# Excalibur1224/Cuda-v-MPI

Hardware: AMD Instinct MI355X
Metric: Riemann subintervals/sec at N=1e9 fp64; |error| vs analytic π (higher is better)
Workload: dtype fp64

## Files before the change

### csrc/cli/miint.cpp

```cpp
#include <algorithm>
#include <cmath>
#include <cstdio>
#include <string>
#include <vector>

#include "cli_common.hpp"
#include "miint/integrator.hpp"
#include "miint/oracle.hpp"
#include "miint/table2d.hpp"
#include "miint/trainscan.hpp"

using namespace miint;

namespace {

struct BenchRow {
  std::string integrand, dtype, rule;
  double n = 0, result = 0, exact = 0, ms = 0;
  int gpus = 1;
  int block = 0, grid = 0;
  bool multistep = false, close_in_launch = false, allreduce_to_host = false;
  BatchDiag diag;
  std::string timeline_file;
  cli::RankFacts facts;
  cli::Topology topo;
};

Integrand integrand_of(const std::string& s) { return cli::parse_integrand(s); }

RiemannConfig make_cfg(const std::string& integ, double n, const std::string& dtype,
                       const std::string& rule, const std::string& div) {
  RiemannConfig c;
  c.integrand = integrand_of(integ);
  c.a = 0.0;
  c.b = c.integrand == Integrand::kPi4 || c.integrand == Integrand::kPoly ? 1.0
      : c.integrand == Integrand::kSin ? 3.14159265358979323846 : 1800.0;
  c.n = static_cast<uint64_t>(n);
  c.dtype = cli::parse_dtype(dtype);
  c.rule = cli::parse_rule(rule);
  c.div = cli::parse_div(div);
  if (c.integrand == Integrand::kTrainVel) { c.p0 = oracle::kTrainTs; c.p1 = oracle::kTrainVs; }
  if (c.integrand == Integrand::kTable) c.table = oracle::profile_table();
  if (c.integrand == Integrand::kPoly) c.coef = {0.3, -1.2, 0.7, 0.05, -0.4, 0.9, 0.1};
  return c;
}

template <class T>
void write_rows(std::FILE* f, const std::vector<T>& v, size_t cols) {
  std::fputc('[', f);
  for (size_t i = 0; i < v.size(); ++i) {
    if (i % cols == 0) std::fputs(i ? ",[" : "[", f);
    else std::fputc(',', f);
    std::fprintf(f, "%llu", static_cast<unsigned long long>(v[i]));
    if (i % cols == cols - 1) std::fputc(']', f);
  }
  std::fputc(']', f);
}

void write_timeline(const std::string& path, const BatchTimeline& t, const RiemannConfig& cfg,
                    const std::string& integrand, const std::string& dtype,
                    const std::string& div, double plain_device_us) {
  std::FILE* f = std::fopen(path.c_str(), "w");
  if (!f) fail("--timeline: cannot open " + path + " for writing", __FILE__, __LINE__);
  std::fprintf(f, "{\"integrand\":\"%s\",\"n\":%llu,", cli::json_escape(integrand).c_str(),
               static_cast<unsigned long long>(cfg.n));
  if (cfg.slice_world > 0)
    std::fprintf(f, "\"slice_of\":[%d,%d],", cfg.slice_rank, cfg.slice_world);
  else
    std::fputs("\"slice_of\":null,", f);
  std::fprintf(f, "\"dtype\":\"%s\",\"div\":\"%s\",", cli::json_escape(dtype).c_str(),
               cli::json_escape(div).c_str());
  std::fprintf(f, "\"steps\":%d,\"grid\":%d,\"block\":%d,\"clock_khz\":%d,\"device_us\":%.17g,",
               t.steps, t.grid, t.block, t.clock_khz, t.device_us);
  if (plain_device_us > 0) std::fprintf(f, "\"plain_device_us\":%.17g,", plain_device_us);
  else std::fputs("\"plain_device_us\":null,", f);
  std::fputs("\"values\":[", f);
  for (size_t i = 0; i < t.values.size(); ++i)
    std::fprintf(f, i ? ",%.17g" : "%.17g", t.values[i]);
  std::fputs("],\n\"stamps\":", f);
  write_rows(f, t.stamps, static_cast<size_t>(t.steps) + 2);
  std::fputs(",\n\"shader_clock\":", f);
  write_rows(f, t.shader_clock, 2);
  std::fputs(",\n\"hw\":", f);
  write_rows(f, t.hw, 2);
  std::fputs("}\n", f);
  if (std::fclose(f) != 0) fail("--timeline: writing " + path + " failed", __FILE__, __LINE__);
}

struct TimelineRequest {
  std::string file, integrand, dtype, div;
};

BenchRow bench_one(const cli::Topology& topo, RiemannConfig cfg, int iters, bool graphs,
                   int settle_steps = -1, bool diagnose = false,
                   const TimelineRequest& timeline = {}) {
  BenchRow row;
  row.n = static_cast<double>(cfg.n);
  row.gpus = topo.world;
  row.exact = oracle::analytic(cfg.integrand, cfg.a, cfg.b, cfg.coef, cfg.p0, cfg.p1);
  row.topo = topo;
  std::mutex mu;
  cli::run_ranks(topo, [&](int rank, int dev, const Comm* comm) {
    RiemannPlan plan(cfg, dev, comm);
    RankAgree agree(comm);
    plan.run_steps(3, comm != nullptr, graphs);
    const double est_s = static_cast<double>(plan.count()) / 1.3e13;
    const int settle = settle_steps >= 0 ? settle_steps
                       : static_cast<int>(std::min(20000.0, std::max(3.0, 0.06 / est_s)));
    plan.run_steps(settle, comm != nullptr, graphs);
    StepTiming t = plan.run_steps(iters, comm != nullptr, graphs);
    const double ms = agree.max(t.wall_s * 1e3 / iters);
    BatchDiag d;
    if (diagnose) d = plan.diagnose_batch(std::min(iters, plan.config().slots));
    if (!timeline.file.empty()) {
      const BatchTimeline tl = plan.timeline_batch(std::min(iters, plan.config().slots));
      if (rank == 0)
        write_timeline(timeline.file, tl, cfg, timeline.integrand, timeline.dtype, timeline.div,
                       d.steps == tl.steps ? d.device_us : 0.0);
    }
    std::lock_guard<std::mutex> g(mu);
    if (ms > row.ms) row.ms = ms;
    if (rank == topo.rank0) {
      row.facts.note(comm);
      row.result = plan.host_result(plan.host_index_of(iters - 1, graphs));
      row.block = plan.shape().block;
      row.grid = plan.shape().grid;
      row.multistep = plan.multistep();
      row.close_in_launch = plan.close_in_launch();
      row.allreduce_to_host = plan.allreduce_to_host();
      row.diag = d;
      row.timeline_file = timeline.file;
    }
  });
  return row;
}

void print_row(const cli::Args& a, const BenchRow& r, const char* integ, const char* dtype,
               const char* rule) {
  cli::JsonRecord rec;
  rec.add("integrand", integ).add("dtype", dtype).add("rule", rule).add("n", r.n).add("gpus", r.gpus);
  r.facts.add(rec, r.topo);
  rec.add("block", r.block)
                   .add("grid", r.grid)
                   .add("multistep", r.multistep)
                   .add("close_in_launch", r.close_in_launch)
                   .add("allreduce_to_host", r.allreduce_to_host)
                   .add("ms_per_integration", r.ms)
                   .add("subintervals_per_s", r.n / (r.ms * 1e-3))
                   .add("result", r.result)
                   .add("analytic", r.exact)
                   .add("abs_err", std::fabs(r.result - r.exact));
  if (r.diag.steps > 0)
    rec.add("diag_steps", r.diag.steps)
        .add("diag_compute_us", r.diag.compute_us)
        .add("diag_close_us", r.diag.close_us)
        .add("diag_allreduce_us", r.diag.allreduce_us)
        .add("diag_copy_us", r.diag.copy_us)
        .add("diag_tail_us", r.diag.tail_us())
        .add("diag_boundary_us", r.diag.boundary_us())
        .add("diag_device_us", r.diag.device_us)
        .add("diag_marker_us", r.diag.marker_us)
        .add("diag_host_us", r.diag.wall_us - r.diag.device_us);
  if (!r.timeline_file.empty()) rec.add("timeline_file", r.timeline_file);
  cli::emit(a, rec, true);
}

int selfcheck() {
  int bad = 0;
  auto check = [&](const char* what, double got, double want, double tol) {
    const bool ok = std::fabs(got - want) <= tol;
    std::printf("%-44s got %.9f want %.9f  %s\n", what, got, want, ok ? "ok" : "MISMATCH");
    bad += !ok;
  };
  {
    RiemannPlan p(make_cfg("pi4", 1e9, "fp64", "left", "series"), 0);
    check("pi4 left N=1e9 (|err| = h)", p.run(), 3.14159265358979323846 + 1e-9, 2e-12);
  }
  {
    RiemannPlan p(make_cfg("pi4", 1e9, "fp64", "mid", "series"), 0);
    check("pi4 mid N=1e9", p.run(), 3.14159265358979323846, 1e-13);
  }
  {
    RiemannPlan p(make_cfg("sin", 1e9, "fp64", "left", "series"), 0);
    check("sin [0,pi] N=1e9", p.run(), 2.0, 1e-12);
  }
  {
    RiemannConfig c = make_cfg("table", 18e6, "fp64", "left", "series");
    RiemannPlan p(c, 0);
    check("cintegrate full coverage", p.run(), 122000.004000, 1e-6);
    c.b = 1792.0;
    c.n = 17920000;
    RiemannPlan q(c, 0);
    check("cintegrate --parity (SP=32,SM=2)", q.run(), 121999.800663, 5e-6);
  }
  {
    TrainScanConfig tc;
    TrainScan ts(tc, 0);
    const TrainScanResult r = ts.run();
    check("trainscan distance (P=1)", r.distance, 122000.004000, 1e-6);
  }
  std::printf("%s\n", bad ? "SELFCHECK FAILED" : "SELFCHECK OK");
  return bad ? 1 : 0;
}

int comm_sweep(const cli::Args& a, const cli::Topology& topo, double max_bytes, int iters) {
  std::vector<size_t> counts;
  for (size_t c = 1; c * 8.0 <= max_bytes; c *= 8) counts.push_back(c);
  if (counts.empty() || counts.back() * 8.0 < max_bytes) counts.push_back(static_cast<size_t>(max_bytes / 8));
  const char* ops[] = {"allreduce", "allgather", "broadcast"};
  std::vector<double> ms(counts.size() * 3, 0.0);
  std::mutex mu;
  auto body = [&](int , int dev, const Comm* comm) {
    DeviceGuard g(dev);
    Stream s;
    RankAgree agree(comm);
    const size_t cmax = counts.back();
    DeviceBuffer<double> a(cmax), b(cmax * static_cast<size_t>(comm->world()));
    MIINT_HIP(hipMemsetAsync(a.get(), 0, a.bytes(), s.get()));
    Event e0, e1;
    for (size_t k = 0; k < counts.size(); ++k)
      for (int op = 0; op < 3; ++op) {
        auto issue = [&] {
          if (op == 0) comm->allreduce_sum(a.get(), b.get(), counts[k], s.get());
          else if (op == 1) comm->allgather(a.get(), b.get(), counts[k], s.get());
          else comm->broadcast(a.get(), counts[k], 0, s.get());
        };
        for (int w = 0; w < 3; ++w) issue();
        s.sync();
        agree.barrier();
        e0.record(s.get());
        for (int i = 0; i < iters; ++i) issue();
        e1.record(s.get());
        e1.sync();
        comm->check_async();
        const double t = agree.max(Event::elapsed_ms(e0, e1) / iters);
        std::lock_guard<std::mutex> l(mu);
        ms[k * 3 + op] = std::max(ms[k * 3 + op], t);
      }
  };
  capture_rccl_log();
  if (!topo.multiproc && topo.world == 1) {
    auto one = RcclComm::init_all({0});
    body(0, 0, one[0].get());
  } else {
    cli::run_ranks(topo, body);
  }
  if (topo.rank0 != 0) return 0;
  const double P = topo.world;
  const RcclTransport tr = rccl_transport();
  const bool share = ranks_share_devices() && topo.world > 1;
  const std::string terr = transport_error(
      tr, topo.world, topo.multiproc ? cli::env_int("LOCAL_WORLD_SIZE", topo.world) : topo.world,
      share);
  if (!terr.empty()) std::fprintf(stderr, "miint comm: transport check: %s\n", terr.c_str());
  for (size_t k = 0; k < counts.size(); ++k)
    for (int op = 0; op < 3; ++op) {
      const double bytes = counts[k] * 8.0 * (op == 1 ? P : 1.0);
      const double t = ms[k * 3 + op];
      const double alg = bytes / (t * 1e-3) / 1e9;
      const double factor = op == 0 ? 2.0 * (P - 1) / P : (op == 1 ? (P - 1) / P : 1.0);
      cli::emit(a, cli::JsonRecord()
                       .add("op", ops[op])
                       .add("gpus", topo.world)
                       .add("bytes", bytes)
                       .add("us", t * 1e3)
                       .add("algbw_GBps", alg)
                       .add("busbw_GBps", alg * factor)
                       .add("ranks_share_gpus", ranks_share_devices() && topo.world > 1)
                       .add("rccl_transport", tr.transport)
                       .add("rccl_nnodes", tr.nnodes)
                       .add("transport_verified", terr.empty()),
                true);
    }
  return 0;
}

}

constexpr const char* kUsage =
    "usage: miint info\n"
    "       miint bench [--integrand pi4] [--n 1e9] [--dtype fp64|fp32|fp32acc] [--rule left]\n"
    "                   [--iters 200] [--gpus G] [--div series_exact|series|ieee] [--unfused] [--no-graph]\n"
    "                   [--block B] [--grid G] [--step-streams S] [--trig-library] [--settle N]\n"
    "                   [--no-multistep] [--slots K] [--close auto|kernel|launch] [--no-ar-host]\n"
    "                   [--diagnose] [--slice R/W] [--timeline FILE]\n"
    "                   (--timeline: after the timed run, one batch from the timeline build of\n"
    "                   the multi-step launch, per-workgroup device-clock stamps as JSON in FILE;\n"
    "                   read it with tools/timeline_report.py. --slice: rank R's share of W)\n"
    "       miint sweep [--gpus G]\n"
    "       miint table2d [--grid 4096] [--gpus G] [--slice R/W] [--no-graph]\n"
    "                     [--step-streams S] [--min-wg W] [--settle-ms MS] [--no-multistep]\n"
    "                     [--phases P] [--graph-steps K]\n"
    "       miint selfcheck\n"
    "       miint comm [--gpus G] [--max-bytes 144e6] [--iters 20]\n"
    "Every record is one JSON line on stdout; --jsonl FILE also appends it to FILE.\n";

int main(int argc, char** argv) {
  try {
    cli::Args a(argc, argv);
    if (cli::usage_requested(a, kUsage)) return 0;
    const std::string cmd = a.positional().empty() ? "info" : a.positional()[0];
    if (cmd == "info") {
      const int nd = device_count();
      std::printf("miint: %d HIP device(s), RCCL %s\n", nd, nd ? RcclComm::version().c_str() : "-");
      for (int d = 0; d < nd; ++d) {
        const DeviceInfo i = device_info(d);
        std::printf("  [%d] %s %s  %d CUs  %.1f GHz  %.1f GB  L2 %d KB  LDS %zu KB/CU (%zu KB/block)\n",
                    d, i.name.c_str(), i.arch.c_str(), i.num_cus, i.clock_khz / 1e6,
                    i.total_mem / 1e9, i.l2_bytes / 1024, i.lds_per_cu / 1024,
                    i.lds_per_block / 1024);
      }
      return 0;
    }
    if (cmd == "selfcheck") return selfcheck();
    {
      int r = 0, w = 0;
      cli::parse_slice(a, &r, &w);
    }
    const cli::Topology topo = cli::topology(a);
    const int iters = static_cast<int>(a.integer("iters", 100));
    const bool graphs = !a.flag("no-graph");
    if (cmd == "bench") {
      RiemannConfig c = make_cfg(a.str("integrand", "pi4"), a.num("n", 1e9), a.str("dtype", "fp64"),
                                 a.str("rule", "left"), a.str("div", "series_exact"));
      c.fused = !a.flag("unfused");
      c.grid = static_cast<int>(a.integer("grid", 0));
      c.block = static_cast<int>(a.integer("block", kRiemannBlock));
      c.step_streams = static_cast<int>(a.integer("step-streams", 0));
      c.multistep = !a.flag("no-multistep");
      c.slots = static_cast<int>(a.integer("slots", c.slots));
      c.close = a.str("close", c.close);
      c.allreduce_to_host = !a.flag("no-ar-host");
      cli::parse_slice(a, &c.slice_rank, &c.slice_world);
      TimelineRequest tl;
      tl.file = a.str("timeline", "");
      tl.integrand = a.str("integrand", "pi4");
      tl.dtype = a.str("dtype", "fp64");
      tl.div = a.str("div", "series_exact");
      if (!tl.file.empty() && c.close == "launch")
        fail(std::string("--timeline: ") + kTimelineNoCloseInLaunch, __FILE__, __LINE__);
      if (a.flag("trig-library")) set_trig_library(true);
      MIINT_CHECK(riemann_block_ok(c.block), "--block must be 64, 128, 256, 512 or 1024");
      c.waves_per_cu = static_cast<int>(a.integer("waves-per-cu", 32));
      const BenchRow r = bench_one(topo, c, iters, graphs,
                                   static_cast<int>(a.integer("settle", -1)),
                                   a.flag("diagnose"), tl);
      if (topo.rank0 == 0)
        print_row(a, r, a.str("integrand", "pi4").c_str(), a.str("dtype", "fp64").c_str(),
                  a.str("rule", "left").c_str());
      return 0;
    }
    if (cmd == "table2d") {
      Table2DConfig c;
      c.grid = static_cast<int>(a.integer("grid", 4096));
      c.bucket = !a.flag("no-bucket");
      c.chain = !a.flag("no-chain");
      c.step_streams = static_cast<int>(a.integer("step-streams", 0));
      c.min_wg = static_cast<int>(a.integer("min-wg", 0));
      c.settle_ms = a.num("settle-ms", c.settle_ms);
      c.multistep = !a.flag("no-multistep");
      c.phases = static_cast<int>(a.integer("phases", 0));
      c.graph_steps = static_cast<int>(a.integer("graph-steps", 0));
      cli::parse_slice(a, &c.rank, &c.world);
      double value = 0.0, timed = 0.0, ms = 0.0;
      bool bucketed = false, chained = false, multistep = false;
      int streams = 1, phases = 0, resident = 0, min_wg = 0, wgs = 0, gsteps = 0;
      cli::RankFacts facts;
      std::mutex mu;
      cli::run_ranks(topo, [&](int rank, int dev, const Comm* comm) {
        Table2DPlan plan(c, dev, comm);
        RankAgree agree(comm);
        const double v = plan.run();
        const double t = agree.max(plan.time(iters, graphs));
        std::lock_guard<std::mutex> g(mu);
        if (rank == topo.rank0) {
          facts.note(comm);
          value = v;
          timed = plan.last_result();
          bucketed = plan.bucketed() && graphs;
          chained = plan.chained() && graphs;
          multistep = plan.multistep() && graphs;
          streams = chained ? plan.step_streams() : 1;
          phases = multistep ? plan.phases() : 0;
          resident = plan.resident_per_cu();
          min_wg = plan.min_wg();
          wgs = plan.workgroups();
          gsteps = graphs ? plan.graph_steps() : 0;
        }
        if (t > ms) ms = t;
      });
      if (topo.rank0 == 0) {
        cli::JsonRecord r;
        r.add("program", "table2d").add("grid", c.grid);
        r.add("step_streams", streams).add("multistep", multistep).add("phases", phases);
        r.add("resident_per_cu", resident).add("min_wg", min_wg).add("workgroups", wgs);
        r.add("graph_steps", gsteps);
        facts.add(r, topo);
        if (c.world > 1) {
          r.add("slice", std::to_string(c.rank) + "/" + std::to_string(c.world))
              .add("partial", value);
        } else {
          const double want = table2d_oracle(c.grid);
          const double exact = 122000.004 * 122000.004;
          r.add("gpus", topo.world)
              .add("result", value)
              .add("timed_result", timed)
              .add("bucketed_allreduce", bucketed)
              .add("chained", chained)
              .add("midpoint_oracle", want)
              .add("rel_err_vs_oracle", std::fabs(value - want) / want)
              .add("rel_err_vs_exact", std::fabs(value - exact) / exact)
              .add("samples_per_s", static_cast<double>(c.grid) * c.grid / (ms * 1e-3));
        }
        cli::emit(a, r.add("ms_per_integration", ms), true);
      }
      return 0;
    }
    if (cmd == "comm") return comm_sweep(a, topo, a.num("max-bytes", 144e6), static_cast<int>(a.integer("iters", 20)));
    if (cmd == "sweep") {
      const std::vector<double> ns = {1e6, 1e9, 1e10};
      const std::vector<std::string> integs = {"pi4", "sin", "poly", "train"};
      for (const auto& integ : integs)
        for (const char* dt : {"fp64", "fp32"}) {
          if (std::string(dt) == "fp32" && integ != "pi4") continue;
          for (double n : ns) {
            if (integ != "pi4" && n > 1e9) continue;
            RiemannConfig c = make_cfg(integ, n, dt, "left", "series");
            const int it = n >= 1e10 ? 10 : (n >= 1e9 ? 50 : 500);
            const BenchRow r = bench_one(topo, c, it, graphs);
            if (topo.rank0 == 0) print_row(a, r, integ.c_str(), dt, "left");
          }
        }
      return 0;
    }
    std::fprintf(stderr, "usage: miint info|bench|sweep|table2d|comm|selfcheck [--flags]\n");
    return 2;
  } catch (const std::exception& e) {
    std::fprintf(stderr, "miint: %s\n", e.what());
    return 1;
  }
}
```

### csrc/include/miint/integrator.hpp

```cpp
#pragma once

#include <hip/hip_runtime.h>

#include <cstdint>
#include <map>
#include <memory>
#include <string>
#include <vector>

#include "miint/comm.hpp"
#include "miint/common.hpp"
#include "miint/kernels.hpp"
#include "miint/runtime.hpp"

namespace miint {

constexpr int kAutoStepStreams = 4;
constexpr uint64_t kStepStreamsMaxCount = 600000000ull;

struct RiemannConfig {
  Integrand integrand = Integrand::kPi4;
  double a = 0.0, b = 1.0;
  uint64_t n = 1000000000ull;
  Rule rule = Rule::kLeft;
  DType dtype = DType::kF64;
  DivMode div = DivMode::kSeriesExact;
  std::vector<double> coef;
  double p0 = 0.0, p1 = 0.0;
  std::vector<double> table;
  int grid = 0;
  int block = kRiemannBlock;
  int waves_per_cu = 32;
  bool fused = true;
  bool chain = true;
  bool host_direct = true;
  int slots = 16;
  bool bucket = true;
  int rank = 0, world = 1;
  bool force_collective = false;
  bool multistep = true;
  std::string close = "auto";
  bool allreduce_to_host = true;
  int step_streams = 0;
  int slice_rank = 0, slice_world = 0;
  double timeout_s = 300.0;
};

inline void rank_slice(uint64_t n, int r, int w, uint64_t* begin, uint64_t* count) {
  const uint64_t q = n / static_cast<uint64_t>(w), rem = n % static_cast<uint64_t>(w);
  const uint64_t ur = static_cast<uint64_t>(r);
  *count = q + (ur < rem ? 1 : 0);
  *begin = ur * q + (ur < rem ? ur : rem);
}

struct StepTiming {
  double wall_s = 0.0;
  double device_ms = 0.0;
  int steps = 0;
};

struct OneShotTiming {
  std::string mode;
  int reps = 0;
  double median_us = 0.0, min_us = 0.0, max_us = 0.0;
  double device_median_us = 0.0, device_min_us = 0.0;
  double value = 0.0;
};

struct BatchDiag {
  int steps = 0;
  double compute_us = 0.0;
  double close_us = 0.0;
  double allreduce_us = 0.0;
  double copy_us = 0.0;
  double marker_us = 0.0;
  double device_us = 0.0;
  double staged_us = 0.0;
  double wall_us = 0.0;
  double tail_us() const { return close_us + allreduce_us + copy_us; }
  double boundary_us() const { return device_us - compute_us - tail_us(); }
};

struct BatchTimeline {
  int steps = 0, grid = 0, block = 0;
  int clock_khz = 0;
  std::vector<uint64_t> stamps;
  std::vector<uint64_t> shader_clock;
  std::vector<uint32_t> hw;
  double device_us = 0.0;
  std::vector<double> values;
};
constexpr uint64_t kTimelineUnsetStamp = 0;
constexpr uint32_t kTimelineUnsetId = 0xffffffffu;

class RiemannPlan {
 public:
  RiemannPlan(const RiemannConfig& cfg, int device, const Comm* comm = nullptr);
  ~RiemannPlan();
  RiemannPlan(const RiemannPlan&) = delete;
  RiemannPlan& operator=(const RiemannPlan&) = delete;

  const RiemannConfig& config() const { return cfg_; }
  int device() const { return device_; }
  int rank() const { return rank_; }
  int world() const { return world_; }
  uint64_t begin() const { return params_.i_begin; }
  uint64_t count() const { return params_.n; }
  double h() const { return params_.h; }
  double scale() const { return scale_; }
  LaunchShape shape() const { return shape_; }
  DivMode effective_div() const;
  bool direct() const { return direct_; }

  void enqueue_compute(hipStream_t s, int slot, int host_index) const;
  void enqueue_reduce(hipStream_t s, int slot) const;
  void enqueue_copyout(hipStream_t s, int slot, int host_index) const;
  void enqueue(hipStream_t s, int slot, int host_index) const;

  double* device_result(int slot) const { return result_.get() + slot; }
  double host_result(int host_index) const { return host_[host_index]; }
  int host_capacity() const { return static_cast<int>(host_.size()); }
  int slots() const { return cfg_.slots; }

  double run();
  void capture_graphs();
  void prepare_steps(int steps);
  bool graphs_ready() const { return !graphs_.empty() && graph_error_.empty(); }
  const std::string& graph_error() const { return graph_error_; }
  size_t graph_nodes() const;
  long graph_launches() const { return graph_launches_; }
  long direct_steps() const { return direct_steps_; }

  StepTiming run_steps(int steps, bool pipeline, bool graphs);
  BatchDiag diagnose_batch(int nsteps);
  BatchTimeline timeline_batch(int nsteps);
  void barrier();
  OneShotTiming time_one_shot(int reps, const std::string& mode, int warmup = 400);
  void launch_steps(int steps, bool pipeline, bool graphs);
  void sync() const;
  int host_index_of(int k, bool graphs) const;
  hipStream_t compute_stream() const { return compute_.get(); }
  hipStream_t comm_stream() const { return comm_stream_.get(); }

  bool collective() const { return comm_ && (world_ > 1 || cfg_.force_collective); }
  bool bucketed() const { return collective() && cfg_.bucket; }
  bool chained() const { return cfg_.fused && cfg_.chain && (!collective() || bucketed()); }
  bool multistep() const { return chained() && multistep_; }
  bool close_in_launch() const { return multistep() && close_launch_; }
  bool allreduce_to_host() const {
    return bucketed() && cfg_.allreduce_to_host && ar_host_ok_;
  }
  void check_allreduce_to_host();

 private:
  void enqueue_batch(hipStream_t cs, hipStream_t rs, int nsteps, bool overlap);
  void enqueue_bucket_reduce(hipStream_t s, int nsteps) const;
  void enqueue_chain(hipStream_t s, int nsteps) const;
  void enqueue_chain_streams(hipStream_t cs, int nsteps);
 public:
  int step_streams(int nsteps) const;
 private:
  const Graph* batch_graph(int nsteps);
  bool use_graphs(bool requested, int steps);
  double* result_ptr(int j) const { return direct_ ? host_.device_ptr() + j : result_.get() + j; }

  RiemannConfig cfg_;
  int device_;
  const Comm* comm_;
  int rank_ = 0, world_ = 1;
  bool direct_ = false;
  RiemannParams params_{};
  double scale_ = 1.0;
  LaunchShape shape_{1, kRiemannBlock};
  DeviceBuffer<double> partials_;
  DeviceBuffer<double> slots_;
  DeviceBuffer<double> ms_partials_;
  bool multistep_ = false;
  bool close_launch_ = false;
  bool capturing_ = false;
  bool ar_host_ok_ = true;
  bool ar_host_checked_ = false;
  DeviceBuffer<unsigned int> ms_ticket_;
  DeviceBuffer<uint64_t> tl_stamps_, tl_shader_;
  DeviceBuffer<uint32_t> tl_hw_;
  DeviceBuffer<double> result_;
  DeviceBuffer<double> sync_;
  DeviceBuffer<unsigned int> ticket_;
  DeviceBuffer<double> table_;
  PinnedBuffer<double> host_;
  Stream compute_;
  Stream comm_stream_;
  std::vector<Stream> step_streams_;
  std::vector<std::unique_ptr<Event>> ev_step_join_;
  std::vector<std::unique_ptr<Event>> ev_computed_, ev_drained_;
  Event ev_fork_, ev_join_;
  Event ev_t0_, ev_t1_;
  std::map<int, std::unique_ptr<Graph>> graphs_;
  std::string graph_error_;
  long graph_launches_ = 0, direct_steps_ = 0;
  int last_mode_ = -1;
};

}
```

### csrc/include/miint/kernels.hpp

```cpp
#pragma once

#include <hip/hip_runtime.h>

#include <algorithm>
#include <cmath>
#include <cstddef>
#include <cstdint>

#include "miint/common.hpp"

namespace miint {

enum class DType : int { kF64 = 0, kF32 = 1, kF32Acc32 = 2 };
inline bool is_fp32(DType t) { return t == DType::kF32 || t == DType::kF32Acc32; }

constexpr int kRiemannTile = 32;
constexpr int kRiemannBlock = 256;
constexpr int kSeriesHalfSpan = 192;
constexpr int kSeriesHalfSpanF32 = 96;

constexpr int kDirectHalfSpan = 16;

inline bool series_ok(double h) { return kSeriesHalfSpan * (h < 0 ? -h : h) <= 2e-6; }
inline bool series_ok_f32(double h) { return kSeriesHalfSpanF32 * (h < 0 ? -h : h) <= 2e-6; }
inline bool direct_ok(double h) { return kDirectHalfSpan * (h < 0 ? -h : h) <= 2e-6; }

inline DivMode effective_div(DivMode d, double h) {
  if (d == DivMode::kIeee) return d;
  if ((d == DivMode::kSeries || d == DivMode::kSeriesExact) && series_ok(h)) return d;
  return direct_ok(h) ? DivMode::kSeriesDirect : DivMode::kIeee;
}
inline bool series_request(DivMode d) { return d == DivMode::kSeries || d == DivMode::kSeriesExact; }
inline DivMode effective_div(DivMode d, double h, Integrand f) {
  if (f == Integrand::kSin || f == Integrand::kTrainVel || f == Integrand::kTable)
    return series_request(d) ? DivMode::kSeries : DivMode::kIeee;
  if (f != Integrand::kPi4) return DivMode::kIeee;
  return effective_div(d, h);
}

constexpr int kPolySeriesMaxCoeffs = 8;

inline DivMode effective_div(DivMode d, double h, Integrand f, DType t, int ncoef = 0) {
  if (is_fp32(t)) {
    if (d == DivMode::kIeee) return DivMode::kIeee;
    if (f == Integrand::kPi4) return series_ok_f32(h) ? DivMode::kSeries : DivMode::kIeee;
    if (f == Integrand::kPoly)
      return (ncoef >= 1 && ncoef <= kPolySeriesMaxCoeffs) ? DivMode::kSeries : DivMode::kIeee;
    return DivMode::kSeries;
  }
  if (f == Integrand::kPoly)
    return (series_request(d) && ncoef >= 1 && ncoef <= kPolySeriesMaxCoeffs)
               ? DivMode::kSeries
               : DivMode::kIeee;
  return effective_div(d, h, f);
}

constexpr double kTrigSeriesMaxN = 2147418112.0;
inline bool trig_series_in_range(const RiemannParams& p) {
  const Integrand f = static_cast<Integrand>(p.integrand);
  if (f != Integrand::kSin && f != Integrand::kTrainVel) return true;
  const double first = static_cast<double>(p.i_begin) + p.off;
  const double last = static_cast<double>(p.i_begin + (p.n > 0 ? p.n - 1 : 0)) + p.off;
  const double w = f == Integrand::kTrainVel ? 1.0 / p.p0 : 1.0;
  const double n0 = std::fabs(std::fma(first, p.h, p.a) * w) * 6.36619772367581382433e-01;
  const double n1 = std::fabs(std::fma(last, p.h, p.a) * w) * 6.36619772367581382433e-01;
  return n0 <= kTrigSeriesMaxN && n1 <= kTrigSeriesMaxN;
}
constexpr double kPi4SeriesMaxX = 0x1p249;
constexpr double kPi4SeriesMaxXF32 = 0x1p62;
inline bool pi4_series_in_range(const RiemannParams& p, DType t) {
  if (static_cast<Integrand>(p.integrand) != Integrand::kPi4) return true;
  const double lim = is_fp32(t) ? kPi4SeriesMaxXF32 : kPi4SeriesMaxX;
  const double first = static_cast<double>(p.i_begin) + p.off;
  const double last = static_cast<double>(p.i_begin + (p.n > 0 ? p.n - 1 : 0)) + p.off;
  return std::fabs(std::fma(first, p.h, p.a)) < lim && std::fabs(std::fma(last, p.h, p.a)) < lim;
}
inline DivMode effective_div(const RiemannParams& p, DivMode d, DType t) {
  const DivMode e = effective_div(d, p.h, static_cast<Integrand>(p.integrand), t, p.ncoef);
  return (e != DivMode::kIeee && !(trig_series_in_range(p) && pi4_series_in_range(p, t)))
             ? DivMode::kIeee
             : e;
}

struct LaunchShape {
  int grid;
  int block;
};

bool riemann_block_ok(int block);
LaunchShape default_riemann_shape(int num_cus, int waves_per_cu = 32, int block = kRiemannBlock);

void launch_riemann_partials(const RiemannParams& p, DType dtype, DivMode div,
                             LaunchShape shape, const double* table, int table_n,
                             double* partials, hipStream_t stream);

void launch_finalize(const double* partials, int n, double scale, double* out,
                     hipStream_t stream, int block = kRiemannBlock);

constexpr unsigned kUnsetSlotWord = 0xFFFAFFFAu;
void fill_unset_slots(double* p, size_t count, hipStream_t stream);

constexpr int kTicketGroups = 16;
constexpr int kTicketStride = 64;
constexpr int kTicketWords = (kTicketGroups + 1) * kTicketStride;

void launch_riemann_fused(const RiemannParams& p, DType dtype, DivMode div, LaunchShape shape,
                          const double* table, int table_n, double* partials,
                          unsigned int* ticket, double scale, double* out, hipStream_t stream);

void launch_riemann_chained(const RiemannParams& p, DType dtype, DivMode div, LaunchShape shape,
                            const double* table, int table_n, double* partials,
                            const double* prev, int nprev, double scale, double* out_prev,
                            hipStream_t stream);

constexpr int kMaxMultiSteps = 64;
int riemann_multistep_grid(const RiemannParams& p, DType dtype, DivMode div, int block,
                           int num_cus, bool close = false);
void launch_riemann_multistep(const RiemannParams& p, DType dtype, DivMode div,
                              LaunchShape shape, const double* table, int table_n,
                              double* partials, int steps, double scale, double* out,
                              hipStream_t stream, unsigned int* ticket = nullptr,
                              bool close_kernel = true);
constexpr const char* kTimelineNoCloseInLaunch =
    "the timeline instruments the kernel-closed multi-step launch only (not close = launch)";
int riemann_timeline_grid(const RiemannParams& p, DType dtype, DivMode div, int block,
                          int num_cus);
void launch_riemann_timeline(const RiemannParams& p, DType dtype, DivMode div,
                             LaunchShape shape, const double* table, int table_n,
                             double* partials, int steps, double scale, double* out,
                             hipStream_t stream, uint64_t* stamps, uint64_t* shader_clock,
                             uint32_t* hw, unsigned int* ticket = nullptr,
                             bool close_kernel = true);
void launch_multistep_close(const double* partials, int grid, int steps, double scale,
                            double* out, int block, hipStream_t stream);

void launch_riemann_point_values(const RiemannParams& p, DivMode div, const double* table,
                                 int table_n, double* out, hipStream_t stream);

void launch_pi4_recip_narrow(const double* d, uint64_t n, double* out, hipStream_t stream);
void launch_pi4_recip_narrow_f32(const float* d, uint64_t n, float* out, hipStream_t stream);
void set_pi4_library_division(bool on);
bool pi4_ieee_narrow(const RiemannParams& p, DType dtype);
void set_trig_library(bool on);
void set_lds_poison(bool on);
void set_lds_poison_trainscan(bool on);
void set_lds_poison_table(bool on);

int riemann_tile_len(const RiemannParams& p, DType dtype, DivMode div);

double integrand_scale(Integrand f);

int default_reduce_grid(int num_cus);
void launch_sum_array(const double* x, uint64_t n, double scale, double* partials, int grid,
                      double* out, hipStream_t stream);

void launch_interp_fill(const double* table, int table_n, double dt, uint64_t i0, uint64_t n,
                        double* y, hipStream_t stream);

size_t scan_state_bytes(uint64_t n);
void launch_inclusive_scan(const double* in, double* out, uint64_t n, void* state,
                           const double* carry_in, hipStream_t stream);
void launch_interp_scan(const double* table, int table_n, double dt, uint64_t i0, uint64_t n,
                        double* out, void* state, const double* carry_in, hipStream_t stream);
void launch_interp_scan_window(const double* table, int table_n, double dt, uint64_t i0,
                               uint64_t n, uint64_t win_lo, uint64_t win_hi, double* out,
                               void* state, const double* carry_in, hipStream_t stream);
unsigned scan_timeout_flag(const void* state, hipStream_t stream);
void launch_add_carry(double* x, uint64_t n, const double* carry, hipStream_t stream);

struct Table2DParams {
  const double* table;
  int nx, ny;
  double X, Y;
  int gx, gy;
  int row0, row1;
  int min_wg = 0;
};
int table2d_grid(const Table2DParams& p);
const char* table2d_path(const Table2DParams& p);
struct Table2DShapeInfo {
  bool stream;
  int rows_per_wave, tile_rows, tile_cols, grid_x, grid_y, tile;
};
Table2DShapeInfo table2d_shape_info(const Table2DParams& p);
constexpr int kT2AutoPhases = 16;
constexpr long kT2AutoWorkgroups = 4096;
constexpr int kT2MaxPhases = 32;
constexpr int kT2MaxReplaySteps = 1024;
bool table2d_multistep_ok(const Table2DParams& p, int num_cus);
int table2d_multistep_resident(const Table2DParams& p);
int table2d_multistep_phases(const Table2DParams& p, int num_cus, int steps, int want = 0);
void launch_table2d_multistep(const Table2DParams& p, double* partials, int steps, double* outs,
                              hipStream_t stream, int phases = 1);
void launch_table2d_partials(const Table2DParams& p, double* partials, hipStream_t stream);
void launch_table2d_fused(const Table2DParams& p, double* partials, unsigned* ticket,
                          double* out, hipStream_t stream);
void launch_table2d_chained(const Table2DParams& p, double* partials, const double* prev,
                            double* prev_out, hipStream_t stream);
void launch_table2d_finalize(const double* partials, int n, double* out, hipStream_t stream);
void launch_outer_product(const double* v, int n, double* table, hipStream_t stream);

}
```

### csrc/kernels/riemann.hip

```cpp
#include <hip/hip_runtime.h>

#include <atomic>
#include <cmath>
#include <string>

#include "miint/common.hpp"
#include "miint/handoff.hpp"
#include "miint/integrands.hpp"
#include "miint/integrands_f32.hpp"
#include "miint/kernels.hpp"
#include "miint/wave_reduce.hpp"

namespace miint {
namespace {

constexpr int B = kRiemannBlock;
constexpr int kMaxBlock = 1024;

__device__ __forceinline__ uint64_t readlane_u64(uint64_t v, int lane) {
  const uint32_t lo = __builtin_amdgcn_readlane(static_cast<uint32_t>(v), lane);
  const uint32_t hi = __builtin_amdgcn_readlane(static_cast<uint32_t>(v >> 32), lane);
  return (static_cast<uint64_t>(hi) << 32) | lo;
}

// ... 412 lines not shown

#define kFullOccupancy __attribute__((amdgpu_waves_per_eu(8, 8)))
template <DivMode M, class F>
constexpr bool occupancy_hint() {
  if constexpr (__is_same(F, Pi4)) return M == DivMode::kSeriesDirect;
  else if constexpr (__is_same(F, Pi4F32) || __is_same(F, Pi4F32Wide) ||
                     __is_same(F, Pi4F32Acc32))
    return M == DivMode::kIeee;
  else if constexpr (__is_same(F, SinLib) || __is_same(F, TrainVelLib)) return true;
  else if constexpr (__is_same(F, Sin)) return M == DivMode::kIeee;
  else if constexpr (__is_same(F, PolyF32<16>)) return true;
  else if constexpr (IsPoly<F>::value) return M == DivMode::kSeries;
  else if constexpr (__is_same(F, SinF32) || __is_same(F, TrainVelF32))
    return M == DivMode::kSeries;
  else return __is_same(F, TrainVel) || __is_same(F, Table) || __is_same(F, TableF32);
}

template <DivMode M, class F>
__device__ __forceinline__ void partials_body(const RiemannParams& p, const double* table,
                                              int table_n, double* partials) {
  using Acc = typename AccOf<F>::type;
  __shared__ Acc red[kMaxBlock / kWave];
  __shared__ double lds[lds_words<M, F>()];
  const F f = make_functor<M, F>(p, table, table_n, lds);
  const double s = static_cast<double>(block_sum_dyn(lane_sum<M>(p, f, blockIdx.x), red));
  if (threadIdx.x == 0) partials[blockIdx.x] = s;
}
template <DivMode M, class F>
__global__ __launch_bounds__(kMaxBlock) void riemann_kernel(RiemannParams p, const double* table,
                                                    int table_n, double* partials) {
  partials_body<M, F>(p, table, table_n, partials);
}
template <DivMode M, class F>
__global__ __launch_bounds__(kMaxBlock) kFullOccupancy void riemann_kernel_o8(RiemannParams p,
                                                                      const double* table,
                                                                      int table_n,
                                                                      double* partials) {
  partials_body<M, F>(p, table, table_n, partials);
}

__device__ __forceinline__ double ordered_sum(const double* partials, int n, double* red) {
  return block_sum_dyn(ordered_partials<0, false>(partials, n), red);
}

__global__ __launch_bounds__(kMaxBlock) void finalize_kernel(const double* partials, int n,
                                                             double scale, double* out) {
  __shared__ double red[kMaxBlock / kWave];
  const double s = ordered_sum(partials, n, red);
  if (threadIdx.x == 0) out[0] = s * scale;
}

template <DivMode M, class F>
__device__ __forceinline__ void fused_body(const RiemannParams& p, const double* table,
                                           int table_n, double* partials, unsigned int* ticket,
                                           double scale, double* out) {
  using Acc = typename AccOf<F>::type;
  __shared__ double red[kMaxBlock / kWave];
  __shared__ Acc red_acc[__is_same(Acc, double) ? 1 : kMaxBlock / kWave];
  __shared__ double lds[lds_words<M, F>()];
  __shared__ int is_last;
  const F f = make_functor<M, F>(p, table, table_n, lds);
  double s;
  if constexpr (__is_same(Acc, double)) s = block_sum_dyn(lane_sum<M>(p, f, blockIdx.x), red);
  else s = static_cast<double>(block_sum_dyn(lane_sum<M>(p, f, blockIdx.x), red_acc));
  if (!publish_and_ticket(s, partials, ticket, blockIdx.x, gridDim.x, &is_last)) return;
  const double v = ordered_partials<0, true>(partials, static_cast<int>(gridDim.x));
  rearm_slots<0>(partials, static_cast<int>(gridDim.x));
  const double tot = block_sum_dyn(v, red);
  if (threadIdx.x == 0) out[0] = tot * scale;
  rearm_ticket(ticket, gridDim.x);
}
template <DivMode M, class F>
__global__ __launch_bounds__(kMaxBlock) void riemann_fused_kernel(RiemannParams p, const double* table,
                                                          int table_n, double* partials,
                                                          unsigned int* ticket, double scale,
                                                          double* out) {
  fused_body<M, F>(p, table, table_n, partials, ticket, scale, out);
}
template <DivMode M, class F>
__global__ __launch_bounds__(kMaxBlock) kFullOccupancy void riemann_fused_kernel_o8(
    RiemannParams p, const double* table, int table_n, double* partials, unsigned int* ticket,
    double scale, double* out) {
  fused_body<M, F>(p, table, table_n, partials, ticket, scale, out);
}

template <DivMode M, class F>
__device__ __forceinline__ void chained_body(const RiemannParams& p, const double* table,
                                             int table_n, double* partials, const double* prev,
                                             int nprev, double scale, double* out_prev) {
  __shared__ double red[kMaxBlock / kWave];
  __shared__ double lds[lds_words<M, F>()];
  if (prev != nullptr && blockIdx.x == gridDim.x - 1) {
    const double tot = block_sum_dyn(ordered_partials<0, false>(prev, nprev), red);
    if (threadIdx.x == 0) out_prev[0] = tot * scale;
    __syncthreads();
  }
  const F f = make_functor<M, F>(p, table, table_n, lds);
  double s;
  if constexpr (__is_same(typename AccOf<F>::type, double)) {
    s = block_sum_dyn(lane_sum<M>(p, f, blockIdx.x), red);
  } else {
    __shared__ typename AccOf<F>::type red_acc[kMaxBlock / kWave];
    s = static_cast<double>(block_sum_dyn(lane_sum<M>(p, f, blockIdx.x), red_acc));
  }
  if (threadIdx.x == 0) partials[blockIdx.x] = s;
}
template <DivMode M, class F>
__global__ __launch_bounds__(kMaxBlock) void riemann_chained_kernel(RiemannParams p, const double* table,
                                                            int table_n, double* partials,
                                                            const double* prev, int nprev,
                                                            double scale, double* out_prev) {
  chained_body<M, F>(p, table, table_n, partials, prev, nprev, scale, out_prev);
}
template <DivMode M, class F>
__global__ __launch_bounds__(kMaxBlock) kFullOccupancy void riemann_chained_kernel_o8(
    RiemannParams p, const double* table, int table_n, double* partials, const double* prev,
    int nprev, double scale, double* out_prev) {
  chained_body<M, F>(p, table, table_n, partials, prev, nprev, scale, out_prev);
}

#ifndef MIINT_MS_CHUNK
#define MIINT_MS_CHUNK 1
#endif
template <class F>
constexpr int ms_chunk() {
  return __is_same(F, Pi4) ? MIINT_MS_CHUNK : 1;
}

struct TimelineOut {
  unsigned long long* stamps;
  unsigned long long* shader_clock;
  unsigned* hw;
};
__device__ __forceinline__ unsigned long long timeline_realtime() {
  unsigned long long t;
  asm volatile("s_memrealtime %0\n\ts_waitcnt lgkmcnt(0)" : "=s"(t) : : "memory");
  return t;
}
__device__ __forceinline__ unsigned long long timeline_realtime_after(double sum) {
  unsigned long long t;
  asm volatile("s_memrealtime %0\n\ts_waitcnt lgkmcnt(0)" : "=s"(t) : "v"(sum) : "memory");
  return t;
}
__device__ __forceinline__ unsigned long long timeline_shader_clock() {
  unsigned long long t;
  asm volatile("s_memtime %0\n\ts_waitcnt lgkmcnt(0)" : "=s"(t) : : "memory");
  return t;
}
template <class T>
__device__ __forceinline__ T* timeline_row(T* base, int row_len) {
  unsigned wg = blockIdx.x;
  asm volatile("" : "+v"(wg));
  return base + static_cast<size_t>(wg) * static_cast<size_t>(row_len);
}
struct TimelineEntry {
  unsigned long long t, clk;
};
__device__ __forceinline__ TimelineEntry timeline_entry() {
  TimelineEntry e;
  e.t = timeline_realtime();
  e.clk = timeline_shader_clock();
  return e;
}
__device__ __forceinline__ void timeline_step(const TimelineOut& tl, int steps, int s,
                                              double sum) {
  const unsigned long long t = timeline_realtime_after(sum);
  timeline_row(tl.stamps, steps + 2)[s + 1] = t;
}
__device__ __forceinline__ void timeline_exit(const TimelineOut& tl, int steps,
                                              const TimelineEntry& e) {
  const unsigned long long t = timeline_realtime();
  unsigned long long* clk = timeline_row(tl.shader_clock, 2);
  clk[0] = e.clk;
  clk[1] = timeline_shader_clock();
  unsigned long long* st = timeline_row(tl.stamps, steps + 2);
  st[0] = e.t;
  st[steps + 1] = t;
  unsigned xcc, hw;
  asm volatile("s_getreg_b32 %0, hwreg(HW_REG_XCC_ID)" : "=s"(xcc));
  asm volatile("s_getreg_b32 %0, hwreg(HW_REG_HW_ID)" : "=s"(hw));
  unsigned* id = timeline_row(tl.hw, 2);
  id[0] = xcc;
  id[1] = hw;
}

template <DivMode M, class F, bool CLOSE, bool TL = false>
__device__ __forceinline__ void multistep_body(const RiemannParams& p, const double* table,
                                               int table_n, double* partials, int steps,
                                               unsigned rot, unsigned* ticket, double scale,
                                               double* out, TimelineOut tl = {}) {
  using Acc = typename AccOf<F>::type;
  constexpr int C = ms_chunk<F>();
  if constexpr (TL) {
    static_assert(!CLOSE, "the timeline covers the kernel-closed step loop only");
    static_assert(C == 1, "the timeline covers one step per block sum (MIINT_MS_CHUNK = 1)");
  }
  TimelineEntry te{};
  if constexpr (TL) te = timeline_entry();
  __shared__ double red[2][C * (kMaxBlock / kWave)];
  __shared__ Acc red_acc[2][__is_same(Acc, double) ? 1 : C * (kMaxBlock / kWave)];
  __shared__ double lds[lds_words<M, F>()];
  const F f = make_functor<M, F>(p, table, table_n, lds);
  const unsigned nb = gridDim.x;
  const TileSplit sp = tile_split<F::template tile_len<M>()>(p.n);
  unsigned vb = blockIdx.x;
  unsigned seq = 0;
  int s = 0;
  if constexpr (C > 1) {
    for (; s + C <= steps; s += C, ++seq) {
      const unsigned vb0 = vb;
      Acc l[C];
#pragma unroll
      for (int k = 0; k < C; ++k) l[k] = Acc(0);
#pragma unroll 1
      for (int c = 0; c < C; ++c) {
        RiemannParams q = p;
        asm volatile("" : "+s"(q.a));
        const Acc x = lane_sum<M>(q, f, vb, sp);
#pragma unroll
        for (int k = 0; k < C; ++k) l[k] = k == c ? x : l[k];
        vb += rot;
        if (vb >= nb) vb -= nb;
      }
      Acc v[C];
      if constexpr (__is_same(Acc, double)) block_sums_dyn<C>(l, red[seq & 1], v);
      else block_sums_dyn<C>(l, red_acc[seq & 1], v);
      if (threadIdx.x == 0) {
        unsigned w = vb0;
#pragma unroll
        for (int k = 0; k < C; ++k) {
          const double vk = static_cast<double>(v[k]);
          if constexpr (CLOSE) slot_store(&partials[static_cast<size_t>(s + k) * nb + w], vk);
          else partials[static_cast<size_t>(s + k) * nb + w] = vk;
          w += rot;
          if (w >= nb) w -= nb;
        }
      }
    }
  }
  for (; s < steps; ++s, ++seq) {
    RiemannParams q = p;
    asm volatile("" : "+s"(q.a));
    double v;
    if constexpr (__is_same(Acc, double)) v = block_sum_dyn(lane_sum<M>(q, f, vb, sp), red[seq & 1]);
    else v = static_cast<double>(block_sum_dyn(lane_sum<M>(q, f, vb, sp), red_acc[seq & 1]));
    if (threadIdx.x == 0) {
      if constexpr (TL) timeline_step(tl, steps, s, v);
      if constexpr (CLOSE) slot_store(&partials[static_cast<size_t>(s) * nb + vb], v);
      else partials[static_cast<size_t>(s) * nb + vb] = v;
    }
    vb += rot;
    if (vb >= nb) vb -= nb;
  }
  if constexpr (TL) {
    if (threadIdx.x == 0) timeline_exit(tl, steps, te);
  }
  if constexpr (CLOSE) {
    __shared__ int role;
    __syncthreads();
    close_batch_in_launch(partials, nb, steps, ticket, scale, out, red[0], &role);
  }
}
template <DivMode M, class F>
__global__ __launch_bounds__(kMaxBlock) void riemann_timeline_kernel(
    RiemannParams p, const double* table, int table_n, double* partials, int steps,
    unsigned rot, TimelineOut tl) {
  multistep_body<M, F, false, true>(p, table, table_n, partials, steps, rot, nullptr, 0.0,
                                    nullptr, tl);
}
template <DivMode M, class F>
__global__ __launch_bounds__(kMaxBlock) kFullOccupancy void riemann_timeline_kernel_o8(
    RiemannParams p, const double* table, int table_n, double* partials, int steps,
    unsigned rot, TimelineOut tl) {
  multistep_body<M, F, false, true>(p, table, table_n, partials, steps, rot, nullptr, 0.0,
                                    nullptr, tl);
}
template <DivMode M, class F, bool CLOSE>
__global__ __launch_bounds__(kMaxBlock) void riemann_multistep_kernel(
    RiemannParams p, const double* table, int table_n, double* partials, int steps,
    unsigned rot, unsigned* ticket, double scale, double* out) {
  multistep_body<M, F, CLOSE>(p, table, table_n, partials, steps, rot, ticket, scale, out);
}
template <DivMode M, class F, bool CLOSE>
__global__ __launch_bounds__(kMaxBlock) kFullOccupancy void riemann_multistep_kernel_o8(
    RiemannParams p, const double* table, int table_n, double* partials, int steps,
    unsigned rot, unsigned* ticket, double scale, double* out) {
  multistep_body<M, F, CLOSE>(p, table, table_n, partials, steps, rot, ticket, scale, out);
}
template <DivMode M, class F>
constexpr bool multistep_o8() {
  if constexpr (__is_same(F, Table) || __is_same(F, TableF32)) return true;
  return M == DivMode::kIeee && (__is_same(F, Pi4F32) || __is_same(F, Pi4F32Wide) ||
                                 __is_same(F, Pi4F32Acc32));
}
template <DivMode M, class F>
constexpr bool multistep_close_ok() {
  return !multistep_o8<M, F>();
}
template <DivMode M, class F>
constexpr bool multistep_pays() {
  return !(M == DivMode::kIeee && (__is_same(F, Pi4) || __is_same(F, Pi4Wide)));
}

__global__ __launch_bounds__(kMaxBlock) void multistep_close_kernel(const double* partials,
                                                                   int nb, double scale,
                                                                   double* out) {
  __shared__ double red[kMaxBlock / kWave];
  const double t = ordered_partials<0, false>(partials + static_cast<size_t>(blockIdx.x) * nb, nb);
  const double tot = block_sum_dyn(t, red);
  if (threadIdx.x == 0) out[blockIdx.x] = tot * scale;
}

template <DivMode M, class F>
__global__ __launch_bounds__(B) void point_values_kernel(RiemannParams p, const double* table,
                                                         int table_n, double* out) {
  constexpr int T = F::template tile_len<M>();
  __shared__ double lds[lds_words<M, F>()];
  const F f = make_functor<M, F>(p, table, table_n, lds);
  const uint64_t t = static_cast<uint64_t>(blockIdx.x) * B + threadIdx.x;
  if (t * T >= p.n) return;
  const double x0 = fma(static_cast<double>(p.i_begin) + p.off + static_cast<double>(t * T),
                        p.h, p.a);
  const double xm = fma(0.5 * (T - 1), p.h, x0);
  const bool full = (t + 1) * T <= p.n;
  for (int u = 0; u < T && t * T + u < p.n; ++u) {
    const double x = fma(static_cast<double>(u), p.h, x0);
    double v;
    if constexpr (M == DivMode::kSeries && __is_same(F, Pi4)) {
      v = full ? f.series_point(xm, p.h, u) : f.point(x);
    } else if constexpr (M == DivMode::kSeriesExact && __is_same(F, Pi4)) {
      v = full ? f.series_exact_point(xm, p.h, u) : f.point(x);
    } else if constexpr (M == DivMode::kSeries && IsPolyF64<F>::value) {
      v = full ? f.series_point(xm, u) : f.point(x);
    } else if constexpr (M == DivMode::kSeries && __is_same(F, Table)) {
      v = full ? f.series_point(xm, p.h, u) : f.point(x);
    } else if constexpr (M == DivMode::kSeries && (__is_same(F, Sin) || __is_same(F, TrainVel))) {
      v = full ? f.series_point(xm, u) : f.point(x);
    } else if constexpr (M == DivMode::kSeriesDirect && __is_same(F, Pi4)) {
      const Pi4::Seed sd = Pi4::seed(xm, p.h);
      const double e = fma(-fma(x, x, 1.0), sd.s, 1.0);
      v = fma(sd.s, e + e * e, sd.s);
    } else if constexpr (M == DivMode::kIeee && __is_same(F, Pi4)) {
      v = full ? Pi4::recip_narrow(fma(x, x, 1.0)) : f.point(x);
    } else if constexpr (M == DivMode::kIeee &&
                         (__is_same(F, Sin) || __is_same(F, SinLib) ||
                          __is_same(F, TrainVel) || __is_same(F, TrainVelLib))) {
      v = full ? f.template ieee_point<T>(x0, p.h, u) : f.point(x);
    } else {
      v = f.point(x);
    }
    out[t * T + u] = v * F::kScale;
  }
}

__global__ __launch_bounds__(B) void recip_narrow_kernel(const double* d, uint64_t n,
                                                         double* out) {
  const uint64_t stride = static_cast<uint64_t>(gridDim.x) * B;
  for (uint64_t i = static_cast<uint64_t>(blockIdx.x) * B + threadIdx.x; i < n; i += stride)
    out[i] = Pi4::recip_narrow(d[i]);
}
__global__ __launch_bounds__(B) void recip_narrow_f32_kernel(const float* d, uint64_t n,
                                                             float* out) {
  const uint64_t stride = static_cast<uint64_t>(gridDim.x) * B;
  for (uint64_t i = static_cast<uint64_t>(blockIdx.x) * B + threadIdx.x; i < n; i += stride)
    out[i] = Pi4F32::recip_narrow(f32x2{d[i], d[i]}).x;
}

template <DivMode M, class F>
void launch_partials_t(const RiemannParams& p, LaunchShape shape, const double* table,
                       int table_n, double* partials, hipStream_t stream) {
  if constexpr (occupancy_hint<M, F>())
    riemann_kernel_o8<M, F><<<shape.grid, shape.block, 0, stream>>>(p, table, table_n, partials);
  else
    riemann_kernel<M, F><<<shape.grid, shape.block, 0, stream>>>(p, table, table_n, partials);
}
template <DivMode M, class F>
void launch_fused_t(const RiemannParams& p, LaunchShape shape, const double* table, int table_n,
                    double* partials, unsigned* ticket, double scale, double* out,
                    hipStream_t stream) {
  if constexpr (occupancy_hint<M, F>())
    riemann_fused_kernel_o8<M, F>
        <<<shape.grid, shape.block, 0, stream>>>(p, table, table_n, partials, ticket, scale, out);
  else
    riemann_fused_kernel<M, F>
        <<<shape.grid, shape.block, 0, stream>>>(p, table, table_n, partials, ticket, scale, out);
}

template <DivMode M, class F>
void launch_chained_t(const RiemannParams& p, LaunchShape shape, const double* table,
                      int table_n, double* partials, const double* prev, int nprev, double scale,
                      double* out_prev, hipStream_t stream) {
  if constexpr (occupancy_hint<M, F>())
    riemann_chained_kernel_o8<M, F><<<shape.grid, shape.block, 0, stream>>>(p, table, table_n, partials,
                                                                  prev, nprev, scale, out_prev);
  else
    riemann_chained_kernel<M, F><<<shape.grid, shape.block, 0, stream>>>(p, table, table_n, partials,
                                                               prev, nprev, scale, out_prev);
}

template <DivMode M, class F, bool CLOSE>
void launch_multistep_c(const RiemannParams& p, LaunchShape shape, const double* table,
                        int table_n, double* partials, int steps, unsigned rot,
                        unsigned* ticket, double scale, double* out, hipStream_t stream) {
  if constexpr (multistep_o8<M, F>())
    riemann_multistep_kernel_o8<M, F, CLOSE><<<shape.grid, shape.block, 0, stream>>>(
        p, table, table_n, partials, steps, rot, ticket, scale, out);
  else
    riemann_multistep_kernel<M, F, CLOSE><<<shape.grid, shape.block, 0, stream>>>(
        p, table, table_n, partials, steps, rot, ticket, scale, out);
}
template <DivMode M, class F>
void launch_multistep_t(const RiemannParams& p, LaunchShape shape, const double* table,
                        int table_n, double* partials, int steps, unsigned rot,
                        unsigned* ticket, double scale, double* out, hipStream_t stream) {
  if constexpr (multistep_pays<M, F>()) {
    if constexpr (multistep_close_ok<M, F>()) {
      if (ticket) {
        launch_multistep_c<M, F, true>(p, shape, table, table_n, partials, steps, rot, ticket,
                                       scale, out, stream);
        return;
      }
    } else {
      MIINT_CHECK(ticket == nullptr, "this integrand closes multi-step batches by a kernel");
    }
    launch_multistep_c<M, F, false>(p, shape, table, table_n, partials, steps, rot, ticket,
                                    scale, out, stream);
  } else {
    fail("this integrand/division keeps chained batches (no multi-step kernel)", __FILE__,
         __LINE__);
  }
}
template <DivMode M, class F, bool CLOSE>
int multistep_occupancy(int block) {
  int n = 0;
  if constexpr (multistep_o8<M, F>())
    MIINT_HIP(hipOccupancyMaxActiveBlocksPerMultiprocessor(
        &n, reinterpret_cast<const void*>(&riemann_multistep_kernel_o8<M, F, CLOSE>), block, 0));
  else
    MIINT_HIP(hipOccupancyMaxActiveBlocksPerMultiprocessor(
        &n, reinterpret_cast<const void*>(&riemann_multistep_kernel<M, F, CLOSE>), block, 0));
  return n;
}
template <DivMode M, class F>
void multistep_per_cu_t(int block, bool close, int* out) {
  if constexpr (!multistep_pays<M, F>())
    *out = 0;
  else if constexpr (!multistep_close_ok<M, F>())
    *out = close ? 0 : multistep_occupancy<M, F, false>(block);
  else
    *out = close ? multistep_occupancy<M, F, true>(block) : multistep_occupancy<M, F, false>(block);
}

template <DivMode M, class F>
void launch_timeline_t(const RiemannParams& p, LaunchShape shape, const double* table,
                       int table_n, double* partials, int steps, unsigned rot, TimelineOut tl,
                       hipStream_t stream) {
  if constexpr (!multistep_pays<M, F>())
    fail("this integrand/division keeps chained batches (no multi-step kernel, no timeline)",
         __FILE__, __LINE__);
  else if constexpr (multistep_o8<M, F>())
    riemann_timeline_kernel_o8<M, F><<<shape.grid, shape.block, 0, stream>>>(
        p, table, table_n, partials, steps, rot, tl);
  else
    riemann_timeline_kernel<M, F><<<shape.grid, shape.block, 0, stream>>>(
        p, table, table_n, partials, steps, rot, tl);
}
template <DivMode M, class F>
void timeline_per_cu_t(int block, int* out) {
  *out = 0;
  if constexpr (multistep_pays<M, F>()) {
    if constexpr (multistep_o8<M, F>())
      MIINT_HIP(hipOccupancyMaxActiveBlocksPerMultiprocessor(
          out, reinterpret_cast<const void*>(&riemann_timeline_kernel_o8<M, F>), block, 0));
    else
      MIINT_HIP(hipOccupancyMaxActiveBlocksPerMultiprocessor(
          out, reinterpret_cast<const void*>(&riemann_timeline_kernel<M, F>), block, 0));
  }
}

std::atomic<bool> g_pi4_library_division{false};
std::atomic<bool> g_trig_library{false};
inline bool trig_library() { return g_trig_library.load(std::memory_order_relaxed); }
inline bool pi4_narrow(const RiemannParams& p, double max_x = kPi4NarrowMaxX) {
  if (g_pi4_library_division.load(std::memory_order_relaxed)) return false;
  const double first = static_cast<double>(p.i_begin) + p.off;
  const double last = static_cast<double>(p.i_begin + (p.n > 0 ? p.n - 1 : 0)) + p.off;
  return std::fabs(std::fma(first, p.h, p.a)) < max_x &&
         std::fabs(std::fma(last, p.h, p.a)) < max_x;
}

template <template <DivMode, class> class Op, class... A>
void dispatch(const RiemannParams& p, DType dtype, DivMode m, A&&... a) {
  const Integrand f = static_cast<Integrand>(p.integrand);
  if (dtype == DType::kF32Acc32) {
    MIINT_CHECK(f == Integrand::kPi4, "fp32 accumulation (fp32acc) is implemented for pi4 only");
    if (m == DivMode::kSeries) Op<DivMode::kSeries, Pi4F32Acc32>::run(a...);
    else if (pi4_narrow(p, kPi4F32NarrowMaxX)) Op<DivMode::kIeee, Pi4F32Acc32>::run(a...);
    else fail("fp32acc: coordinates beyond 2^49 need the wide division (use fp32)", __FILE__,
              __LINE__);
    return;
  }
  if (dtype == DType::kF32) {
    const bool ser = m == DivMode::kSeries;
    switch (f) {
      case Integrand::kPi4:
        if (ser) Op<DivMode::kSeries, Pi4F32>::run(a...);
        else if (pi4_narrow(p, kPi4F32NarrowMaxX)) Op<DivMode::kIeee, Pi4F32>::run(a...);
        else Op<DivMode::kIeee, Pi4F32Wide>::run(a...);
        return;
      case Integrand::kSin:
        if (ser) Op<DivMode::kSeries, SinF32>::run(a...);
        else if (!trig_series_in_range(p)) Op<DivMode::kIeee, Sin>::run(a...);
        else Op<DivMode::kIeee, SinF32>::run(a...);
        return;
      case Integrand::kTrainVel:
        if (ser) Op<DivMode::kSeries, TrainVelF32>::run(a...);
        else if (!trig_series_in_range(p)) Op<DivMode::kIeee, TrainVel>::run(a...);
        else Op<DivMode::kIeee, TrainVelF32>::run(a...);
        return;
      case Integrand::kTable:
        if (ser) Op<DivMode::kSeries, TableF32>::run(a...);
        else Op<DivMode::kIeee, TableF32>::run(a...);
        return;
      case Integrand::kPoly:
        if (ser && p.ncoef <= 4) Op<DivMode::kSeries, PolyF32<4>>::run(a...);
        else if (ser && p.ncoef <= 6) Op<DivMode::kSeries, PolyF32<6>>::run(a...);
        else if (ser && p.ncoef == 7) Op<DivMode::kSeries, PolyF32<7>>::run(a...);
        else if (ser && p.ncoef <= 8) Op<DivMode::kSeries, PolyF32<8>>::run(a...);
        else if (p.ncoef <= 4) Op<DivMode::kIeee, PolyF32<4>>::run(a...);
        else if (p.ncoef <= 8) Op<DivMode::kIeee, PolyF32<8>>::run(a...);
        else Op<DivMode::kIeee, PolyF32<16>>::run(a...);
        return;
    }
    fail("unknown integrand", __FILE__, __LINE__);
  }
  switch (f) {
    case Integrand::kPi4:
      if (m == DivMode::kSeries) Op<DivMode::kSeries, Pi4>::run(a...);
      else if (m == DivMode::kSeriesExact) Op<DivMode::kSeriesExact, Pi4>::run(a...);
      else if (m == DivMode::kSeriesDirect) Op<DivMode::kSeriesDirect, Pi4>::run(a...);
      else if (pi4_narrow(p)) Op<DivMode::kIeee, Pi4>::run(a...);
      else Op<DivMode::kIeee, Pi4Wide>::run(a...);
      return;
    case Integrand::kSin:
      if (m == DivMode::kSeries) Op<DivMode::kSeries, Sin>::run(a...);
      else if (trig_library()) Op<DivMode::kIeee, SinLib>::run(a...);
      else Op<DivMode::kIeee, Sin>::run(a...);
      return;
    case Integrand::kPoly:
      if (m == DivMode::kSeries && p.ncoef <= 4) Op<DivMode::kSeries, Poly<4>>::run(a...);
      else if (m == DivMode::kSeries && p.ncoef <= 6) Op<DivMode::kSeries, Poly<6>>::run(a...);
      else if (m == DivMode::kSeries && p.ncoef == 7) Op<DivMode::kSeries, Poly<7>>::run(a...);
      else if (m == DivMode::kSeries && p.ncoef <= 8) Op<DivMode::kSeries, Poly<8>>::run(a...);
      else if (p.ncoef <= 4) Op<DivMode::kIeee, Poly<4>>::run(a...);
      else if (p.ncoef <= 8) Op<DivMode::kIeee, Poly<8>>::run(a...);
      else Op<DivMode::kIeee, Poly<16>>::run(a...);
      return;
    case Integrand::kTrainVel:
      if (m == DivMode::kSeries) Op<DivMode::kSeries, TrainVel>::run(a...);
      else if (trig_library()) Op<DivMode::kIeee, TrainVelLib>::run(a...);
      else Op<DivMode::kIeee, TrainVel>::run(a...);
      return;
    case Integrand::kTable:
      if (m == DivMode::kSeries) Op<DivMode::kSeries, Table>::run(a...);
      else Op<DivMode::kIeee, Table>::run(a...);
      return;
  }
  fail("unknown integrand", __FILE__, __LINE__);
}

template <DivMode M, class F> struct PartialsOp {
  template <class... A> static void run(A... a) { launch_partials_t<M, F>(a...); }
};
template <DivMode M, class F> struct FusedOp {
  template <class... A> static void run(A... a) { launch_fused_t<M, F>(a...); }
};
template <DivMode M, class F> struct ChainedOp {
  template <class... A> static void run(A... a) { launch_chained_t<M, F>(a...); }
};
template <DivMode M, class F> struct MultiStepOp {
  template <class... A> static void run(A... a) { launch_multistep_t<M, F>(a...); }
};
template <DivMode M, class F> struct MultiStepOccOp {
  static void run(int block, bool close, int* out) { multistep_per_cu_t<M, F>(block, close, out); }
};
template <DivMode M, class F> struct TimelineOp {
  template <class... A> static void run(A... a) { launch_timeline_t<M, F>(a...); }
};
template <DivMode M, class F> struct TimelineOccOp {
  static void run(int block, int* out) { timeline_per_cu_t<M, F>(block, out); }
};
template <DivMode M, class F> struct TileLenOp {
  static void run(int* out) { *out = F::template tile_len<M>(); }
};
template <DivMode M, class F> struct PointsOp {
  static void run(const RiemannParams& p, const double* table, int table_n, double* out,
                  hipStream_t stream) {
    constexpr int T = F::template tile_len<M>();
    const uint64_t ntile = (p.n + T - 1) / T;
    const int grid = static_cast<int>((ntile + B - 1) / B);
    point_values_kernel<M, F><<<grid, B, 0, stream>>>(p, table, table_n, out);
  }
};

}

bool riemann_block_ok(int block) {
  return block == 64 || block == 128 || block == 256 || block == 512 || block == 1024;
}

LaunchShape default_riemann_shape(int num_cus, int waves_per_cu, int block) {
  MIINT_CHECK(riemann_block_ok(block), "unsupported Riemann block size");
  const int waves_per_block = block / kWave;
  int blocks = (num_cus * waves_per_cu) / waves_per_block;
  if (blocks < 1) blocks = 1;
  return {blocks, block};
}

double integrand_scale(Integrand f) { return f == Integrand::kPi4 ? Pi4::kScale : 1.0; }

static void check_shape(LaunchShape s) {
  MIINT_CHECK(riemann_block_ok(s.block),
              "riemann kernels run 64-, 128-, 256-, 512- or 1024-thread workgroups (got " +
                  std::to_string(s.block) + ")");
  MIINT_CHECK(s.grid >= 1 && s.grid <= (1 << 20), "grid out of range");
}

static void check_params(const RiemannParams& p, const double* table, int table_n) {
  const int f = p.integrand;
  MIINT_CHECK(f >= 0 && f <= static_cast<int>(Integrand::kTable), "unknown integrand");
  if (static_cast<Integrand>(f) == Integrand::kTable) {
    MIINT_CHECK(table != nullptr, "table integrand needs a device table");
    MIINT_CHECK(table_n >= 2 && table_n <= kMaxTable, "table size must be in [2, 2048]");
  }
  if (static_cast<Integrand>(f) == Integrand::kPoly)
    MIINT_CHECK(p.ncoef >= 1 && p.ncoef <= kMaxPolyCoeffs, "poly needs 1..16 coefficients");
  if (static_cast<Integrand>(f) == Integrand::kTrainVel)
    MIINT_CHECK(p.p0 != 0.0, "train integrand needs ts != 0");
  MIINT_CHECK(p.i_begin + p.n < (uint64_t(1) << 52), "sample index must stay below 2^52");
}

static RiemannParams prepared(const RiemannParams& p, DivMode eff) {
  RiemannParams q = p;
  const Integrand f = static_cast<Integrand>(p.integrand);
  if (f == Integrand::kPoly && eff == DivMode::kSeries) {
    long double hp = 1.0L;
    for (int i = 0; i < kMaxPolyCoeffs; ++i) {
      q.coef_h[i] = i < p.ncoef ? static_cast<double>(static_cast<long double>(p.coef[i]) * hp)
                                : 0.0;
      hp *= static_cast<long double>(p.h);
    }
  }
  if ((f == Integrand::kSin || f == Integrand::kTrainVel) && eff == DivMode::kSeries) {
    const long double delta =
        f == Integrand::kSin ? static_cast<long double>(p.h)
                             : static_cast<long double>(p.h) / static_cast<long double>(p.p0);
    for (int j = 0; j < AngleSeries<12>::kPairs; ++j) {
      const long double k = j + 0.5L;
      q.trig[j] = static_cast<double>(cosl(k * delta));
      q.trig[AngleSeries<12>::kPairs + j] = static_cast<double>(sinl(k * delta));
    }
    for (int i = 0; i < AngleSeries<12>::kSubs / 2; ++i) {
      const long double c0 = AngleSeries<12>::kSub * (i + 0.5L);
      q.trig[2 * AngleSeries<12>::kPairs + 2 * i] = static_cast<double>(cosl(c0 * delta));
      q.trig[2 * AngleSeries<12>::kPairs + 2 * i + 1] = static_cast<double>(sinl(c0 * delta));
    }
    for (int i = 0; i < kSinTrig; ++i) q.trig32[i] = static_cast<float>(q.trig[i]);
  }
  return q;
}

int riemann_tile_len(const RiemannParams& p, DType dtype, DivMode div) {
  int t = 0;
  dispatch<TileLenOp>(p, dtype, effective_div(p, div, dtype), &t);
  return t;
}

void launch_riemann_partials(const RiemannParams& p, DType dtype, DivMode div, LaunchShape shape,
                             const double* table, int table_n, double* partials,
                             hipStream_t stream) {
  check_shape(shape);
  check_params(p, table, table_n);
  const DivMode eff = effective_div(p, div, dtype);
  dispatch<PartialsOp>(p, dtype, eff, prepared(p, eff), shape, table, table_n, partials, stream);
  MIINT_HIP(hipGetLastError());
}

void launch_finalize(const double* partials, int n, double scale, double* out,
                     hipStream_t stream, int block) {
  MIINT_CHECK(n >= 1, "finalize needs at least one partial");
  MIINT_CHECK(riemann_block_ok(block), "unsupported finalize block size");
  finalize_kernel<<<1, block, 0, stream>>>(partials, n, scale, out);
  MIINT_HIP(hipGetLastError());
}

void launch_riemann_fused(const RiemannParams& p, DType dtype, DivMode div, LaunchShape shape,
                          const double* table, int table_n, double* partials,
                          unsigned int* ticket, double scale, double* out, hipStream_t stream) {
  check_shape(shape);
  check_params(p, table, table_n);
  const DivMode eff = effective_div(p, div, dtype);
  dispatch<FusedOp>(p, dtype, eff, prepared(p, eff), shape, table, table_n, partials, ticket,
                    scale, out, stream);
  MIINT_HIP(hipGetLastError());
}

void launch_riemann_chained(const RiemannParams& p, DType dtype, DivMode div, LaunchShape shape,
                            const double* table, int table_n, double* partials,
                            const double* prev, int nprev, double scale, double* out_prev,
                            hipStream_t stream) {
  check_shape(shape);
  check_params(p, table, table_n);
  MIINT_CHECK(prev == nullptr || (nprev == shape.grid && out_prev != nullptr),
              "chained finalize: previous partials must come from the same grid");
  const DivMode eff = effective_div(p, div, dtype);
  dispatch<ChainedOp>(p, dtype, eff, prepared(p, eff), shape, table, table_n, partials, prev,
                      nprev, scale, out_prev, stream);
  MIINT_HIP(hipGetLastError());
}

int riemann_multistep_grid(const RiemannParams& p, DType dtype, DivMode div, int block,
                          int num_cus, bool close) {
  MIINT_CHECK(riemann_block_ok(block), "unsupported Riemann block size");
  int per_cu = 0;
  dispatch<MultiStepOccOp>(p, dtype, effective_div(p, div, dtype), block, close, &per_cu);
  return per_cu * num_cus;
}

static unsigned multistep_rot(const RiemannParams& p, DType dtype, DivMode eff,
                              LaunchShape shape) {
  int tl = 0;
  dispatch<TileLenOp>(p, dtype, eff, &tl);
  const uint64_t lanes = static_cast<uint64_t>(shape.grid) * static_cast<uint64_t>(shape.block);
  const uint64_t extra = (p.n / static_cast<uint64_t>(tl)) % lanes;
  const unsigned heavy = static_cast<unsigned>((extra + shape.block - 1) / shape.block);
  return heavy % static_cast<unsigned>(shape.grid);
}

void launch_riemann_multistep(const RiemannParams& p, DType dtype, DivMode div,
                              LaunchShape shape, const double* table, int table_n,
                              double* partials, int steps, double scale, double* out,
                              hipStream_t stream, unsigned int* ticket, bool close_kernel) {
  check_shape(shape);
  check_params(p, table, table_n);
  MIINT_CHECK(steps >= 1 && steps <= kMaxMultiSteps, "multi-step launch: 1..64 steps");
  MIINT_CHECK(partials != nullptr && out != nullptr, "multi-step launch needs partials and results");
  const DivMode eff = effective_div(p, div, dtype);
  const unsigned rot = multistep_rot(p, dtype, eff, shape);
  dispatch<MultiStepOp>(p, dtype, eff, prepared(p, eff), shape, table, table_n, partials, steps,
                        rot, ticket, scale, out, stream);
  MIINT_HIP(hipGetLastError());
  if (ticket || !close_kernel) return;
  launch_multistep_close(partials, shape.grid, steps, scale, out, shape.block, stream);
}

int riemann_timeline_grid(const RiemannParams& p, DType dtype, DivMode div, int block,
                          int num_cus) {
  MIINT_CHECK(riemann_block_ok(block), "unsupported Riemann block size");
  int per_cu = 0;
  dispatch<TimelineOccOp>(p, dtype, effective_div(p, div, dtype), block, &per_cu);
  return per_cu * num_cus;
}

void launch_riemann_timeline(const RiemannParams& p, DType dtype, DivMode div,
                             LaunchShape shape, const double* table, int table_n,
                             double* partials, int steps, double scale, double* out,
                             hipStream_t stream, uint64_t* stamps, uint64_t* shader_clock,
                             uint32_t* hw, unsigned int* ticket, bool close_kernel) {
  check_shape(shape);
  check_params(p, table, table_n);
  MIINT_CHECK(ticket == nullptr, kTimelineNoCloseInLaunch);
  MIINT_CHECK(steps >= 1 && steps <= kMaxMultiSteps, "timeline launch: 1..64 steps");
  MIINT_CHECK(partials != nullptr && out != nullptr, "timeline launch needs partials and results");
  MIINT_CHECK(stamps != nullptr && shader_clock != nullptr && hw != nullptr,
              "timeline launch needs its three buffers");
  const DivMode eff = effective_div(p, div, dtype);
  const unsigned rot = multistep_rot(p, dtype, eff, shape);
  static_assert(sizeof(unsigned long long) == sizeof(uint64_t), "stamp words are 64-bit");
  const TimelineOut tl{reinterpret_cast<unsigned long long*>(stamps),
                       reinterpret_cast<unsigned long long*>(shader_clock), hw};
  dispatch<TimelineOp>(p, dtype, eff, prepared(p, eff), shape, table, table_n, partials, steps,
                       rot, tl, stream);
  MIINT_HIP(hipGetLastError());
  if (!close_kernel) return;
  launch_multistep_close(partials, shape.grid, steps, scale, out, shape.block, stream);
}

void launch_multistep_close(const double* partials, int grid, int steps, double scale,
                            double* out, int block, hipStream_t stream) {
  MIINT_CHECK(steps >= 1 && steps <= kMaxMultiSteps && grid >= 1 && riemann_block_ok(block),
              "multi-step close: 1..64 steps, a Riemann block size");
  multistep_close_kernel<<<steps, block, 0, stream>>>(partials, grid, scale, out);
  MIINT_HIP(hipGetLastError());
}

void launch_riemann_point_values(const RiemannParams& p, DivMode div, const double* table,
                                 int table_n, double* out, hipStream_t stream) {
  check_params(p, table, table_n);
  MIINT_CHECK(p.n >= 1, "empty range");
  const DivMode eff = effective_div(p, div, DType::kF64);
  dispatch<PointsOp>(p, DType::kF64, eff, prepared(p, eff), table, table_n, out, stream);
  MIINT_HIP(hipGetLastError());
}

void set_pi4_library_division(bool on) { g_pi4_library_division.store(on); }
bool pi4_ieee_narrow(const RiemannParams& p, DType dtype) {
  return pi4_narrow(p, is_fp32(dtype) ? kPi4F32NarrowMaxX : kPi4NarrowMaxX);
}
void set_trig_library(bool on) { g_trig_library.store(on); }

void launch_pi4_recip_narrow(const double* d, uint64_t n, double* out, hipStream_t stream) {
  if (n == 0) return;
  const uint64_t blocks = (n + B - 1) / B;
  const int grid = static_cast<int>(blocks < 8192 ? blocks : 8192);
  recip_narrow_kernel<<<grid, B, 0, stream>>>(d, n, out);
  MIINT_HIP(hipGetLastError());
}

void launch_pi4_recip_narrow_f32(const float* d, uint64_t n, float* out, hipStream_t stream) {
  if (n == 0) return;
  const uint64_t blocks = (n + B - 1) / B;
  const int grid = static_cast<int>(blocks < 8192 ? blocks : 8192);
  recip_narrow_f32_kernel<<<grid, B, 0, stream>>>(d, n, out);
  MIINT_HIP(hipGetLastError());
}

}
```

### csrc/python/module.cpp

```cpp
#include <pybind11/numpy.h>
#include <pybind11/pybind11.h>
#include <pybind11/stl.h>

#include <algorithm>
#include <cmath>
#include <cstdint>
#include <string>
#include <vector>

#include "miint/comm.hpp"
#include "miint/expr.hpp"
#include "miint/fast_trig.hpp"
#include "miint/host.hpp"
#include "miint/integrator.hpp"
#include "miint/kernels.hpp"
#include "miint/oracle.hpp"
#include "miint/runtime.hpp"
#include "miint/selftest.hpp"
#include "miint/table2d.hpp"
#include "miint/trace.hpp"
#include "miint/trainscan.hpp"

namespace py = pybind11;
using namespace miint;

namespace {

template <typename T>
T* ptr(uintptr_t p) { return reinterpret_cast<T*>(p); }
hipStream_t stream(uintptr_t s) { return reinterpret_cast<hipStream_t>(s); }

RiemannParams make_params(int integrand, double a, double h, double off, uint64_t i_begin,
                          uint64_t n, const std::vector<double>& coef, double p0, double p1) {
  RiemannParams p{};
  p.a = a;
  p.h = h;
  p.off = off;
  p.i_begin = i_begin;
  p.n = n;
  p.integrand = integrand;
  MIINT_CHECK(coef.size() <= static_cast<size_t>(kMaxPolyCoeffs), "too many coefficients");
  p.ncoef = static_cast<int>(coef.size());
  for (size_t i = 0; i < coef.size(); ++i) p.coef[i] = coef[i];
  p.p0 = p0;
  p.p1 = p1;
  return p;
}

using ParamRows = py::object;
std::vector<double> param_rows(const ParamRows& obj, int nparams, uint64_t* rows) {
  auto arr = py::array_t<double, py::array::c_style | py::array::forcecast>::ensure(obj);
  if (!arr) {
    PyErr_Clear();
    fail("expression sweep: params must be K rows of " + std::to_string(nparams) +
             " numbers (a list of rows or a 2-D float64 array)", __FILE__, __LINE__);
  }
  if (arr.size() == 0 && arr.ndim() >= 1 && arr.shape(0) == 0) {
    *rows = 0;
    return {};
  }
  MIINT_CHECK(arr.ndim() == 2, "expression sweep: params must be 2-D (K rows x nparams)");
  MIINT_CHECK(arr.shape(1) == nparams,
              "expression sweep: rows of " + std::to_string(arr.shape(1)) +
                  " values, the expression was built for nparams = " + std::to_string(nparams));
  *rows = static_cast<uint64_t>(arr.shape(0));
  return std::vector<double>(arr.data(), arr.data() + arr.size());
}

}

static const char* scan_algo_name(ScanAlgo a) {
  return a == ScanAlgo::kFused ? "fused" : a == ScanAlgo::kOnePass ? "onepass" : "lookback";
}
static ScanAlgo scan_algo_of(const std::string& s) {
  MIINT_CHECK(s == "fused" || s == "lookback" || s == "onepass",
              "algo must be onepass|fused|lookback");
  return s == "fused" ? ScanAlgo::kFused : s == "onepass" ? ScanAlgo::kOnePass : ScanAlgo::kLookback;
}

PYBIND11_MODULE(_miint, m) {
  m.doc() = "miint: MI355X-native numerical integration (HIP/gfx950 kernels, RCCL, hipGraph)";
  py::register_exception<miint::Error>(m, "MiintError", PyExc_RuntimeError);
  install_crash_handler_from_env();

  py::enum_<Integrand>(m, "Integrand")
      .value("pi4", Integrand::kPi4)
      .value("sin", Integrand::kSin)
      .value("poly", Integrand::kPoly)
      .value("train", Integrand::kTrainVel)
      .value("table", Integrand::kTable);
  py::enum_<Rule>(m, "Rule").value("left", Rule::kLeft).value("mid", Rule::kMid).value("right", Rule::kRight);
  py::enum_<DType>(m, "DType")
      .value("fp64", DType::kF64)
      .value("fp32", DType::kF32)
      .value("fp32acc", DType::kF32Acc32);
  py::enum_<DivMode>(m, "DivMode")
      .value("series", DivMode::kSeries)
      .value("ieee", DivMode::kIeee)
      .value("series_direct", DivMode::kSeriesDirect)
      .value("series_exact", DivMode::kSeriesExact);

  m.attr("TICKET_WORDS") = kTicketWords;
  m.attr("UNSET_SLOT_WORD") = kUnsetSlotWord;
  m.def("fill_unset_slots", [](uintptr_t p, size_t count, uintptr_t s) {
    fill_unset_slots(ptr<double>(p), count, stream(s));
  });
  m.attr("RIEMANN_TILE") = kRiemannTile;
  m.attr("RIEMANN_BLOCK") = kRiemannBlock;
  m.def("series_ok", &series_ok);
  m.def("series_ok_f32", &series_ok_f32);
  m.def("integrand_scale", &integrand_scale);

  m.def("device_count", &device_count);
  m.def("device_info", [](int d) {
    DeviceInfo i = device_info(d);
    py::dict r;
    r["index"] = i.index;
    r["name"] = i.name;
    r["arch"] = i.arch;
    r["num_cus"] = i.num_cus;
    r["clock_khz"] = i.clock_khz;
    r["total_mem"] = i.total_mem;
    r["l2_bytes"] = i.l2_bytes;
    return r;
  });
  m.def("set_device", &set_device);
  m.def("device_synchronize", []() { MIINT_HIP(hipDeviceSynchronize()); });
  m.def("set_device_flags", [](const std::string& mode) {
    unsigned f = hipDeviceScheduleAuto;
    if (mode == "spin") f = hipDeviceScheduleSpin;
    else if (mode == "yield") f = hipDeviceScheduleYield;
    else if (mode == "blocking") f = hipDeviceScheduleBlockingSync;
    else if (mode != "auto") throw std::invalid_argument("spin|yield|blocking|auto");
    MIINT_HIP(hipSetDeviceFlags(f));
  });
  m.def("get_device_flags", []() {
    unsigned f = 0;
    MIINT_HIP(hipGetDeviceFlags(&f));
    return f;
  });
  m.def("process_start_seconds", &process_start_seconds);
  m.def("enable_tracing", &enable_tracing, py::arg("on"),
        "roctx ranges around runtime phases (MIINT_ROCTX=1)");
  m.def("tracing_enabled", &tracing_enabled);
  m.def("trace_mark", &trace_mark);
  m.def("wait_with_timeout", [](uintptr_t s, double timeout_s) {
    py::gil_scoped_release nogil;
    return wait_with_timeout(stream(s), timeout_s, nullptr);
  });
  m.def("wall_seconds", &wall_seconds);

  py::class_<Comm>(m, "Communicator")
      .def_property_readonly("rank", &Comm::rank)
      .def_property_readonly("world", &Comm::world)
      .def_property_readonly("device", &Comm::device)
      .def_property_readonly("kind", [](const Comm& c) { return std::string(c.kind()); })
      .def_property_readonly("transport_world", &Comm::transport_world,
                             "ranks the transport reports (ncclCommCount for RCCL)")
      .def("allreduce_sum", [](const Comm& c, uintptr_t send, uintptr_t recv, size_t count,
                               uintptr_t s) {
             py::gil_scoped_release nogil;
             c.allreduce_sum(ptr<double>(send), ptr<double>(recv), count, stream(s));
           })
      .def("allgather", [](const Comm& c, uintptr_t send, uintptr_t recv, size_t count,
                           uintptr_t s) {
             py::gil_scoped_release nogil;
             c.allgather(ptr<double>(send), ptr<double>(recv), count, stream(s));
           })
      .def("broadcast", [](const Comm& c, uintptr_t buf, size_t count, int root, uintptr_t s) {
        py::gil_scoped_release nogil;
        c.broadcast(ptr<double>(buf), count, root, stream(s));
      })
      .def("reduce_sum", [](const Comm& c, uintptr_t send, uintptr_t recv, size_t count,
                            int root, uintptr_t s) {
        py::gil_scoped_release nogil;
        c.reduce_sum(ptr<double>(send), ptr<double>(recv), count, root, stream(s));
      })
      .def("check_async", &Comm::check_async);
  py::class_<RcclComm, Comm>(m, "Comm")
      .def(py::init([](py::bytes id, int rank, int world, int device) {
             return new RcclComm(std::string(id), rank, world, device);
           }),
           py::arg("unique_id"), py::arg("rank"), py::arg("world"), py::arg("device"))
      .def_static("unique_id", []() { return py::bytes(RcclComm::unique_id()); })
      .def_static("version", &RcclComm::version);
  py::class_<LoopbackComm, Comm>(m, "LoopbackComm");
  py::class_<LoopbackGroup, std::shared_ptr<LoopbackGroup>>(m, "LoopbackGroup",
      "W logical ranks on one device (test transport; drive rank r from its own thread)")
      .def(py::init(&LoopbackGroup::create), py::arg("world"), py::arg("device") = 0,
           py::arg("timeout_s") = 120.0)
      .def_property_readonly("world", &LoopbackGroup::world)
      .def_property_readonly("device", &LoopbackGroup::device)
      .def("comm", &LoopbackGroup::comm, py::arg("rank"), py::return_value_policy::reference_internal)
      .def("barrier", &LoopbackGroup::barrier, py::arg("rank"), py::call_guard<py::gil_scoped_release>())
      .def("mark_broken", &LoopbackGroup::mark_broken)
      .def_property_readonly("broken", &LoopbackGroup::broken)
      .def_property_readonly("collectives", &LoopbackGroup::collectives)
      .def_property_readonly("graph_launches", &LoopbackGroup::graph_launches);
  m.def(
      "rendezvous_unique_id",
      [](const std::string& addr, int port, int rank, int world, double timeout_s) {
        std::string id;
        {
          py::gil_scoped_release rel;
          id = rendezvous_unique_id(addr, port, rank, world, timeout_s);
        }
        return py::bytes(id);
      },
      py::arg("addr"), py::arg("port"), py::arg("rank"), py::arg("world"),
      py::arg("timeout_s") = 120.0);
  auto transport_dict = [](const RcclTransport& t) {
    py::dict d;
    d["transport"] = t.transport;
    d["nranks"] = t.nranks;
    d["nnodes"] = t.nnodes;
    d["local_ranks"] = t.local_ranks;
    d["connections"] = t.connections;
    d["comms"] = t.comms;
    d["uses_net"] = t.uses_net();
    d["log"] = t.log;
    return d;
  };
  m.def("parse_rccl_log", [transport_dict](const std::string& text) {
    return transport_dict(parse_rccl_log(text));
  });
  m.def("capture_rccl_log", &capture_rccl_log,
        "route RCCL's INIT log into a per-process file (call before the first RCCL call)");
  m.def("rccl_log_path", &rccl_log_path);
  m.def("rccl_transport", [transport_dict]() { return transport_dict(rccl_transport()); });
  m.def(
      "transport_error",
      [](const std::string& log_text, int world, int local_world, bool share) {
        return transport_error(parse_rccl_log(log_text), world, local_world, share);
      },
      "the native CLIs' fail-closed transport verdict on an RCCL INIT log (\"\" = ok)",
      py::arg("log_text"), py::arg("world"), py::arg("local_world"), py::arg("share"));

  py::class_<RiemannConfig>(m, "RiemannConfig")
      .def(py::init<>())
      .def_readwrite("integrand", &RiemannConfig::integrand)
      .def_readwrite("a", &RiemannConfig::a)
      .def_readwrite("b", &RiemannConfig::b)
      .def_readwrite("n", &RiemannConfig::n)
      .def_readwrite("rule", &RiemannConfig::rule)
      .def_readwrite("dtype", &RiemannConfig::dtype)
      .def_readwrite("div", &RiemannConfig::div)
      .def_readwrite("coef", &RiemannConfig::coef)
      .def_readwrite("p0", &RiemannConfig::p0)
      .def_readwrite("p1", &RiemannConfig::p1)
      .def_readwrite("table", &RiemannConfig::table)
      .def_readwrite("grid", &RiemannConfig::grid)
      .def_readwrite("block", &RiemannConfig::block)
      .def_readwrite("waves_per_cu", &RiemannConfig::waves_per_cu)
      .def_readwrite("fused", &RiemannConfig::fused)
      .def_readwrite("slots", &RiemannConfig::slots)
      .def_readwrite("bucket", &RiemannConfig::bucket)
      .def_readwrite("rank", &RiemannConfig::rank)
      .def_readwrite("world", &RiemannConfig::world)
      .def_readwrite("force_collective", &RiemannConfig::force_collective)
      .def_readwrite("step_streams", &RiemannConfig::step_streams)
      .def_readwrite("multistep", &RiemannConfig::multistep)
      .def_readwrite("slice_rank", &RiemannConfig::slice_rank)
      .def_readwrite("slice_world", &RiemannConfig::slice_world)
      .def_readwrite("timeout_s", &RiemannConfig::timeout_s)
      .def_readwrite("host_direct", &RiemannConfig::host_direct)
      .def_readwrite("close", &RiemannConfig::close)
      .def_readwrite("allreduce_to_host", &RiemannConfig::allreduce_to_host)
      .def_readwrite("chain", &RiemannConfig::chain);

  py::class_<RiemannPlan>(m, "RiemannPlan")
      .def(py::init<const RiemannConfig&, int, const Comm*>(), py::arg("config"),
           py::arg("device"), py::arg("comm") = nullptr, py::keep_alive<1, 4>())
      .def_property_readonly("device", &RiemannPlan::device)
      .def_property_readonly("rank", &RiemannPlan::rank)
      .def_property_readonly("world", &RiemannPlan::world)
      .def("step_streams", &RiemannPlan::step_streams, py::arg("nsteps"))
      .def_property_readonly("begin", &RiemannPlan::begin)
      .def_property_readonly("count", &RiemannPlan::count)
      .def_property_readonly("h", &RiemannPlan::h)
      .def_property_readonly("scale", &RiemannPlan::scale)
      .def_property_readonly("grid", [](const RiemannPlan& p) { return p.shape().grid; })
      .def_property_readonly("block", [](const RiemannPlan& p) { return p.shape().block; })
      .def_property_readonly("effective_div", &RiemannPlan::effective_div)
      .def_property_readonly("compute_stream", [](const RiemannPlan& p) { return reinterpret_cast<uintptr_t>(p.compute_stream()); })
      .def_property_readonly("comm_stream", [](const RiemannPlan& p) { return reinterpret_cast<uintptr_t>(p.comm_stream()); })
      .def("run", &RiemannPlan::run, py::call_guard<py::gil_scoped_release>())
      .def("capture_graphs", &RiemannPlan::capture_graphs, py::call_guard<py::gil_scoped_release>())
      .def("prepare_steps", &RiemannPlan::prepare_steps, py::arg("steps"),
           py::call_guard<py::gil_scoped_release>())
      .def_property_readonly("graph_launches", &RiemannPlan::graph_launches)
      .def_property_readonly("direct_steps", &RiemannPlan::direct_steps)
      .def("launch_steps", &RiemannPlan::launch_steps, py::arg("steps"), py::arg("pipeline") = true,
           py::arg("graphs") = true, py::call_guard<py::gil_scoped_release>())
      .def("sync", &RiemannPlan::sync, py::call_guard<py::gil_scoped_release>())
      .def("run_steps", [](RiemannPlan& p, int steps, bool pipeline, bool graphs) {
             StepTiming t;
             {
               py::gil_scoped_release nogil;
               t = p.run_steps(steps, pipeline, graphs);
             }
             py::dict r;
             r["wall_s"] = t.wall_s;
             r["device_ms"] = t.device_ms;
             r["steps"] = t.steps;
             return r;
           }, py::arg("steps"), py::arg("pipeline") = true, py::arg("graphs") = true)
      .def("barrier", &RiemannPlan::barrier, py::call_guard<py::gil_scoped_release>())
      .def("time_one_shot", [](RiemannPlan& p, int reps, const std::string& mode, int warmup) {
             OneShotTiming t;
             {
               py::gil_scoped_release nogil;
               t = p.time_one_shot(reps, mode, warmup);
             }
             py::dict r;
             r["mode"] = t.mode;
             r["reps"] = t.reps;
             r["median_us"] = t.median_us;
             r["min_us"] = t.min_us;
             r["max_us"] = t.max_us;
             r["device_median_us"] = t.device_median_us;
             r["device_min_us"] = t.device_min_us;
             r["value"] = t.value;
             return r;
           }, py::arg("reps"), py::arg("mode") = "direct", py::arg("warmup") = 400)
      .def("diagnose_batch", [](RiemannPlan& p, int steps) {
             BatchDiag d;
             {
               py::gil_scoped_release nogil;
               d = p.diagnose_batch(steps);
             }
             py::dict r;
             r["steps"] = d.steps;
             r["compute_us"] = d.compute_us;
             r["close_us"] = d.close_us;
             r["allreduce_us"] = d.allreduce_us;
             r["copy_us"] = d.copy_us;
             r["tail_us"] = d.tail_us();
             r["boundary_us"] = d.boundary_us();
             r["marker_us"] = d.marker_us;
             r["device_us"] = d.device_us;
             r["staged_us"] = d.staged_us;
             r["wall_us"] = d.wall_us;
             return r;
           }, py::arg("steps"))
      .def("timeline_batch", [](RiemannPlan& p, int steps) {
             BatchTimeline t;
             {
               py::gil_scoped_release nogil;
               t = p.timeline_batch(steps);
             }
             auto arr64 = [](const std::vector<uint64_t>& v, py::ssize_t rows, py::ssize_t cols) {
               py::array_t<uint64_t> a({rows, cols});
               std::copy(v.begin(), v.end(), a.mutable_data());
               return a;
             };
             py::array_t<uint32_t> hw({static_cast<py::ssize_t>(t.grid), py::ssize_t(2)});
             std::copy(t.hw.begin(), t.hw.end(), hw.mutable_data());
             py::dict r;
             r["steps"] = t.steps;
             r["grid"] = t.grid;
             r["block"] = t.block;
             r["clock_khz"] = t.clock_khz;
             r["device_us"] = t.device_us;
             r["stamps"] = arr64(t.stamps, t.grid, t.steps + 2);
             r["shader_clock"] = arr64(t.shader_clock, t.grid, 2);
             r["hw"] = hw;
             r["values"] = t.values;
             return r;
           }, py::arg("steps"))
      .def("host_result", &RiemannPlan::host_result)
      .def_property_readonly("host_capacity", &RiemannPlan::host_capacity)
      .def_property_readonly("slots", &RiemannPlan::slots)
      .def_property_readonly("bucketed", &RiemannPlan::bucketed)
      .def_property_readonly("chained", &RiemannPlan::chained)
      .def_property_readonly("multistep", &RiemannPlan::multistep)
      .def_property_readonly("close_in_launch", &RiemannPlan::close_in_launch)
      .def_property_readonly("allreduce_to_host", &RiemannPlan::allreduce_to_host)
      .def_property_readonly("direct", &RiemannPlan::direct)
      .def_property_readonly("graph_nodes", &RiemannPlan::graph_nodes)
      .def_property_readonly("graphs_ready", &RiemannPlan::graphs_ready)
      .def_property_readonly("graph_error", &RiemannPlan::graph_error)
      .def_property_readonly("collective", &RiemannPlan::collective)
      .def("host_index_of", &RiemannPlan::host_index_of, py::arg("k"), py::arg("graphs"))
      .def("enqueue", [](const RiemannPlan& p, uintptr_t s, int slot, int hidx) { p.enqueue(stream(s), slot, hidx); })
      .def("device_result", [](const RiemannPlan& p, int slot) { return reinterpret_cast<uintptr_t>(p.device_result(slot)); });

  m.def("launch_riemann_partials",
        [](int integrand, double a, double h, double off, uint64_t i_begin, uint64_t n,
           std::vector<double> coef, double p0, double p1, DType dtype, DivMode div, int grid,
           uintptr_t table, int table_n, uintptr_t partials, uintptr_t s) {
          const RiemannParams p = make_params(integrand, a, h, off, i_begin, n, coef, p0, p1);
          launch_riemann_partials(p, dtype, div, {grid, kRiemannBlock}, ptr<const double>(table),
                                  table_n, ptr<double>(partials), stream(s));
        });
  m.def("riemann_tile_len",
        [](int integrand, double a, double h, double off, uint64_t i_begin, uint64_t n,
           std::vector<double> coef, double p0, double p1, DType dtype, DivMode div) {
          return riemann_tile_len(make_params(integrand, a, h, off, i_begin, n, coef, p0, p1),
                                  dtype, div);
        });
  m.def("riemann_effective_div",
        [](int integrand, double a, double h, double off, uint64_t i_begin, uint64_t n,
           std::vector<double> coef, double p0, double p1, DType dtype, DivMode div) {
          return effective_div(make_params(integrand, a, h, off, i_begin, n, coef, p0, p1), div,
                               dtype);
        });
  m.def("riemann_pi4_ieee_narrow",
        [](int integrand, double a, double h, double off, uint64_t i_begin, uint64_t n,
           std::vector<double> coef, double p0, double p1, DType dtype) {
          return pi4_ieee_narrow(make_params(integrand, a, h, off, i_begin, n, coef, p0, p1),
                                 dtype);
        });
  m.attr("TRIG_SERIES_MAX_N") = kTrigSeriesMaxN;
  m.attr("FAST_TRIG_MAX_N") = kFastTrigMaxN;
  m.attr("PI4_SERIES_MAX_X") = kPi4SeriesMaxX;
  m.attr("PI4_F32_SERIES_MAX_X") = kPi4SeriesMaxXF32;
  m.def("launch_riemann_fused",
        [](int integrand, double a, double h, double off, uint64_t i_begin, uint64_t n,
           std::vector<double> coef, double p0, double p1, DType dtype, DivMode div, int grid,
           uintptr_t table, int table_n, uintptr_t partials, uintptr_t ticket, double scale,
           uintptr_t out, uintptr_t s) {
          const RiemannParams p = make_params(integrand, a, h, off, i_begin, n, coef, p0, p1);
          launch_riemann_fused(p, dtype, div, {grid, kRiemannBlock}, ptr<const double>(table),
                               table_n, ptr<double>(partials), ptr<unsigned>(ticket), scale,
                               ptr<double>(out), stream(s));
        });
  m.def("launch_riemann_point_values",
        [](int integrand, double a, double h, double off, uint64_t i_begin, uint64_t n,
           std::vector<double> coef, double p0, double p1, DivMode div, uintptr_t table,
           int table_n, uintptr_t out, uintptr_t s) {
          const RiemannParams p = make_params(integrand, a, h, off, i_begin, n, coef, p0, p1);
          launch_riemann_point_values(p, div, ptr<const double>(table), table_n, ptr<double>(out),
                                      stream(s));
        });
  m.def("launch_pi4_recip_narrow", [](uintptr_t d, uint64_t n, uintptr_t out, uintptr_t s) {
    launch_pi4_recip_narrow(ptr<const double>(d), n, ptr<double>(out), stream(s));
  });
  m.def("launch_pi4_recip_narrow_f32", [](uintptr_t d, uint64_t n, uintptr_t out, uintptr_t s) {
    launch_pi4_recip_narrow_f32(ptr<const float>(d), n, ptr<float>(out), stream(s));
  });
  m.def("set_lds_poison", &set_lds_poison, py::arg("on"),
        "validation: staged-window kernels fill their LDS with NaN first (current device)");
  m.def("set_trig_library", &set_trig_library, py::arg("on"),
        "validation: kIeee sin/cos by ocml per sample (SinLib / TrainVelLib)");
  m.def("fast_trig_host", [](uintptr_t x, uint64_t n, int shift, uintptr_t val, uintptr_t ulp) {
    const double* xs = reinterpret_cast<const double*>(x);
    double* v = reinterpret_cast<double*>(val);
    double* e = reinterpret_cast<double*>(ulp);
    for (uint64_t i = 0; i < n; ++i) {
      double out;
      if (!fast_trig_point(xs[i], shift, out)) {
        v[i] = e[i] = std::nan("");
        continue;
      }
      const long double ref = shift ? cosl(static_cast<long double>(xs[i]))
                                    : sinl(static_cast<long double>(xs[i]));
      const double rd = static_cast<double>(ref);
      const double sp = std::nextafter(std::fabs(rd), INFINITY) - std::fabs(rd);
      v[i] = out;
      e[i] = static_cast<double>((static_cast<long double>(out) - ref) / sp);
    }
  });
  m.def("set_pi4_library_division", &set_pi4_library_division,
        "validation: kIeee Pi4 launches use the full library division (bitwise the same sums)");
  m.def("riemann_block_ok", &riemann_block_ok);
  m.def("launch_finalize", [](uintptr_t partials, int n, double scale, uintptr_t out, uintptr_t s,
                              int block) {
    launch_finalize(ptr<const double>(partials), n, scale, ptr<double>(out), stream(s), block);
  }, py::arg("partials"), py::arg("n"), py::arg("scale"), py::arg("out"), py::arg("stream"),
     py::arg("block") = kRiemannBlock);
  m.def("default_riemann_grid", [](int cus, int waves) { return default_riemann_shape(cus, waves).grid; });
  m.def("default_reduce_grid", &default_reduce_grid);
  m.def("launch_sum_array", [](uintptr_t x, uint64_t n, double scale, uintptr_t partials, int grid,
                               uintptr_t out, uintptr_t s) {
    launch_sum_array(ptr<const double>(x), n, scale, ptr<double>(partials), grid, ptr<double>(out), stream(s));
  });
  m.def("launch_interp_fill", [](uintptr_t table, int tn, double dt, uint64_t i0, uint64_t n,
                                 uintptr_t y, uintptr_t s) {
    launch_interp_fill(ptr<const double>(table), tn, dt, i0, n, ptr<double>(y), stream(s));
  });
  m.def("scan_state_bytes", &scan_state_bytes);
  m.def("launch_inclusive_scan", [](uintptr_t in, uintptr_t out, uint64_t n, uintptr_t state,
                                    uintptr_t carry, uintptr_t s) {
    launch_inclusive_scan(ptr<const double>(in), ptr<double>(out), n, ptr<void>(state),
                          ptr<const double>(carry), stream(s));
  });
  m.def("launch_interp_scan", [](uintptr_t table, int tn, double dt, uint64_t i0, uint64_t n,
                                 uint64_t win_lo, uint64_t win_hi, uintptr_t out, uintptr_t state,
                                 uintptr_t carry, uintptr_t s) {
    launch_interp_scan_window(ptr<const double>(table), tn, dt, i0, n, win_lo, win_hi,
                              ptr<double>(out), ptr<void>(state), ptr<const double>(carry), stream(s));
  });
  m.def("scan_timeout_flag", [](uintptr_t state, uintptr_t s) { return scan_timeout_flag(ptr<const void>(state), stream(s)); });
  m.def("launch_add_carry", [](uintptr_t x, uint64_t n, uintptr_t carry, uintptr_t s) {
    launch_add_carry(ptr<double>(x), n, ptr<const double>(carry), stream(s));
  });
  m.def("table2d_grid", [](int nx, int ny, double X, double Y, int gx, int gy, int row0, int row1) {
    Table2DParams p{nullptr, nx, ny, X, Y, gx, gy, row0, row1};
    return table2d_grid(p);
  });
  m.def("table2d_path", [](int nx, int ny, double X, double Y, int gx, int gy, int row0, int row1) {
    Table2DParams p{nullptr, nx, ny, X, Y, gx, gy, row0, row1};
    return std::string(table2d_path(p));
  });
  m.def("table2d_shape_info", [](int nx, int ny, double X, double Y, int gx, int gy, int row0,
                                 int row1, int min_wg) {
    Table2DParams p{nullptr, nx, ny, X, Y, gx, gy, row0, row1, min_wg};
    const Table2DShapeInfo i = table2d_shape_info(p);
    py::dict d;
    d["stream"] = i.stream;
    d["rows_per_wave"] = i.rows_per_wave;
    d["tile_rows"] = i.tile_rows;
    d["tile_cols"] = i.tile_cols;
    d["grid"] = py::make_tuple(i.grid_x, i.grid_y);
    d["tile"] = i.tile;
    return d;
  }, py::arg("nx"), py::arg("ny"), py::arg("X"), py::arg("Y"), py::arg("gx"), py::arg("gy"),
     py::arg("row0"), py::arg("row1"), py::arg("min_wg") = 0);
  m.def("launch_table2d_partials", [](uintptr_t table, int nx, int ny, double X, double Y, int gx,
                                      int gy, int row0, int row1, uintptr_t partials, uintptr_t s) {
    Table2DParams p{ptr<const double>(table), nx, ny, X, Y, gx, gy, row0, row1};
    launch_table2d_partials(p, ptr<double>(partials), stream(s));
  });
  m.def("launch_table2d_fused", [](uintptr_t table, int nx, int ny, double X, double Y, int gx,
                                    int gy, int row0, int row1, uintptr_t partials,
                                    uintptr_t ticket, uintptr_t out, uintptr_t s) {
    Table2DParams p{ptr<const double>(table), nx, ny, X, Y, gx, gy, row0, row1};
    launch_table2d_fused(p, ptr<double>(partials), ptr<unsigned>(ticket), ptr<double>(out),
                         stream(s));
  });
  m.def("launch_table2d_chained", [](uintptr_t table, int nx, int ny, double X, double Y, int gx,
                                      int gy, int row0, int row1, uintptr_t partials,
                                      uintptr_t prev, uintptr_t prev_out, uintptr_t s) {
    Table2DParams p{ptr<const double>(table), nx, ny, X, Y, gx, gy, row0, row1};
    launch_table2d_chained(p, ptr<double>(partials), ptr<const double>(prev),
                           ptr<double>(prev_out), stream(s));
  });
  m.def("table2d_multistep_phases", [](int nx, int ny, double X, double Y, int gx, int gy,
                                       int row0, int row1, int min_wg, int steps, int want) {
    Table2DParams p{nullptr, nx, ny, X, Y, gx, gy, row0, row1, min_wg};
    return table2d_multistep_phases(p, 0, steps, want);
  }, py::arg("nx"), py::arg("ny"), py::arg("X"), py::arg("Y"), py::arg("gx"), py::arg("gy"),
     py::arg("row0"), py::arg("row1"), py::arg("min_wg"), py::arg("steps"), py::arg("want") = 0);
  m.def("launch_table2d_multistep", [](uintptr_t table, int nx, int ny, double X, double Y,
                                        int gx, int gy, int row0, int row1, int min_wg,
                                        uintptr_t partials, int steps, uintptr_t outs,
                                        uintptr_t s, int phases) {
    Table2DParams p{ptr<const double>(table), nx, ny, X, Y, gx, gy, row0, row1, min_wg};
    launch_table2d_multistep(p, ptr<double>(partials), steps, ptr<double>(outs), stream(s),
                             phases);
  }, py::arg("table"), py::arg("nx"), py::arg("ny"), py::arg("X"), py::arg("Y"), py::arg("gx"),
     py::arg("gy"), py::arg("row0"), py::arg("row1"), py::arg("min_wg"), py::arg("partials"),
     py::arg("steps"), py::arg("outs"), py::arg("stream"), py::arg("phases") = 1);
  m.def("launch_table2d_finalize", [](uintptr_t partials, int n, uintptr_t out, uintptr_t s) {
    launch_table2d_finalize(ptr<const double>(partials), n, ptr<double>(out), stream(s));
  });
  m.def("launch_outer_product", [](uintptr_t v, int n, uintptr_t t, uintptr_t s) {
    launch_outer_product(ptr<const double>(v), n, ptr<double>(t), stream(s));
  });
  m.def("selftest_wave_ops", [](uintptr_t in, uint64_t n, bool f32, uintptr_t sums, uintptr_t scan, uintptr_t s) {
    selftest_wave_ops(ptr<const void>(in), n, f32, ptr<void>(sums), ptr<void>(scan), stream(s));
  });
  m.def("selftest_block_ops", [](uintptr_t in, uint64_t n, int block, bool f32, uintptr_t sums,
                                 uintptr_t scan, uintptr_t s) {
    selftest_block_ops(ptr<const void>(in), n, block, f32, ptr<void>(sums), ptr<void>(scan), stream(s));
  });

  py::class_<TrainScanConfig>(m, "TrainScanConfig")
      .def(py::init<>())
      .def_readwrite("steps_per_sec", &TrainScanConfig::steps_per_sec)
      .def_readwrite("seconds", &TrainScanConfig::seconds)
      .def_readwrite("parity", &TrainScanConfig::parity)
      .def_readwrite("replicate", &TrainScanConfig::replicate)
      .def_readwrite("phase2", &TrainScanConfig::phase2)
      .def_readwrite("table", &TrainScanConfig::table)
      .def_property("algo", [](const TrainScanConfig& c) { return scan_algo_name(c.algo); },
                    [](TrainScanConfig& c, const std::string& s) {
                      c.algo = scan_algo_of(s);
                    });
  m.def("trainscan_workspace_bytes", &trainscan_workspace_bytes);
  m.def("replica_digest", [](const std::vector<double>& v) {
    const ReplicaDigest d = digest_table(v.data(), v.size());
    py::dict r;
    r["hash"] = d.hash;
    r["n"] = d.n;
    r["sum"] = d.sum;
    r["at"] = std::vector<double>(d.at, d.at + 5);
    return r;
  });

  py::class_<Table2DPlan>(m, "Table2DPlan")
      .def(py::init([](int grid, double extent, int device, const Comm* comm, bool bucket,
                       bool chain, int step_streams, int slice_rank, int slice_world,
                       bool multistep, int phases, int min_wg, int graph_steps,
                       bool force_collective) {
             Table2DConfig c;
             c.force_collective = force_collective;
             c.graph_steps = graph_steps;
             c.phases = phases;
             c.min_wg = min_wg;
             c.grid = grid;
             c.extent = extent;
             c.bucket = bucket;
             c.chain = chain;
             c.step_streams = step_streams;
             c.multistep = multistep;
             c.rank = slice_rank;
             c.world = slice_world;
             return new Table2DPlan(c, device, comm);
           }),
           py::arg("grid") = 4096, py::arg("extent") = 1800.0, py::arg("device") = 0,
           py::arg("comm") = nullptr, py::arg("bucket") = true, py::arg("chain") = true,
           py::arg("step_streams") = 0, py::arg("slice_rank") = 0, py::arg("slice_world") = 1,
           py::arg("multistep") = true, py::arg("phases") = 0, py::arg("min_wg") = 0,
           py::arg("graph_steps") = 0, py::arg("force_collective") = false,
           py::keep_alive<1, 5>())
      .def_property_readonly("phases", &Table2DPlan::phases)
      .def_property_readonly("min_wg", &Table2DPlan::min_wg)
      .def_property_readonly("workgroups", &Table2DPlan::workgroups)
      .def_property_readonly("resident_per_cu", &Table2DPlan::resident_per_cu)
      .def_property_readonly("step_streams",
                             [](const Table2DPlan& p) { return p.step_streams(); })
      .def_property_readonly("multistep", &Table2DPlan::multistep)
      .def("run", &Table2DPlan::run, py::call_guard<py::gil_scoped_release>())
      .def("time", &Table2DPlan::time, py::arg("iters"), py::arg("graphs") = true,
           py::call_guard<py::gil_scoped_release>())
      .def("last_result", &Table2DPlan::last_result)
      .def_property_readonly("bucketed", &Table2DPlan::bucketed)
      .def_property_readonly("chained", &Table2DPlan::chained)
      .def_property_readonly("collective", &Table2DPlan::collective)
      .def_property_readonly("graph_steps", &Table2DPlan::graph_steps)
      .def_property_readonly("row0", &Table2DPlan::row0)
      .def_property_readonly("row1", &Table2DPlan::row1);
  m.def("table2d_oracle", &table2d_oracle, py::arg("grid"), py::arg("extent") = 1800.0);
  m.def("table2d_auto_graph_steps", &table2d_auto_graph_steps, py::arg("grid"),
        py::arg("extent") = 1800.0, py::arg("world") = 1);
  m.def("launch_trainscan", [](uintptr_t table, int tn, double dt, uint64_t i0, uint64_t n,
                               uint64_t win_lo, uint64_t win_hi, uintptr_t ws, uintptr_t totals,
                               uintptr_t carries, uintptr_t vel, uintptr_t pos, uintptr_t s,
                               bool fold) {
    TrainScanKernelParams p{ptr<const double>(table), tn, dt, i0, n, win_lo, win_hi};
    launch_trainscan_local(p, ptr<void>(ws), ptr<double>(totals), stream(s), fold);
    launch_trainscan_write(p, ptr<const void>(ws), ptr<const double>(carries), ptr<double>(vel),
                           ptr<double>(pos), stream(s), fold);
  }, py::arg("table"), py::arg("table_n"), py::arg("dt"), py::arg("i0"), py::arg("n"),
     py::arg("win_lo"), py::arg("win_hi"), py::arg("ws"), py::arg("totals"), py::arg("carries"),
     py::arg("vel"), py::arg("pos"), py::arg("stream"), py::arg("fold") = false);
  m.def("trainscan_fold_applies", [](double dt, uint64_t n) {
    TrainScanKernelParams p{nullptr, 2, dt, 0, n, 0, ~uint64_t(0)};
    return trainscan_fold_applies(p);
  }, "does launch_trainscan(fold = true) take the fold variant for this dt and slice length?");
  m.def("launch_trainscan_onepass", [](uintptr_t table, int tn, double dt, uint64_t i0,
                                       uint64_t n, uint64_t win_lo, uint64_t win_hi, uintptr_t ws,
                                       uintptr_t totals, uintptr_t vel, uintptr_t pos,
                                       uintptr_t s) {
    TrainScanKernelParams p{ptr<const double>(table), tn, dt, i0, n, win_lo, win_hi};
    launch_trainscan_onepass(p, ptr<void>(ws), ptr<double>(vel), ptr<double>(pos),
                             ptr<double>(totals), stream(s));
  });
  m.def("trainscan_onepass_timeout", [](uintptr_t ws, uintptr_t s) {
    return trainscan_onepass_timeout(ptr<const void>(ws), stream(s));
  });
  py::class_<TrainScan>(m, "TrainScan")
      .def(py::init<const TrainScanConfig&, int, const Comm*>(), py::arg("config"),
           py::arg("device"), py::arg("comm") = nullptr, py::keep_alive<1, 4>())
      .def("run", [](TrainScan& t) {
        TrainScanResult r;
        {
          py::gil_scoped_release nogil;
          r = t.run();
        }
        py::dict d;
        d["distance"] = r.distance;
        d["sum_of_sums"] = r.sum_of_sums;
        d["distance_scan"] = r.distance_scan;
        d["device_ms"] = r.device_ms;
        d["timeout"] = r.timeout;
        return d;
      })
      .def_property_readonly("local_begin", &TrainScan::local_begin)
      .def_property_readonly("algo", [](const TrainScan& t) { return scan_algo_name(t.algo()); })
      .def_property_readonly("local_count", &TrainScan::local_count)
      .def("velocity_ptr", [](const TrainScan& t) { return reinterpret_cast<uintptr_t>(t.velocity()); })
      .def("position_ptr", [](const TrainScan& t) { return reinterpret_cast<uintptr_t>(t.position()); })
      .def("replicated_ptr", [](const TrainScan& t) { return reinterpret_cast<uintptr_t>(t.replicated()); })
      .def_property_readonly("total", &TrainScan::total);

  m.def("expr_source", &expr_source, "kernel source generated for an expression over x");
  m.def("expr_compile", [](const std::string& e) {
          std::string code;
          {
            py::gil_scoped_release nogil;
            code = expr_compile(e);
          }
          return py::bytes(code);
        },
        "compile an expression for gfx950 with hipRTC (no device needed); the code object");
  py::class_<ExprIntegrator>(m, "ExprIntegrator",
                             "f(x) given as an expression, compiled with hipRTC for gfx950")
      .def(py::init<const std::string&, int, int>(), py::arg("expr"), py::arg("device") = 0,
           py::arg("grid") = 2048)
      .def("integrate", &ExprIntegrator::integrate, py::arg("a"), py::arg("b"), py::arg("n"),
           py::arg("rule"), py::arg("begin"), py::arg("count"), py::arg("scale") = 1.0,
           py::arg("comm") = nullptr, py::call_guard<py::gil_scoped_release>())
      .def("time",
           [](ExprIntegrator& e, double a, double b, uint64_t n, Rule rule, uint64_t begin,
              uint64_t count, int iters) { return e.time(a, b, n, rule, begin, count, iters); },
           py::arg("a"), py::arg("b"), py::arg("n"), py::arg("rule"), py::arg("begin"),
           py::arg("count"), py::arg("iters"), py::call_guard<py::gil_scoped_release>())
      .def_property_readonly("expression", &ExprIntegrator::expression);

  m.def("expr_sweep_source", &expr_sweep_source, py::arg("expr"), py::arg("nparams"),
        "kernel source generated for an expression over x and p0..p{nparams-1}");
  m.def("expr_sweep_compile", [](const std::string& e, int nparams) {
// ... 192 lines not shown
```

### csrc/runtime/integrator.cpp

```cpp
#include "miint/integrator.hpp"

#include <algorithm>
#include <atomic>
#include <cstring>
#include <limits>
#include <string>
#include <vector>

#include "miint/fault.hpp"
#include "miint/trace.hpp"

namespace miint {

namespace {
constexpr int kHostRing = 4096;
}

RiemannPlan::RiemannPlan(const RiemannConfig& cfg, int device, const Comm* comm)
    : cfg_(cfg), device_(device), comm_(comm), compute_((set_device(device), Stream())),
      comm_stream_(), ev_fork_(false), ev_join_(false) {
  MIINT_CHECK(cfg.n >= 1, "n must be >= 1");
  MIINT_CHECK(cfg.b != cfg.a, "empty interval");
  MIINT_CHECK(cfg.slots >= 1 && cfg.slots <= 64, "slots must be in [1, 64]");
  if (comm) {
    rank_ = comm->rank();
    world_ = comm->world();
    MIINT_CHECK(comm->device() == device, "communicator bound to another device");
  } else {
    MIINT_CHECK(cfg.world >= 1 && cfg.rank >= 0 && cfg.rank < cfg.world, "bad rank/world");
    rank_ = cfg.rank;
    world_ = cfg.world;
  }
  direct_ = cfg.host_direct && !(comm_ && (world_ > 1 || cfg.force_collective));
  DeviceGuard g(device);
  params_.a = cfg.a;
  params_.h = (cfg.b - cfg.a) / static_cast<double>(cfg.n);
  params_.off = rule_offset(cfg.rule);
  if (cfg.slice_world > 0) {
    MIINT_CHECK(cfg.slice_rank >= 0 && cfg.slice_rank < cfg.slice_world, "bad slice rank");
    rank_slice(cfg.n, cfg.slice_rank, cfg.slice_world, &params_.i_begin, &params_.n);
  } else {
    rank_slice(cfg.n, rank_, world_, &params_.i_begin, &params_.n);
  }
  params_.integrand = static_cast<int>(cfg.integrand);
  params_.ncoef = static_cast<int>(cfg.coef.size());
  MIINT_CHECK(cfg.coef.size() <= static_cast<size_t>(kMaxPolyCoeffs), "too many coefficients");
  for (size_t i = 0; i < cfg.coef.size(); ++i) params_.coef[i] = cfg.coef[i];
  params_.p0 = cfg.p0;
  params_.p1 = cfg.p1;
  scale_ = params_.h * integrand_scale(cfg.integrand);

  const DeviceInfo info = device_info(device);
  MIINT_CHECK(riemann_block_ok(cfg.block),
              "block must be 64, 128, 256, 512 or 1024 threads (got " + std::to_string(cfg.block) +
                  ")");
  const uint64_t bs = static_cast<uint64_t>(cfg.block);
  shape_ = default_riemann_shape(info.num_cus, cfg.waves_per_cu, cfg.block);
  if (cfg.grid > 0) shape_.grid = cfg.grid;
  const uint64_t tl = static_cast<uint64_t>(riemann_tile_len(params_, cfg.dtype, cfg.div));
  const uint64_t tiles = (params_.n + tl - 1) / tl;
  const uint64_t need = std::max<uint64_t>(1, (tiles + bs - 1) / bs);
  shape_.grid = static_cast<int>(std::min<uint64_t>(static_cast<uint64_t>(shape_.grid), need));
  if (cfg.grid <= 0) {
    const uint64_t cus = static_cast<uint64_t>(info.num_cus);
    const uint64_t four =
        std::max<uint64_t>(cus, (tiles + 4 * bs - 1) / (4 * bs));
    uint64_t g = std::min<uint64_t>(static_cast<uint64_t>(shape_.grid), four);
    if (g > cus) g -= g % cus;
    shape_.grid = static_cast<int>(g);
  }
  MIINT_CHECK(cfg.close == "auto" || cfg.close == "kernel" || cfg.close == "launch",
              "close must be auto, kernel or launch (got " + cfg.close + ")");
  if (cfg.multistep && chained()) {
    const int res_kernel =
        riemann_multistep_grid(params_, cfg.dtype, cfg.div, cfg.block, info.num_cus, false);
    close_launch_ = cfg.close == "launch";
    const int res_close =
        close_launch_
            ? riemann_multistep_grid(params_, cfg.dtype, cfg.div, cfg.block, info.num_cus, true)
            : 0;
    if (res_close == 0) close_launch_ = false;
    const int resident = close_launch_ ? res_close : res_kernel;
    if (resident > 0 && cfg.grid <= 0 && shape_.grid > resident) shape_.grid = resident;
    multistep_ = resident > 0 && shape_.grid <= resident;
    if (!multistep_) close_launch_ = false;
  }

  const int lanes = step_streams(cfg.slots);
  partials_ = DeviceBuffer<double>(2 * static_cast<size_t>(std::max(1, lanes)) *
                                   static_cast<size_t>(shape_.grid));
  for (int l = 1; l < lanes; ++l) {
    step_streams_.emplace_back();
    ev_step_join_.emplace_back(new Event(false));
  }
  slots_ = DeviceBuffer<double>(static_cast<size_t>(shape_.grid));
  fill_unset_slots(slots_.get(), slots_.size(), nullptr);
  if (multistep_)
    ms_partials_ = DeviceBuffer<double>(static_cast<size_t>(cfg.slots) * shape_.grid);
  if (close_launch_) {
    ms_ticket_ = DeviceBuffer<unsigned int>(kTicketWords);
    MIINT_HIP(hipMemset(ms_ticket_.get(), 0, ms_ticket_.bytes()));
  }
  result_ = DeviceBuffer<double>(static_cast<size_t>(cfg.slots));
  sync_ = DeviceBuffer<double>(1);
  MIINT_HIP(hipMemset(sync_.get(), 0, sync_.bytes()));
  ticket_ = DeviceBuffer<unsigned int>(kTicketWords);
  MIINT_HIP(hipMemset(ticket_.get(), 0, ticket_.bytes()));
  MIINT_HIP(hipMemset(result_.get(), 0, result_.bytes()));
  if (cfg.integrand == Integrand::kTable) {
    MIINT_CHECK(cfg.table.size() >= 2, "table integrand needs a table");
    table_ = DeviceBuffer<double>(cfg.table.size());
    MIINT_HIP(hipMemcpy(table_.get(), cfg.table.data(), table_.bytes(), hipMemcpyHostToDevice));
  }
  host_ = PinnedBuffer<double>(static_cast<size_t>(std::max(kHostRing, cfg.slots)));
  for (int i = 0; i < cfg.slots; ++i) {
    ev_computed_.emplace_back(new Event(false));
    ev_drained_.emplace_back(new Event(false));
  }
  MIINT_HIP(hipDeviceSynchronize());
}

RiemannPlan::~RiemannPlan() {
  (void)hipSetDevice(device_);
  (void)hipStreamSynchronize(compute_.get());
  (void)hipStreamSynchronize(comm_stream_.get());
  for (const auto& s : step_streams_) (void)hipStreamSynchronize(s.get());
}

DivMode RiemannPlan::effective_div() const {
  return miint::effective_div(params_, cfg_.div, cfg_.dtype);
}

size_t RiemannPlan::graph_nodes() const {
  size_t n = 0;
  for (const auto& kv : graphs_) n = std::max(n, kv.second->num_nodes());
  return n;
}

void RiemannPlan::enqueue_compute(hipStream_t s, int slot, int host_index) const {
  double* out = direct_ ? host_.device_ptr() + host_index : result_.get() + slot;
  const int tn = static_cast<int>(cfg_.table.size());
  if (cfg_.fused) {
    launch_riemann_fused(params_, cfg_.dtype, cfg_.div, shape_, table_.get(), tn,
                         slots_.get(), ticket_.get(), scale_, out, s);
  } else {
    launch_riemann_partials(params_, cfg_.dtype, cfg_.div, shape_, table_.get(), tn,
                            partials_.get(), s);
    launch_finalize(partials_.get(), shape_.grid, scale_, out, s, shape_.block);
  }
}

void RiemannPlan::enqueue_reduce(hipStream_t s, int slot) const {
  if (collective()) {
    double* v = result_.get() + slot;
    comm_->allreduce_sum(v, v, 1, s);
  }
}

void RiemannPlan::enqueue_copyout(hipStream_t s, int slot, int host_index) const {
  if (direct_) return;
  MIINT_HIP(hipMemcpyAsync(host_.get() + host_index, result_.get() + slot, sizeof(double),
                           hipMemcpyDeviceToHost, s));
}

void RiemannPlan::enqueue(hipStream_t s, int slot, int host_index) const {
  enqueue_compute(s, slot, host_index);
  enqueue_reduce(s, slot);
  enqueue_copyout(s, slot, host_index);
}

double RiemannPlan::run() {
  DeviceGuard g(device_);
  enqueue(compute_.get(), 0, 0);
  compute_.sync();
  return host_[0];
}

void RiemannPlan::enqueue_chain(hipStream_t s, int nsteps) const {
  const int g = shape_.grid;
  const int tn = static_cast<int>(cfg_.table.size());
  for (int j = 0; j < nsteps; ++j) {
    double* cur = partials_.get() + static_cast<size_t>(j & 1) * g;
    const double* prev = j ? partials_.get() + static_cast<size_t>((j - 1) & 1) * g : nullptr;
    launch_riemann_chained(params_, cfg_.dtype, cfg_.div, shape_, table_.get(), tn, cur, prev, g,
                           scale_, j ? result_ptr(j - 1) : nullptr, s);
  }
  launch_finalize(partials_.get() + static_cast<size_t>((nsteps - 1) & 1) * g, g, scale_,
                  result_ptr(nsteps - 1), s, shape_.block);
}

int RiemannPlan::step_streams(int nsteps) const {
  if (!chained() || multistep_) return 1;
  const int want = cfg_.step_streams > 0            ? cfg_.step_streams
                   : params_.n >= kStepStreamsMaxCount ? 1
                                                       : kAutoStepStreams;
  return std::max(1, std::min(want, nsteps));
}

void RiemannPlan::enqueue_chain_streams(hipStream_t cs, int nsteps) {
  const int L = std::min(step_streams(nsteps), 1 + static_cast<int>(step_streams_.size()));
  if (L <= 1) {
    enqueue_chain(cs, nsteps);
    return;
  }
  const int g = shape_.grid;
  const int tn = static_cast<int>(cfg_.table.size());
  auto lane = [&](int l) { return l == 0 ? cs : step_streams_[static_cast<size_t>(l - 1)].get(); };
  auto half = [&](int l, int jj) {
    return partials_.get() + (2 * static_cast<size_t>(l) + static_cast<size_t>(jj & 1)) * g;
  };
  ev_fork_.record(cs);
  for (int l = 1; l < L; ++l) MIINT_HIP(hipStreamWaitEvent(lane(l), ev_fork_.get(), 0));
  for (int j = 0; j < nsteps; ++j) {
    const int l = j % L, jj = j / L;
    launch_riemann_chained(params_, cfg_.dtype, cfg_.div, shape_, table_.get(), tn, half(l, jj),
                           jj ? half(l, jj - 1) : nullptr, g, scale_,
                           jj ? result_ptr(j - L) : nullptr, lane(l));
  }
  for (int l = 0; l < L && l < nsteps; ++l) {
    const int last = l + ((nsteps - 1 - l) / L) * L;
    launch_finalize(half(l, last / L), g, scale_, result_ptr(last), lane(l), shape_.block);
    if (l > 0) {
      ev_step_join_[static_cast<size_t>(l - 1)]->record(lane(l));
      MIINT_HIP(hipStreamWaitEvent(cs, ev_step_join_[static_cast<size_t>(l - 1)]->get(), 0));
    }
  }
}

void RiemannPlan::enqueue_bucket_reduce(hipStream_t s, int nsteps) const {
  const size_t n = static_cast<size_t>(nsteps);
  if (allreduce_to_host() && !capturing_) {
    comm_->allreduce_sum(result_.get(), host_.device_ptr(), n, s);
    return;
  }
  comm_->allreduce_sum(result_.get(), result_.get(), n, s);
  MIINT_HIP(hipMemcpyAsync(host_.get(), result_.get(), sizeof(double) * n,
                           hipMemcpyDeviceToHost, s));
}

void RiemannPlan::check_allreduce_to_host() {
  if (ar_host_checked_ || !bucketed() || !cfg_.allreduce_to_host) return;
  ar_host_checked_ = true;
  DeviceGuard g(device_);
  hipStream_t s = compute_.get();
  const double want = 0.5 * static_cast<double>(world_) * (static_cast<double>(world_) + 1.0);
  const size_t probe = host_.size() - 1;
  host_[probe] = std::numeric_limits<double>::quiet_NaN();
  host_[0] = static_cast<double>(rank_) + 1.0;
  MIINT_HIP(hipMemcpyAsync(result_.get(), host_.get(), sizeof(double), hipMemcpyHostToDevice, s));
  bool ok = true;
  try {
    comm_->allreduce_sum(result_.get(), host_.device_ptr() + probe, 1, s);
    if (cfg_.timeout_s > 0) wait_with_timeout(s, cfg_.timeout_s, comm_);
    else compute_.sync();
    ok = host_[probe] == want && !fault::allreduce_to_host_fails(rank_);
  } catch (const Error&) {
    ok = false;
    (void)hipGetLastError();
    compute_.sync();
  }
  host_[0] = ok ? 0.0 : 1.0;
  MIINT_HIP(hipMemcpyAsync(sync_.get(), host_.get(), sizeof(double), hipMemcpyHostToDevice, s));
  comm_->allreduce_sum(sync_.get(), sync_.get(), 1, s);
  MIINT_HIP(hipMemcpyAsync(host_.get(), sync_.get(), sizeof(double), hipMemcpyDeviceToHost, s));
  MIINT_HIP(hipMemsetAsync(sync_.get(), 0, sizeof(double), s));
  if (cfg_.timeout_s > 0) wait_with_timeout(s, cfg_.timeout_s, comm_);
  else compute_.sync();
  ar_host_ok_ = host_[0] == 0.0;
}

void RiemannPlan::enqueue_batch(hipStream_t cs, hipStream_t rs, int nsteps, bool overlap) {
  if (chained()) {
    if (nsteps == 1)
      launch_riemann_fused(params_, cfg_.dtype, cfg_.div, shape_, table_.get(),
                           static_cast<int>(cfg_.table.size()), slots_.get(), ticket_.get(),
                           scale_, result_ptr(0), cs);
    else if (multistep_)
      launch_riemann_multistep(params_, cfg_.dtype, cfg_.div, shape_, table_.get(),
                               static_cast<int>(cfg_.table.size()), ms_partials_.get(), nsteps,
                               scale_, result_ptr(0), cs,
                               close_launch_ ? ms_ticket_.get() : nullptr);
    else
      enqueue_chain_streams(cs, nsteps);
    if (bucketed()) {
      enqueue_bucket_reduce(cs, nsteps);
      return;
    }
    if (!direct_)
      MIINT_HIP(hipMemcpyAsync(host_.get(), result_.get(), sizeof(double) * nsteps,
                               hipMemcpyDeviceToHost, cs));
    return;
  }
  if (bucketed()) {
    for (int j = 0; j < nsteps; ++j) enqueue_compute(cs, j, j);
    enqueue_bucket_reduce(cs, nsteps);
    return;
  }
  if (!overlap || direct_ || !collective()) {
    for (int j = 0; j < nsteps; ++j) enqueue(cs, j, j);
    return;
  }
  ev_fork_.record(cs);
  MIINT_HIP(hipStreamWaitEvent(rs, ev_fork_.get(), 0));
  for (int j = 0; j < nsteps; ++j) {
    enqueue_compute(cs, j, j);
    ev_computed_[j]->record(cs);
    MIINT_HIP(hipStreamWaitEvent(rs, ev_computed_[j]->get(), 0));
    enqueue_reduce(rs, j);
    enqueue_copyout(rs, j, j);
  }
  ev_join_.record(rs);
  MIINT_HIP(hipStreamWaitEvent(cs, ev_join_.get(), 0));
}

void RiemannPlan::capture_graphs() { batch_graph(cfg_.slots); }

const Graph* RiemannPlan::batch_graph(int nsteps) {
  auto it = graphs_.find(nsteps);
  if (it != graphs_.end()) return it->second.get();
  if (!graph_error_.empty()) return nullptr;
  DeviceGuard g(device_);
  TraceRange tr("miint.plan.capture_graphs");
  if (collective() && graphs_.empty()) {
    comm_->allreduce_sum(result_.get(), result_.get(), 1, compute_.get());
    MIINT_HIP(hipStreamSynchronize(compute_.get()));
  }
  std::unique_ptr<Graph> gr(new Graph());
  const bool one = collective() && comm_->capture_single_stream();
  try {
    capturing_ = true;
    capture_with(collective() ? comm_ : nullptr, *gr, compute_.get(), [&](hipStream_t s) {
      enqueue_batch(s, one ? s : comm_stream_.get(), nsteps, !one);
    });
    capturing_ = false;
  } catch (const Error& e) {
    capturing_ = false;
    graph_error_ = e.what();
    (void)hipGetLastError();
    (void)hipStreamSynchronize(compute_.get());
    (void)hipStreamSynchronize(comm_stream_.get());
    if (collective() && std::string(comm_->kind()) == "loopback") throw;
    return nullptr;
  }
  return (graphs_[nsteps] = std::move(gr)).get();
}

void RiemannPlan::prepare_steps(int steps) {
  const int S = cfg_.slots;
  if (steps >= S) batch_graph(S);
  if (steps % S) batch_graph(steps % S);
}

bool RiemannPlan::use_graphs(bool requested, int steps) {
  if (!requested) return false;
  const int S = cfg_.slots;
  if (steps >= S && !batch_graph(S)) return false;
  if (steps % S && !batch_graph(steps % S)) return false;
  return true;
}

int RiemannPlan::host_index_of(int k, bool graphs) const {
  const bool batched = last_mode_ < 0 ? ((graphs && graphs_ready()) || bucketed() || multistep())
                                       : last_mode_ == 1;
  return batched ? k % cfg_.slots : k % host_capacity();
}

void RiemannPlan::launch_steps(int steps, bool pipeline, bool graphs) {
  DeviceGuard g(device_);
  TraceRange tr("miint.plan.launch_steps");
  check_allreduce_to_host();
  hipStream_t cs = compute_.get();
  hipStream_t rs = comm_stream_.get();
  const int S = cfg_.slots;
  const Comm* gc = collective() ? comm_ : nullptr;
  if (use_graphs(graphs, steps)) {
    last_mode_ = 1;
    if (steps >= S) {
      const Graph* full = batch_graph(S);
      for (int b = 0; b < steps / S; ++b) launch_with(gc, *full, cs);
      graph_launches_ += steps / S;
    }
    if (steps % S) {
      launch_with(gc, *batch_graph(steps % S), cs);
      ++graph_launches_;
    }
    return;
  }
  direct_steps_ += steps;
  last_mode_ = (bucketed() || multistep()) ? 1 : 0;
  if (bucketed() || multistep()) {
    for (int k = 0; k < steps; k += S) enqueue_batch(cs, rs, std::min(S, steps - k), false);
    return;
  }
  const bool overlap = pipeline && !direct_ && collective();
  for (int k = 0; k < steps; ++k) {
    const int slot = k % S;
    const int hidx = k % host_capacity();
    if (!overlap) {
      enqueue(cs, slot, hidx);
      continue;
    }
    if (k >= S) MIINT_HIP(hipStreamWaitEvent(cs, ev_drained_[slot]->get(), 0));
    enqueue_compute(cs, slot, hidx);
    ev_computed_[slot]->record(cs);
    MIINT_HIP(hipStreamWaitEvent(rs, ev_computed_[slot]->get(), 0));
    enqueue_reduce(rs, slot);
    enqueue_copyout(rs, slot, hidx);
    ev_drained_[slot]->record(rs);
  }
  if (overlap) {
    ev_join_.record(rs);
    MIINT_HIP(hipStreamWaitEvent(cs, ev_join_.get(), 0));
  }
}

void RiemannPlan::sync() const {
  DeviceGuard g(device_);
  TraceRange tr("miint.plan.sync");
  if (collective() && cfg_.timeout_s > 0) {
    wait_with_timeout(comm_stream_.get(), cfg_.timeout_s, comm_);
    wait_with_timeout(compute_.get(), cfg_.timeout_s, comm_);
    return;
  }
  compute_.sync();
  comm_stream_.sync();
}

void RiemannPlan::barrier() {
  if (!collective()) return;
  DeviceGuard g(device_);
  comm_->allreduce_sum(sync_.get(), sync_.get(), 1, compute_.get());
  if (cfg_.timeout_s > 0) wait_with_timeout(compute_.get(), cfg_.timeout_s, comm_);
  else compute_.sync();
}

StepTiming RiemannPlan::run_steps(int steps, bool pipeline, bool graphs) {
  DeviceGuard g(device_);
  check_allreduce_to_host();
  use_graphs(graphs, steps);
  StepTiming t;
  sync();
  barrier();
  const double w0 = wall_seconds();
  ev_t0_.record(compute_.get());
  launch_steps(steps, pipeline, graphs);
  fault::delay(rank_);
  ev_t1_.record(compute_.get());
  sync();
  t.wall_s = wall_seconds() - w0;
  t.device_ms = Event::elapsed_ms(ev_t0_, ev_t1_);
  t.steps = steps;
  return t;
}

BatchDiag RiemannPlan::diagnose_batch(int nsteps) {
  MIINT_CHECK(nsteps >= 1 && nsteps <= cfg_.slots, "diagnose_batch: 1 <= steps <= slots");
  DeviceGuard g(device_);
  TraceRange tr("miint.plan.diagnose_batch");
  check_allreduce_to_host();
  hipStream_t cs = compute_.get();
  const int tn = static_cast<int>(cfg_.table.size());
  BatchDiag d;
  d.steps = nsteps;
  {
    Event a0, a1;
    sync();
    barrier();
    const double w0 = wall_seconds();
    a0.record(cs);
    enqueue_batch(cs, comm_stream_.get(), nsteps, false);
    a1.record(cs);
    sync();
    d.wall_us = (wall_seconds() - w0) * 1e6;
    d.device_us = Event::elapsed_ms(a0, a1) * 1e3;
  }
  Event e0, e1, e2, e3, e4;
  sync();
  barrier();
  e0.record(cs);
  if (chained() && nsteps > 1 && multistep_) {
    launch_riemann_multistep(params_, cfg_.dtype, cfg_.div, shape_, table_.get(), tn,
                             ms_partials_.get(), nsteps, scale_, result_ptr(0), cs,
                             close_launch_ ? ms_ticket_.get() : nullptr, false);
    e1.record(cs);
    if (!close_launch_)
      launch_multistep_close(ms_partials_.get(), shape_.grid, nsteps, scale_, result_ptr(0),
                             shape_.block, cs);
  } else if (chained() && nsteps > 1) {
    enqueue_chain_streams(cs, nsteps);
    e1.record(cs);
  } else {
    for (int j = 0; j < nsteps; ++j) enqueue_compute(cs, j, j);
    e1.record(cs);
  }
  e2.record(cs);
  if (bucketed()) {
    const size_t n = static_cast<size_t>(nsteps);
    if (allreduce_to_host()) {
      comm_->allreduce_sum(result_.get(), host_.device_ptr(), n, cs);
      e3.record(cs);
    } else {
      comm_->allreduce_sum(result_.get(), result_.get(), n, cs);
      e3.record(cs);
      MIINT_HIP(hipMemcpyAsync(host_.get(), result_.get(), sizeof(double) * n,
                               hipMemcpyDeviceToHost, cs));
    }
  } else {
    for (int j = 0; j < nsteps; ++j) enqueue_reduce(cs, j);
    e3.record(cs);
    for (int j = 0; j < nsteps; ++j) enqueue_copyout(cs, j, j);
  }
  e4.record(cs);
  sync();
  last_mode_ = 1;
  d.staged_us = Event::elapsed_ms(e0, e4) * 1e3;
  {
    Event m[9];
    for (Event& e : m) e.record(cs);
    MIINT_HIP(hipStreamSynchronize(cs));
    std::vector<double> gaps;
    for (int i = 1; i < 9; ++i) gaps.push_back(Event::elapsed_ms(m[i - 1], m[i]) * 1e3);
    std::nth_element(gaps.begin(), gaps.begin() + 4, gaps.end());
    d.marker_us = gaps[4];
  }
  const double m = d.marker_us;
  d.compute_us = Event::elapsed_ms(e0, e1) * 1e3 - m;
  d.close_us = std::max(0.0, Event::elapsed_ms(e1, e2) * 1e3 - m);
  d.allreduce_us = std::max(0.0, Event::elapsed_ms(e2, e3) * 1e3 - m);
  d.copy_us = std::max(0.0, Event::elapsed_ms(e3, e4) * 1e3 - m);
  return d;
}

BatchTimeline RiemannPlan::timeline_batch(int nsteps) {
  MIINT_CHECK(nsteps >= 1 && nsteps <= cfg_.slots, "timeline_batch: 1 <= steps <= slots");
  MIINT_CHECK(multistep(), "timeline_batch: not a multi-step plan (its batches run chained or "
                           "fused launches: there is no persistent launch to time)");
  MIINT_CHECK(!close_launch_, std::string("timeline_batch: ") + kTimelineNoCloseInLaunch);
  DeviceGuard g(device_);
  TraceRange tr("miint.plan.timeline_batch");
  const DeviceInfo info = device_info(device_);
  const int resident =
      riemann_timeline_grid(params_, cfg_.dtype, cfg_.div, shape_.block, info.num_cus);
  MIINT_CHECK(shape_.grid <= resident,
              "timeline_batch: the timeline kernel holds " + std::to_string(resident) +
                  " workgroups of " + std::to_string(shape_.block) + " threads at once, the plan "
                  "launches " + std::to_string(shape_.grid) + " (a second round of workgroups "
                  "would be another launch's timeline)");
  BatchTimeline t;
  t.steps = nsteps;
  t.grid = shape_.grid;
  t.block = shape_.block;
  MIINT_HIP(hipDeviceGetAttribute(&t.clock_khz, hipDeviceAttributeWallClockRate, device_));
  MIINT_CHECK(t.clock_khz > 0, "timeline_batch: the device reports no wall clock rate");
  const size_t grid = static_cast<size_t>(shape_.grid);
  if (tl_stamps_.size() == 0) {
    tl_stamps_ = DeviceBuffer<uint64_t>(grid * static_cast<size_t>(cfg_.slots + 2));
    tl_shader_ = DeviceBuffer<uint64_t>(grid * 2);
    tl_hw_ = DeviceBuffer<uint32_t>(grid * 2);
  }
  check_allreduce_to_host();
  hipStream_t cs = compute_.get();
  const size_t nstamp = grid * static_cast<size_t>(nsteps + 2);
  sync();
  barrier();
  MIINT_HIP(hipMemsetAsync(tl_stamps_.get(), 0, tl_stamps_.bytes(), cs));
  MIINT_HIP(hipMemsetAsync(tl_shader_.get(), 0, tl_shader_.bytes(), cs));
  MIINT_HIP(hipMemsetAsync(tl_hw_.get(), 0xff, tl_hw_.bytes(), cs));
  Event a0, a1;
  a0.record(cs);
  launch_riemann_timeline(params_, cfg_.dtype, cfg_.div, shape_, table_.get(),
                          static_cast<int>(cfg_.table.size()), ms_partials_.get(), nsteps, scale_,
                          result_ptr(0), cs, tl_stamps_.get(), tl_shader_.get(), tl_hw_.get());
  a1.record(cs);
  if (bucketed())
    enqueue_bucket_reduce(cs, nsteps);
  else if (!direct_)
    MIINT_HIP(hipMemcpyAsync(host_.get(), result_.get(), sizeof(double) * nsteps,
                             hipMemcpyDeviceToHost, cs));
  t.stamps.resize(nstamp);
  t.shader_clock.resize(grid * 2);
  t.hw.resize(grid * 2);
  MIINT_HIP(hipMemcpyAsync(t.stamps.data(), tl_stamps_.get(), nstamp * sizeof(uint64_t),
                           hipMemcpyDeviceToHost, cs));
  MIINT_HIP(hipMemcpyAsync(t.shader_clock.data(), tl_shader_.get(), tl_shader_.bytes(),
                           hipMemcpyDeviceToHost, cs));
  MIINT_HIP(hipMemcpyAsync(t.hw.data(), tl_hw_.get(), tl_hw_.bytes(), hipMemcpyDeviceToHost, cs));
  sync();
  last_mode_ = 1;
  t.device_us = Event::elapsed_ms(a0, a1) * 1e3;
  t.values.resize(static_cast<size_t>(nsteps));
  for (int j = 0; j < nsteps; ++j) t.values[static_cast<size_t>(j)] = host_[j];
  return t;
}

OneShotTiming RiemannPlan::time_one_shot(int reps, const std::string& mode, int warmup) {
  MIINT_CHECK(reps >= 1 && warmup >= 0, "time_one_shot: reps >= 1");
  MIINT_CHECK(!collective(), "time_one_shot: single-rank plans only");
  const bool graph = mode == "graph" || mode == "graph_poll";
  const bool poll = mode == "direct_poll" || mode == "graph_poll";
  MIINT_CHECK(graph || poll || mode == "direct",
              "time_one_shot mode: direct|direct_poll|graph|graph_poll");
  MIINT_CHECK(!poll || direct_, "a polled one-shot needs the result stored straight into pinned "
                                "memory (single GPU, host_direct)");
  DeviceGuard g(device_);
  hipStream_t cs = compute_.get();
  const Graph* g1 = graph ? batch_graph(1) : nullptr;
  MIINT_CHECK(!graph || g1, "time_one_shot: 1-step graph capture failed: " + graph_error_);
  volatile uint64_t* word = reinterpret_cast<volatile uint64_t*>(host_.get());
  constexpr uint64_t kSentinel = 0x7ff8dead5eed0001ull;
  std::vector<double> host_us, dev_us;
  double first = 0.0;
  for (int i = 0; i < warmup + 2 * reps; ++i) {
    const bool events = i >= warmup && (i - warmup) % 2 == 1;
    MIINT_HIP(hipStreamSynchronize(cs));
    *word = kSentinel;
    std::atomic_thread_fence(std::memory_order_seq_cst);
    const double t0 = wall_seconds();
    if (events) ev_t0_.record(cs);
    if (graph) g1->launch(cs);
    else enqueue(cs, 0, 0);
    if (events) ev_t1_.record(cs);
    if (poll) {
      const double limit = cfg_.timeout_s > 0 ? cfg_.timeout_s : 60.0;
      for (uint32_t spin = 1; *word == kSentinel; ++spin) {
        if ((spin & 1023u) != 0) continue;
        const double waited = wall_seconds() - t0;
        if (waited < 0.05) continue;
        const hipError_t q = hipStreamQuery(cs);
        if (q != hipErrorNotReady && *word == kSentinel) {
          MIINT_HIP(q);
          throw Error("time_one_shot: the stream finished but the result word was never stored");
        }
        if (waited > limit)
          throw Error("time_one_shot: no result after " + std::to_string(limit) + " s (" + mode + ")");
      }
    } else {
      MIINT_HIP(hipStreamSynchronize(cs));
    }
    const double t1 = wall_seconds();
    MIINT_HIP(hipStreamSynchronize(cs));
    uint64_t bits = *word;
    double v;
    std::memcpy(&v, &bits, sizeof(v));
    if (!direct_) v = host_[0];
    if (i == 0) first = v;
    MIINT_CHECK(std::memcmp(&v, &first, sizeof(v)) == 0,
                "time_one_shot: calls disagree (" + std::to_string(v) + " vs " +
                    std::to_string(first) + ")");
    if (i < warmup) continue;
    if (events) dev_us.push_back(static_cast<double>(Event::elapsed_ms(ev_t0_, ev_t1_)) * 1e3);
    else host_us.push_back((t1 - t0) * 1e6);
  }
  last_mode_ = graph ? 1 : 0;
  auto med = [](std::vector<double> v) {
    std::sort(v.begin(), v.end());
    const size_t n = v.size();
    return n % 2 ? v[n / 2] : 0.5 * (v[n / 2 - 1] + v[n / 2]);
  };
  OneShotTiming r;
  r.mode = mode;
  r.reps = reps;
  r.median_us = med(host_us);
  r.min_us = *std::min_element(host_us.begin(), host_us.end());
  r.max_us = *std::max_element(host_us.begin(), host_us.end());
  r.device_median_us = med(dev_us);
  r.device_min_us = *std::min_element(dev_us.begin(), dev_us.end());
  r.value = first;
  return r;
}

}
```

### cuda_v_mpi_amd/integrate.py

```python
from __future__ import annotations

import dataclasses
import math
import time

import torch

from .models import integrands
from .parallel import decomposition
from .parallel.dist import DistContext, native_comm


@dataclasses.dataclass
class IntegrationResult:
    value: float
    analytic: float
    n: int
    integrand: str
    rule: str
    dtype: str
    gpus: int
    seconds_wall: float
    seconds_device: float

    @property
    def abs_err(self) -> float:
        return abs(self.value - self.analytic)

    @property
    def rel_err(self) -> float:
        return self.abs_err / abs(self.analytic) if self.analytic else float("nan")

    @property
    def subintervals_per_s(self) -> float:
        t = self.seconds_device if self.seconds_device > 0 else self.seconds_wall
        return self.n / t if t > 0 else float("nan")

    def as_dict(self) -> dict:
        d = dataclasses.asdict(self)
        d.update(abs_err=self.abs_err, rel_err=self.rel_err,
                 subintervals_per_s=self.subintervals_per_s)
        return d


class Integrator:
    def __init__(self, integrand: str | integrands.IntegrandSpec = "pi4", n: int = 10**9,
                 rule: str = "left", dtype: str = "fp64", div: str = "series_exact",
                 backend: str = "hip", ctx: DistContext | None = None, comm: str = "native",
                 fused: bool = True, grid: int = 0, slots: int = 16, a: float | None = None,
                 b: float | None = None, force_collective: bool = False, bucket: bool = True,
                 chain: bool = True, comm_obj=None, threads: int = 0,
                 slice_of: tuple[int, int] | None = None, step_streams: int = 0,
                 block: int = 256, multistep: bool = True, close: str = "auto",
                 allreduce_to_host: bool = True, timeout_s: float = 300.0, **spec_kw):
        spec = integrands.get(integrand, **spec_kw) if isinstance(integrand, str) else integrand
        if a is not None or b is not None:
            spec = dataclasses.replace(spec, a=spec.a if a is None else a,
                                       b=spec.b if b is None else b)
        if n < 1:
            raise ValueError("n must be >= 1")
        if rule not in ("left", "mid", "right"):
            raise ValueError("rule must be left|mid|right")
        if dtype not in ("fp64", "fp32", "fp32acc"):
            raise ValueError("dtype must be fp64|fp32|fp32acc")
        self.spec, self.n, self.rule, self.dtype, self.div = spec, int(n), rule, dtype, div
        self.backend, self.comm_kind = backend, comm
        if comm_obj is not None:
            ctx = DistContext(rank=comm_obj.rank, world=comm_obj.world, device=comm_obj.device,
                              backend=comm_obj.kind)
        self.ctx = ctx or DistContext()
        self.begin, self.count = decomposition.rank_slice(self.n, self.ctx.rank, self.ctx.world)
        self._plan = None
        self._comm = None
        self._pool = None
        if backend in ("hip", "host"):
            from ._native import native

            m = native()
            if backend == "hip" and m.device_count() < 1:
                raise RuntimeError("backend='hip' needs a HIP device; use backend='host' or "
                                   "'cpu' explicitly")
            cfg = m.RiemannConfig()
            cfg.integrand = getattr(m.Integrand, spec.name)
            cfg.a, cfg.b, cfg.n = spec.a, spec.b, self.n
            cfg.rule = getattr(m.Rule, rule)
            cfg.dtype = getattr(m.DType, dtype)
            cfg.div = getattr(m.DivMode, div)
            cfg.coef = list(spec.coef)
            cfg.p0, cfg.p1 = spec.p0, spec.p1
            cfg.table = spec.native_table()
            cfg.grid, cfg.fused, cfg.slots = grid, fused, slots
            cfg.block = block
            cfg.force_collective = force_collective
            cfg.bucket = bucket
            cfg.chain = chain
            cfg.step_streams = step_streams
            cfg.multistep = multistep
            cfg.close = close
            cfg.allreduce_to_host = allreduce_to_host
            cfg.timeout_s = timeout_s
            if slice_of is not None:
                cfg.slice_rank, cfg.slice_world = int(slice_of[0]), int(slice_of[1])
            self._m = m
            if backend == "host":
                self._cfg = cfg
                self._pool = m.HostPool(threads)
                return
            if comm_obj is not None:
                self._comm = comm_obj
                self._plan = m.RiemannPlan(cfg, comm_obj.device, comm_obj)
            elif (self.ctx.world > 1 or force_collective) and comm == "native":
                self._comm = native_comm(self.ctx)
                self._plan = m.RiemannPlan(cfg, self.ctx.device, self._comm)
            else:
                cfg.rank, cfg.world = self.ctx.rank, self.ctx.world
                self._plan = m.RiemannPlan(cfg, self.ctx.device)
        elif backend != "cpu":
            raise ValueError("backend must be 'hip', 'host' or 'cpu'")

    @property
    def plan(self):
        return self._plan

    @property
    def h(self) -> float:
        return (self.spec.b - self.spec.a) / self.n

    def describe(self) -> dict:
        d = dict(integrand=self.spec.name, n=self.n, rule=self.rule, dtype=self.dtype,
                 backend=self.backend, rank=self.ctx.rank, world=self.ctx.world,
                 begin=self.begin, count=self.count)
        if self._plan is not None:
            d.update(grid=self._plan.grid, block=self._plan.block,
                     div=str(self._plan.effective_div).split(".")[-1])
        return d

    def _torch_reduce(self, value: float) -> float:
        dev = "cuda" if self.ctx.backend == "nccl" else "cpu"
        t = torch.tensor([value], dtype=torch.float64, device=dev)
        self.ctx.all_reduce_sum(t)
        return float(t.item())

    def _cpu_local(self) -> float:
        spec, h = self.spec, self.h
        off = {"left": 0.0, "mid": 0.5, "right": 1.0}[self.rule]
        dt = torch.float64 if self.dtype == "fp64" else torch.float32
        chunk = 1 << 22
        parts = []
        for s in range(self.begin, self.begin + self.count, chunk):
            i = torch.arange(s, min(self.begin + self.count, s + chunk), dtype=torch.float64)
            x = (spec.a + (i + off) * h).to(dt)
            parts.append(float(spec.f_torch(x).to(torch.float64).sum()))
        return math.fsum(parts) * h

    def run(self) -> IntegrationResult:
        t0 = time.perf_counter()
        dev_s = 0.0
        if self.backend == "cpu":
            value = self._torch_reduce(self._cpu_local()) if self.ctx.world > 1 else self._cpu_local()
        elif self.backend == "host":
            t = time.perf_counter()
            value = self._m.host_riemann(self._cfg, self.begin, self.count, self._pool)
            dev_s = time.perf_counter() - t
            if self.ctx.world > 1:
                value = self._torch_reduce(value)
        else:
            if self._comm is not None or self.ctx.world == 1:
                t = self._plan.run_steps(1, pipeline=False, graphs=False)
                value = self._plan.host_result(0)
                dev_s = t["device_ms"] * 1e-3
            else:
                t = self._plan.run_steps(1, pipeline=False, graphs=False)
                value = self._torch_reduce(self._plan.host_result(0))
                dev_s = t["device_ms"] * 1e-3
        wall = time.perf_counter() - t0
        return IntegrationResult(value=value, analytic=self.spec.analytic(), n=self.n,
                                 integrand=self.spec.name, rule=self.rule, dtype=self.dtype,
                                 gpus=self.ctx.world, seconds_wall=wall, seconds_device=dev_s)

    def run_steps(self, steps: int, pipeline: bool = True, graphs: bool = True) -> dict:
        if self._plan is None:
            raise RuntimeError("run_steps needs backend='hip'")
        return self._plan.run_steps(steps, pipeline, graphs)

    def launch_steps(self, steps: int, pipeline: bool = True, graphs: bool = True) -> None:
        if self._plan is None:
            raise RuntimeError("launch_steps needs backend='hip'")
        self._plan.launch_steps(steps, pipeline, graphs)

    def sync(self) -> None:
        if self._plan is not None:
            self._plan.sync()

    def timeline(self, steps: int) -> dict:
        if self._plan is None:
            raise RuntimeError("timeline needs backend='hip'")
        t = self._plan.timeline_batch(steps)
        t["xcc"] = t["hw"][:, 0] & 0xF
        return t


def integrate(integrand: str = "pi4", n: int = 10**9, **kw) -> IntegrationResult:
    return Integrator(integrand, n=n, **kw).run()


def integrate_expr(expr: str, a: float, b: float, n: int = 10**9, rule: str = "left",
                   backend: str = "hip", ctx: DistContext | None = None, threads: int = 0,
                   analytic: float | None = None) -> IntegrationResult:
    from ._native import native

    if rule not in ("left", "mid", "right"):
        raise ValueError("rule must be left|mid|right")
    m = native()
    ctx = ctx or DistContext()
    begin, count = decomposition.rank_slice(int(n), ctx.rank, ctx.world)
    rl = getattr(m.Rule, rule)
    t0 = time.perf_counter()
    if backend == "hip":
        value = m.ExprIntegrator(expr, ctx.device).integrate(float(a), float(b), int(n), rl,
                                                              begin, count)
    elif backend == "host":
        value = m.HostExpr(expr).integrate(float(a), float(b), int(n), rl, begin, count,
                                           m.HostPool(threads))
    else:
        raise ValueError("integrate_expr backend must be 'hip' or 'host'")
    dev_s = time.perf_counter() - t0
    if ctx.world > 1:
        dev = "cuda" if ctx.backend == "nccl" else "cpu"
        t = torch.tensor([value], dtype=torch.float64, device=dev)
        ctx.all_reduce_sum(t)
        value = float(t.item())
    return IntegrationResult(value=value, analytic=float("nan") if analytic is None else analytic,
                             n=int(n), integrand=f"expr:{expr}", rule=rule, dtype="fp64",
                             gpus=ctx.world, seconds_wall=time.perf_counter() - t0,
                             seconds_device=dev_s)


@dataclasses.dataclass
class SweepResult:
    values: list
    abs_err: list | None
    rows: int
    nparams: int
    n: int
    expr: str
    rule: str
    seconds: float

    @property
    def subintervals_per_s(self) -> float:
        return self.rows * self.n / self.seconds if self.seconds > 0 else float("nan")

    def as_dict(self) -> dict:
        d = dataclasses.asdict(self)
        d.update(subintervals_per_s=self.subintervals_per_s)
        return d


def integrate_expr_sweep(expr: str, params, a: float, b: float, n: int = 10**6,
                         rule: str = "left", backend: str = "hip", threads: int = 0,
                         analytic=None) -> SweepResult:
    from ._native import native
    from .ops.kernels import _param_rows

    if rule not in ("left", "mid", "right"):
        raise ValueError("rule must be left|mid|right")
    m = native()
    p = _param_rows(params)
    if backend == "hip":
        from .ops import kernels

        m.expr_sweep_compile(expr, int(p.shape[1]))
        t0 = time.perf_counter()
        values = kernels.riemann_expr_sweep(expr, p, float(a), float(b), int(n), rule=rule)
        values = [float(v) for v in values.cpu()]
    elif backend == "host":
        hs, pool = m.HostExprSweep(expr, p.shape[1]), m.HostPool(threads)
        t0 = time.perf_counter()
        values = [float(v) for v in hs.integrate(p, float(a), float(b), int(n),
                                                 getattr(m.Rule, rule), 0, int(n), pool)]
    else:
        raise ValueError("integrate_expr_sweep backend must be 'hip' or 'host'")
    secs = time.perf_counter() - t0
    err = None
    if analytic is not None:
        want = [float(w) for w in analytic]
        if len(want) != len(values):
            raise ValueError(f"analytic has {len(want)} values for {len(values)} rows")
        err = [abs(v - w) for v, w in zip(values, want)]
    return SweepResult(values=values, abs_err=err, rows=len(values), nparams=int(p.shape[1]),
                       n=int(n), expr=expr, rule=rule, seconds=secs)
```

Measured before the change: 31530 billion.

## Add atomic work-queue scheduling for the persistent multi-step Riemann kernel

```diff
diff --git a/csrc/cli/miint.cpp b/csrc/cli/miint.cpp
--- a/csrc/cli/miint.cpp
+++ b/csrc/cli/miint.cpp
@@ -22,6 +22,9 @@
   bool multistep = false, close_in_launch = false, allreduce_to_host = false;
   BatchDiag diag;
   std::string timeline_file;
+  std::string timeline_work;
+  std::string work = "static";
+  int queue_workgroups = 0;
   cli::RankFacts facts;
   cli::Topology topo;
 };
@@ -77,8 +80,18 @@
   std::fputs("\"values\":[", f);
   for (size_t i = 0; i < t.values.size(); ++i)
     std::fprintf(f, i ? ",%.17g" : "%.17g", t.values[i]);
-  std::fputs("],\n\"stamps\":", f);
-  write_rows(f, t.stamps, static_cast<size_t>(t.steps) + 2);
+  std::fprintf(f, "],\n\"work\":\"%s\"", t.work.c_str());
+  if (t.work == "queue") {
+    std::fprintf(f, ",\"workgroups\":%d,\n\"wg_stamps\":", t.workgroups);
+    write_rows(f, t.wg_stamps, 2);
+    std::fputs(",\n\"item_stamp\":", f);
+    write_rows(f, t.item_stamp, static_cast<size_t>(t.grid));
+    std::fputs(",\n\"item_owner\":", f);
+    write_rows(f, t.item_owner, static_cast<size_t>(t.grid));
+  } else {
+    std::fputs(",\n\"stamps\":", f);
+    write_rows(f, t.stamps, static_cast<size_t>(t.steps) + 2);
+  }
   std::fputs(",\n\"shader_clock\":", f);
   write_rows(f, t.shader_clock, 2);
   std::fputs(",\n\"hw\":", f);
@@ -112,8 +125,11 @@
     const double ms = agree.max(t.wall_s * 1e3 / iters);
     BatchDiag d;
     if (diagnose) d = plan.diagnose_batch(std::min(iters, plan.config().slots));
+    std::string tl_work;
     if (!timeline.file.empty()) {
-      const BatchTimeline tl = plan.timeline_batch(std::min(iters, plan.config().slots));
+      const BatchTimeline tl =
+          plan.timeline_batch(std::min(iters, plan.config().slots), plan.work());
+      tl_work = tl.work;
       if (rank == 0)
         write_timeline(timeline.file, tl, cfg, timeline.integrand, timeline.dtype, timeline.div,
                        d.steps == tl.steps ? d.device_us : 0.0);
@@ -127,9 +143,12 @@
       row.grid = plan.shape().grid;
       row.multistep = plan.multistep();
       row.close_in_launch = plan.close_in_launch();
+      row.work = plan.work();
+      row.queue_workgroups = plan.queue_workgroups();
       row.allreduce_to_host = plan.allreduce_to_host();
       row.diag = d;
       row.timeline_file = timeline.file;
+      row.timeline_work = tl_work;
     }
   });
   return row;
@@ -144,6 +163,8 @@
                    .add("grid", r.grid)
                    .add("multistep", r.multistep)
                    .add("close_in_launch", r.close_in_launch)
+                   .add("work", r.work)
+                   .add("queue_workgroups", r.queue_workgroups)
                    .add("allreduce_to_host", r.allreduce_to_host)
                    .add("ms_per_integration", r.ms)
                    .add("subintervals_per_s", r.n / (r.ms * 1e-3))
@@ -161,7 +182,8 @@
         .add("diag_device_us", r.diag.device_us)
         .add("diag_marker_us", r.diag.marker_us)
         .add("diag_host_us", r.diag.wall_us - r.diag.device_us);
-  if (!r.timeline_file.empty()) rec.add("timeline_file", r.timeline_file);
+  if (!r.timeline_file.empty())
+    rec.add("timeline_file", r.timeline_file).add("timeline_work", r.timeline_work);
   cli::emit(a, rec, true);
 }
 
@@ -283,6 +305,7 @@
     "                   [--iters 200] [--gpus G] [--div series_exact|series|ieee] [--unfused] [--no-graph]\n"
     "                   [--block B] [--grid G] [--step-streams S] [--trig-library] [--settle N]\n"
     "                   [--no-multistep] [--slots K] [--close auto|kernel|launch] [--no-ar-host]\n"
+    "                   [--work auto|static|queue] [--queue-wg-per-cu W]\n"
     "                   [--diagnose] [--slice R/W] [--timeline FILE]\n"
     "                   (--timeline: after the timed run, one batch from the timeline build of\n"
     "                   the multi-step launch, per-workgroup device-clock stamps as JSON in FILE;\n"
@@ -330,6 +353,8 @@
       c.multistep = !a.flag("no-multistep");
       c.slots = static_cast<int>(a.integer("slots", c.slots));
       c.close = a.str("close", c.close);
+      c.work = a.str("work", c.work);
+      c.queue_wg_per_cu = static_cast<int>(a.integer("queue-wg-per-cu", 0));
       c.allreduce_to_host = !a.flag("no-ar-host");
       cli::parse_slice(a, &c.slice_rank, &c.slice_world);
       TimelineRequest tl;
diff --git a/csrc/include/miint/integrator.hpp b/csrc/include/miint/integrator.hpp
--- a/csrc/include/miint/integrator.hpp
+++ b/csrc/include/miint/integrator.hpp
@@ -40,11 +40,27 @@
   bool force_collective = false;
   bool multistep = true;
   std::string close = "auto";
+  std::string work = "auto";
+  int queue_wg_per_cu = 0;
   bool allreduce_to_host = true;
   int step_streams = 0;
   int slice_rank = 0, slice_world = 0;
   double timeout_s = 300.0;
 };
+
+inline std::string resolve_work(const std::string& work, const char* env, bool pays,
+                                bool keeps_static = false) {
+  MIINT_CHECK(work == "auto" || work == "static" || work == "queue",
+              "work must be auto, static or queue (got " + work + ")");
+  if (keeps_static) return "static";
+  if (work != "auto") return work;
+  if (env && *env) {
+    const std::string e(env);
+    MIINT_CHECK(e == "static" || e == "queue", "MIINT_MS_WORK must be static or queue (got " + e + ")");
+    return e;
+  }
+  return pays ? "queue" : "static";
+}
 
 inline void rank_slice(uint64_t n, int r, int w, uint64_t* begin, uint64_t* count) {
   const uint64_t q = n / static_cast<uint64_t>(w), rem = n % static_cast<uint64_t>(w);
@@ -89,6 +105,11 @@
   std::vector<uint32_t> hw;
   double device_us = 0.0;
   std::vector<double> values;
+  std::string work = "static";
+  int workgroups = 0;
+  std::vector<uint64_t> wg_stamps;
+  std::vector<uint64_t> item_stamp;
+  std::vector<uint32_t> item_owner;
 };
 constexpr uint64_t kTimelineUnsetStamp = 0;
 constexpr uint32_t kTimelineUnsetId = 0xffffffffu;
@@ -133,7 +154,7 @@
 
   StepTiming run_steps(int steps, bool pipeline, bool graphs);
   BatchDiag diagnose_batch(int nsteps);
-  BatchTimeline timeline_batch(int nsteps);
+  BatchTimeline timeline_batch(int nsteps, const std::string& form = "auto");
   void barrier();
   OneShotTiming time_one_shot(int reps, const std::string& mode, int warmup = 400);
   void launch_steps(int steps, bool pipeline, bool graphs);
@@ -147,6 +168,8 @@
   bool chained() const { return cfg_.fused && cfg_.chain && (!collective() || bucketed()); }
   bool multistep() const { return chained() && multistep_; }
   bool close_in_launch() const { return multistep() && close_launch_; }
+  const char* work() const { return multistep() && work_queue_ ? "queue" : "static"; }
+  int queue_workgroups() const { return multistep() && work_queue_ ? queue_wgs_ : 0; }
   bool allreduce_to_host() const {
     return bucketed() && cfg_.allreduce_to_host && ar_host_ok_;
   }
@@ -181,6 +204,13 @@
   bool ar_host_ok_ = true;
   bool ar_host_checked_ = false;
   DeviceBuffer<unsigned int> ms_ticket_;
+  bool work_queue_ = false;
+  int queue_wgs_ = 0;
+  DeviceBuffer<unsigned int> queue_;
+  void reset_queue() const;
+  void enqueue_multistep(hipStream_t s, int nsteps, bool close_kernel) const;
+  DeviceBuffer<uint64_t> qtl_item_stamp_, qtl_wg_stamps_, qtl_shader_;
+  DeviceBuffer<uint32_t> qtl_item_owner_, qtl_hw_;
   DeviceBuffer<uint64_t> tl_stamps_, tl_shader_;
   DeviceBuffer<uint32_t> tl_hw_;
   DeviceBuffer<double> result_;
diff --git a/csrc/include/miint/kernels.hpp b/csrc/include/miint/kernels.hpp
--- a/csrc/include/miint/kernels.hpp
+++ b/csrc/include/miint/kernels.hpp
@@ -131,6 +131,22 @@
                              hipStream_t stream, uint64_t* stamps, uint64_t* shader_clock,
                              uint32_t* hw, unsigned int* ticket = nullptr,
                              bool close_kernel = true);
+constexpr int kQueueWords = 2 * kTicketStride;
+struct QueueTimeline {
+  uint64_t* item_stamp;
+  uint32_t* item_owner;
+  uint64_t* wg_stamps;
+  uint64_t* shader_clock;
+  uint32_t* hw;
+};
+int riemann_queue_grid(const RiemannParams& p, DType dtype, DivMode div, int block, int num_cus,
+                       bool timeline = false);
+bool riemann_queue_pays(const RiemannParams& p, DType dtype, DivMode div);
+void launch_riemann_queue(const RiemannParams& p, DType dtype, DivMode div, LaunchShape shape,
+                          int workgroups, const double* table, int table_n, double* partials,
+                          int steps, double scale, double* out, hipStream_t stream,
+                          unsigned int* queue, bool close_kernel = true,
+                          const QueueTimeline* timeline = nullptr);
 void launch_multistep_close(const double* partials, int grid, int steps, double scale,
                             double* out, int block, hipStream_t stream);
 
diff --git a/csrc/kernels/riemann.hip b/csrc/kernels/riemann.hip
--- a/csrc/kernels/riemann.hip
+++ b/csrc/kernels/riemann.hip
@@ -738,6 +738,128 @@
   return !(M == DivMode::kIeee && (__is_same(F, Pi4) || __is_same(F, Pi4Wide)));
 }
 
+struct QueueTimelineOut {
+  unsigned long long* item_stamp;
+  unsigned* item_owner;
+  unsigned long long* wg_stamps;
+  unsigned long long* shader_clock;
+  unsigned* hw;
+};
+template <int T>
+__device__ __forceinline__ TileSplit tile_split(uint64_t n, unsigned nb) {
+  const uint32_t bs = blockDim.x;
+  const uint64_t lanes = static_cast<uint64_t>(nb) * bs;
+  const uint64_t ntile = n / T;
+  const uint64_t q = ntile / lanes;
+  return {lanes, q, bs, static_cast<uint32_t>(ntile - q * lanes)};
+}
+__device__ __forceinline__ unsigned queue_claim(unsigned* head) {
+  unsigned zero = 0;
+  asm volatile("" : "+v"(zero));
+  return __hip_atomic_fetch_add(head + zero, 1u, __ATOMIC_RELAXED, __HIP_MEMORY_SCOPE_AGENT);
+}
+template <DivMode M, class F, bool TL = false>
+__device__ __forceinline__ void queue_body(const RiemannParams& p, const double* table,
+                                           int table_n, double* partials, int steps, unsigned nb,
+                                           unsigned* queue, QueueTimelineOut tl = {}) {
+  using Acc = typename AccOf<F>::type;
+  TimelineEntry te{};
+  if constexpr (TL) te = timeline_entry();
+  __shared__ double red[2][kMaxBlock / kWave];
+  __shared__ Acc red_acc[2][__is_same(Acc, double) ? 1 : kMaxBlock / kWave];
+  __shared__ unsigned next_item[2];
+  __shared__ double lds[lds_words<M, F>()];
+  const F f = make_functor<M, F>(p, table, table_n, lds);
+  const TileSplit sp = tile_split<F::template tile_len<M>()>(p.n, nb);
+  const unsigned total = static_cast<unsigned>(steps) * nb;
+  const bool one_wave = blockDim.x == kWave;
+  unsigned* head = queue;
+  unsigned* done = queue + kTicketStride;
+  unsigned c = 0;
+  if (threadIdx.x == 0) c = queue_claim(head);
+  if (!one_wave) {
+    if (threadIdx.x == 0) next_item[1] = c;
+    __syncthreads();
+    c = next_item[1];
+  }
+  unsigned i = __builtin_amdgcn_readfirstlane(c);
+  unsigned sbase = 0;
+  for (unsigned seq = 0; i < total; ++seq) {
+    unsigned nxt = 0;
+    if (threadIdx.x == 0) nxt = queue_claim(head);
+    while (i - sbase >= nb) sbase += nb;
+    const unsigned vb = i - sbase;
+    RiemannParams q = p;
+    asm volatile("" : "+s"(q.a));
+    const Acc l = lane_sum<M>(q, f, vb, sp);
+    asm volatile("" : "+v"(nxt));
+    if (!one_wave && threadIdx.x == 0) next_item[seq & 1] = nxt;
+    double v;
+    if constexpr (__is_same(Acc, double)) v = block_sum_dyn(l, red[seq & 1]);
+    else v = static_cast<double>(block_sum_dyn(l, red_acc[seq & 1]));
+    if (threadIdx.x == 0) {
+      if constexpr (TL) {
+        unsigned wg = blockIdx.x;
+        asm volatile("" : "+v"(wg));
+        tl.item_stamp[i] = timeline_realtime_after(v);
+        tl.item_owner[i] = wg;
+      }
+      partials[i] = v;
+    }
+    i = __builtin_amdgcn_readfirstlane(one_wave ? nxt : next_item[seq & 1]);
+  }
+  if (threadIdx.x == 0) {
+    if constexpr (TL) {
+      const unsigned long long t = timeline_realtime();
+      unsigned long long* clk = timeline_row(tl.shader_clock, 2);
+      clk[0] = te.clk;
+      clk[1] = timeline_shader_clock();
+      unsigned long long* st = timeline_row(tl.wg_stamps, 2);
+      st[0] = te.t;
+      st[1] = t;
+      unsigned xcc, hw;
+      asm volatile("s_getreg_b32 %0, hwreg(HW_REG_XCC_ID)" : "=s"(xcc));
+      asm volatile("s_getreg_b32 %0, hwreg(HW_REG_HW_ID)" : "=s"(hw));
+      unsigned* id = timeline_row(tl.hw, 2);
+      id[0] = xcc;
+      id[1] = hw;
+    }
+    const unsigned d = __hip_atomic_fetch_add(done, 1u, __ATOMIC_RELAXED, __HIP_MEMORY_SCOPE_AGENT);
+    if (d == gridDim.x - 1) {
+      __hip_atomic_store(head, 0u, __ATOMIC_RELAXED, __HIP_MEMORY_SCOPE_AGENT);
+      __hip_atomic_store(done, 0u, __ATOMIC_RELAXED, __HIP_MEMORY_SCOPE_AGENT);
+    }
+  }
+}
+template <DivMode M, class F>
+__global__ __launch_bounds__(kMaxBlock) void riemann_queue_kernel(
+    RiemannParams p, const double* table, int table_n, double* partials, int steps, unsigned nb,
+    unsigned* queue) {
+  queue_body<M, F>(p, table, table_n, partials, steps, nb, queue);
+}
+template <DivMode M, class F>
+__global__ __launch_bounds__(kMaxBlock) kFullOccupancy void riemann_queue_kernel_o8(
+    RiemannParams p, const double* table, int table_n, double* partials, int steps, unsigned nb,
+    unsigned* queue) {
+  queue_body<M, F>(p, table, table_n, partials, steps, nb, queue);
+}
+template <DivMode M, class F>
+__global__ __launch_bounds__(kMaxBlock) void riemann_queue_timeline_kernel(
+    RiemannParams p, const double* table, int table_n, double* partials, int steps, unsigned nb,
+    unsigned* queue, QueueTimelineOut tl) {
+  queue_body<M, F, true>(p, table, table_n, partials, steps, nb, queue, tl);
+}
+template <DivMode M, class F>
+__global__ __launch_bounds__(kMaxBlock) kFullOccupancy void riemann_queue_timeline_kernel_o8(
+    RiemannParams p, const double* table, int table_n, double* partials, int steps, unsigned nb,
+    unsigned* queue, QueueTimelineOut tl) {
+  queue_body<M, F, true>(p, table, table_n, partials, steps, nb, queue, tl);
+}
+template <DivMode M, class F>
+constexpr bool queue_pays() {
+  return M == DivMode::kSeriesExact && __is_same(F, Pi4);
+}
+
 __global__ __launch_bounds__(kMaxBlock) void multistep_close_kernel(const double* partials,
                                                                    int nb, double scale,
                                                                    double* out) {
@@ -914,6 +1036,45 @@
   }
 }
 
+template <DivMode M, class F>
+void launch_queue_t(const RiemannParams& p, LaunchShape shape, int wgs, const double* table,
+                    int table_n, double* partials, int steps, unsigned* queue,
+                    const QueueTimelineOut* tl, hipStream_t stream) {
+  const unsigned nb = static_cast<unsigned>(shape.grid);
+  if constexpr (!multistep_pays<M, F>()) {
+    fail("this integrand/division keeps chained batches (no multi-step kernel, no queue)",
+         __FILE__, __LINE__);
+  } else if constexpr (multistep_o8<M, F>()) {
+    if (tl)
+      riemann_queue_timeline_kernel_o8<M, F><<<wgs, shape.block, 0, stream>>>(
+          p, table, table_n, partials, steps, nb, queue, *tl);
+    else
+      riemann_queue_kernel_o8<M, F><<<wgs, shape.block, 0, stream>>>(p, table, table_n, partials,
+                                                                     steps, nb, queue);
+  } else {
+    if (tl)
+      riemann_queue_timeline_kernel<M, F><<<wgs, shape.block, 0, stream>>>(
+          p, table, table_n, partials, steps, nb, queue, *tl);
+    else
+      riemann_queue_kernel<M, F><<<wgs, shape.block, 0, stream>>>(p, table, table_n, partials,
+                                                                  steps, nb, queue);
+  }
+}
+template <DivMode M, class F>
+void queue_per_cu_t(int block, bool timeline, int* out) {
+  *out = 0;
+  if constexpr (multistep_pays<M, F>()) {
+    const void* k;
+    if constexpr (multistep_o8<M, F>())
+      k = timeline ? reinterpret_cast<const void*>(&riemann_queue_timeline_kernel_o8<M, F>)
+                   : reinterpret_cast<const void*>(&riemann_queue_kernel_o8<M, F>);
+    else
+      k = timeline ? reinterpret_cast<const void*>(&riemann_queue_timeline_kernel<M, F>)
+                   : reinterpret_cast<const void*>(&riemann_queue_kernel<M, F>);
+    MIINT_HIP(hipOccupancyMaxActiveBlocksPerMultiprocessor(out, k, block, 0));
+  }
+}
+
 std::atomic<bool> g_pi4_library_division{false};
 std::atomic<bool> g_trig_library{false};
 inline bool trig_library() { return g_trig_library.load(std::memory_order_relaxed); }
@@ -1026,6 +1187,15 @@
 template <DivMode M, class F> struct TimelineOccOp {
   static void run(int block, int* out) { timeline_per_cu_t<M, F>(block, out); }
 };
+template <DivMode M, class F> struct QueueOp {
+  template <class... A> static void run(A... a) { launch_queue_t<M, F>(a...); }
+};
+template <DivMode M, class F> struct QueueOccOp {
+  static void run(int block, bool timeline, int* out) { queue_per_cu_t<M, F>(block, timeline, out); }
+};
+template <DivMode M, class F> struct QueuePaysOp {
+  static void run(bool* out) { *out = multistep_pays<M, F>() && queue_pays<M, F>(); }
+};
 template <DivMode M, class F> struct TileLenOp {
   static void run(int* out) { *out = F::template tile_len<M>(); }
 };
@@ -1222,6 +1392,48 @@
   launch_multistep_close(partials, shape.grid, steps, scale, out, shape.block, stream);
 }
 
+int riemann_queue_grid(const RiemannParams& p, DType dtype, DivMode div, int block, int num_cus,
+                       bool timeline) {
+  MIINT_CHECK(riemann_block_ok(block), "unsupported Riemann block size");
+  int per_cu = 0;
+  dispatch<QueueOccOp>(p, dtype, effective_div(p, div, dtype), block, timeline, &per_cu);
+  return per_cu * num_cus;
+}
+
+bool riemann_queue_pays(const RiemannParams& p, DType dtype, DivMode div) {
+  bool pays = false;
+  dispatch<QueuePaysOp>(p, dtype, effective_div(p, div, dtype), &pays);
+  return pays;
+}
+
+void launch_riemann_queue(const RiemannParams& p, DType dtype, DivMode div, LaunchShape shape,
+                          int workgroups, const double* table, int table_n, double* partials,
+                          int steps, double scale, double* out, hipStream_t stream,
+                          unsigned int* queue, bool close_kernel, const QueueTimeline* timeline) {
+  check_shape(shape);
+  check_params(p, table, table_n);
+  MIINT_CHECK(workgroups >= 1 && workgroups <= (1 << 20), "queue launch: workgroups out of range");
+  MIINT_CHECK(steps >= 1 && steps <= kMaxMultiSteps, "queue launch: 1..64 steps");
+  MIINT_CHECK(partials != nullptr && out != nullptr && queue != nullptr,
+              "queue launch needs partials, results and the queue words");
+  static_assert(sizeof(unsigned long long) == sizeof(uint64_t), "stamp words are 64-bit");
+  QueueTimelineOut tl{};
+  if (timeline) {
+    MIINT_CHECK(timeline->item_stamp && timeline->item_owner && timeline->wg_stamps &&
+                    timeline->shader_clock && timeline->hw,
+                "queue timeline launch needs its five buffers");
+    tl = {reinterpret_cast<unsigned long long*>(timeline->item_stamp), timeline->item_owner,
+          reinterpret_cast<unsigned long long*>(timeline->wg_stamps),
+          reinterpret_cast<unsigned long long*>(timeline->shader_clock), timeline->hw};
+  }
+  const DivMode eff = effective_div(p, div, dtype);
+  dispatch<QueueOp>(p, dtype, eff, prepared(p, eff), shape, workgroups, table, table_n, partials,
+                    steps, queue, timeline ? &tl : nullptr, stream);
+  MIINT_HIP(hipGetLastError());
+  if (!close_kernel) return;
+  launch_multistep_close(partials, shape.grid, steps, scale, out, shape.block, stream);
+}
+
 void launch_multistep_close(const double* partials, int grid, int steps, double scale,
                             double* out, int block, hipStream_t stream) {
   MIINT_CHECK(steps >= 1 && steps <= kMaxMultiSteps && grid >= 1 && riemann_block_ok(block),
diff --git a/csrc/python/module.cpp b/csrc/python/module.cpp
--- a/csrc/python/module.cpp
+++ b/csrc/python/module.cpp
@@ -265,6 +265,8 @@
       .def_readwrite("timeout_s", &RiemannConfig::timeout_s)
       .def_readwrite("host_direct", &RiemannConfig::host_direct)
       .def_readwrite("close", &RiemannConfig::close)
+      .def_readwrite("work", &RiemannConfig::work)
+      .def_readwrite("queue_wg_per_cu", &RiemannConfig::queue_wg_per_cu)
       .def_readwrite("allreduce_to_host", &RiemannConfig::allreduce_to_host)
       .def_readwrite("chain", &RiemannConfig::chain);
 
@@ -343,18 +345,20 @@
              r["wall_us"] = d.wall_us;
              return r;
            }, py::arg("steps"))
-      .def("timeline_batch", [](RiemannPlan& p, int steps) {
+      .def("timeline_batch", [](RiemannPlan& p, int steps, const std::string& form) {
              BatchTimeline t;
              {
                py::gil_scoped_release nogil;
-               t = p.timeline_batch(steps);
+               t = p.timeline_batch(steps, form);
              }
              auto arr64 = [](const std::vector<uint64_t>& v, py::ssize_t rows, py::ssize_t cols) {
                py::array_t<uint64_t> a({rows, cols});
                std::copy(v.begin(), v.end(), a.mutable_data());
                return a;
              };
-             py::array_t<uint32_t> hw({static_cast<py::ssize_t>(t.grid), py::ssize_t(2)});
+             const bool queue = t.work == "queue";
+             const py::ssize_t rows = queue ? t.workgroups : t.grid;
+             py::array_t<uint32_t> hw({rows, py::ssize_t(2)});
              std::copy(t.hw.begin(), t.hw.end(), hw.mutable_data());
              py::dict r;
              r["steps"] = t.steps;
@@ -362,12 +366,23 @@
              r["block"] = t.block;
              r["clock_khz"] = t.clock_khz;
              r["device_us"] = t.device_us;
-             r["stamps"] = arr64(t.stamps, t.grid, t.steps + 2);
-             r["shader_clock"] = arr64(t.shader_clock, t.grid, 2);
+             r["work"] = t.work;
+             if (queue) {
+               r["workgroups"] = t.workgroups;
+               r["wg_stamps"] = arr64(t.wg_stamps, rows, 2);
+               r["item_stamp"] = arr64(t.item_stamp, t.steps, t.grid);
+               py::array_t<uint32_t> owner({static_cast<py::ssize_t>(t.steps),
+                                            static_cast<py::ssize_t>(t.grid)});
+               std::copy(t.item_owner.begin(), t.item_owner.end(), owner.mutable_data());
+               r["item_owner"] = owner;
+             } else {
+               r["stamps"] = arr64(t.stamps, t.grid, t.steps + 2);
+             }
+             r["shader_clock"] = arr64(t.shader_clock, rows, 2);
              r["hw"] = hw;
              r["values"] = t.values;
              return r;
-           }, py::arg("steps"))
+           }, py::arg("steps"), py::arg("form") = "auto")
       .def("host_result", &RiemannPlan::host_result)
       .def_property_readonly("host_capacity", &RiemannPlan::host_capacity)
       .def_property_readonly("slots", &RiemannPlan::slots)
@@ -375,6 +390,8 @@
       .def_property_readonly("chained", &RiemannPlan::chained)
       .def_property_readonly("multistep", &RiemannPlan::multistep)
       .def_property_readonly("close_in_launch", &RiemannPlan::close_in_launch)
+      .def_property_readonly("work", [](const RiemannPlan& p) { return std::string(p.work()); })
+      .def_property_readonly("queue_workgroups", &RiemannPlan::queue_workgroups)
       .def_property_readonly("allreduce_to_host", &RiemannPlan::allreduce_to_host)
       .def_property_readonly("direct", &RiemannPlan::direct)
       .def_property_readonly("graph_nodes", &RiemannPlan::graph_nodes)
@@ -410,6 +427,19 @@
            std::vector<double> coef, double p0, double p1, DType dtype) {
           return pi4_ieee_narrow(make_params(integrand, a, h, off, i_begin, n, coef, p0, p1),
                                  dtype);
+        });
+  m.def("resolve_work",
+        [](const std::string& work, py::object env, bool pays, bool keeps_static) {
+          const std::string e = env.is_none() ? std::string() : env.cast<std::string>();
+          return resolve_work(work, env.is_none() ? nullptr : e.c_str(), pays, keeps_static);
+        },
+        py::arg("work"), py::arg("env") = py::none(), py::arg("pays") = false,
+        py::arg("keeps_static") = false);
+  m.def("riemann_queue_pays",
+        [](int integrand, double a, double h, double off, uint64_t i_begin, uint64_t n,
+           std::vector<double> coef, double p0, double p1, DType dtype, DivMode div) {
+          return riemann_queue_pays(make_params(integrand, a, h, off, i_begin, n, coef, p0, p1),
+                                    dtype, div);
         });
   m.attr("TRIG_SERIES_MAX_N") = kTrigSeriesMaxN;
   m.attr("FAST_TRIG_MAX_N") = kFastTrigMaxN;
diff --git a/csrc/runtime/integrator.cpp b/csrc/runtime/integrator.cpp
--- a/csrc/runtime/integrator.cpp
+++ b/csrc/runtime/integrator.cpp
@@ -2,6 +2,7 @@
 
 #include <algorithm>
 #include <atomic>
+#include <cstdlib>
 #include <cstring>
 #include <limits>
 #include <string>
@@ -85,6 +86,23 @@
     multistep_ = resident > 0 && shape_.grid <= resident;
     if (!multistep_) close_launch_ = false;
   }
+  {
+    const std::string w =
+        resolve_work(cfg.work, std::getenv("MIINT_MS_WORK"),
+                     multistep_ && riemann_queue_pays(params_, cfg.dtype, cfg.div),
+                     !multistep_ || close_launch_);
+    MIINT_CHECK(cfg.queue_wg_per_cu >= 0, "queue_wg_per_cu must be >= 0");
+    const int per_cu_max =
+        w == "queue" ? riemann_queue_grid(params_, cfg.dtype, cfg.div, cfg.block, 1) : 0;
+    if (per_cu_max > 0) {
+      const int per_cu =
+          cfg.queue_wg_per_cu > 0 ? std::min(cfg.queue_wg_per_cu, per_cu_max) : per_cu_max;
+      const uint64_t items = static_cast<uint64_t>(shape_.grid) * static_cast<uint64_t>(cfg.slots);
+      queue_wgs_ = static_cast<int>(
+          std::min<uint64_t>(static_cast<uint64_t>(per_cu) * info.num_cus, items));
+      work_queue_ = true;
+    }
+  }
 
   const int lanes = step_streams(cfg.slots);
   partials_ = DeviceBuffer<double>(2 * static_cast<size_t>(std::max(1, lanes)) *
@@ -100,6 +118,10 @@
   if (close_launch_) {
     ms_ticket_ = DeviceBuffer<unsigned int>(kTicketWords);
     MIINT_HIP(hipMemset(ms_ticket_.get(), 0, ms_ticket_.bytes()));
+  }
+  if (work_queue_) {
+    queue_ = DeviceBuffer<unsigned int>(kQueueWords);
+    MIINT_HIP(hipMemset(queue_.get(), 0, queue_.bytes()));
   }
   result_ = DeviceBuffer<double>(static_cast<size_t>(cfg.slots));
   sync_ = DeviceBuffer<double>(1);
@@ -276,10 +298,7 @@
                            static_cast<int>(cfg_.table.size()), slots_.get(), ticket_.get(),
                            scale_, result_ptr(0), cs);
     else if (multistep_)
-      launch_riemann_multistep(params_, cfg_.dtype, cfg_.div, shape_, table_.get(),
-                               static_cast<int>(cfg_.table.size()), ms_partials_.get(), nsteps,
-                               scale_, result_ptr(0), cs,
-                               close_launch_ ? ms_ticket_.get() : nullptr);
+      enqueue_multistep(cs, nsteps, true);
     else
       enqueue_chain_streams(cs, nsteps);
     if (bucketed()) {
@@ -311,6 +330,24 @@
   }
   ev_join_.record(rs);
   MIINT_HIP(hipStreamWaitEvent(cs, ev_join_.get(), 0));
+}
+
+void RiemannPlan::enqueue_multistep(hipStream_t s, int nsteps, bool close_kernel) const {
+  const int tn = static_cast<int>(cfg_.table.size());
+  if (work_queue_)
+    launch_riemann_queue(params_, cfg_.dtype, cfg_.div, shape_, queue_wgs_, table_.get(), tn,
+                         ms_partials_.get(), nsteps, scale_, result_ptr(0), s, queue_.get(),
+                         close_kernel);
+  else
+    launch_riemann_multistep(params_, cfg_.dtype, cfg_.div, shape_, table_.get(), tn,
+                             ms_partials_.get(), nsteps, scale_, result_ptr(0), s,
+                             close_launch_ ? ms_ticket_.get() : nullptr, close_kernel);
+}
+
+void RiemannPlan::reset_queue() const {
+  if (queue_.size() == 0) return;
+  (void)hipSetDevice(device_);
+  (void)hipMemset(queue_.get(), 0, queue_.bytes());
 }
 
 void RiemannPlan::capture_graphs() { batch_graph(cfg_.slots); }
@@ -417,13 +454,18 @@
 void RiemannPlan::sync() const {
   DeviceGuard g(device_);
   TraceRange tr("miint.plan.sync");
-  if (collective() && cfg_.timeout_s > 0) {
-    wait_with_timeout(comm_stream_.get(), cfg_.timeout_s, comm_);
-    wait_with_timeout(compute_.get(), cfg_.timeout_s, comm_);
-    return;
-  }
-  compute_.sync();
-  comm_stream_.sync();
+  try {
+    if (collective() && cfg_.timeout_s > 0) {
+      wait_with_timeout(comm_stream_.get(), cfg_.timeout_s, comm_);
+      wait_with_timeout(compute_.get(), cfg_.timeout_s, comm_);
+      return;
+    }
+    compute_.sync();
+    comm_stream_.sync();
+  } catch (...) {
+    reset_queue();
+    throw;
+  }
 }
 
 void RiemannPlan::barrier() {
@@ -459,7 +501,6 @@
   TraceRange tr("miint.plan.diagnose_batch");
   check_allreduce_to_host();
   hipStream_t cs = compute_.get();
-  const int tn = static_cast<int>(cfg_.table.size());
   BatchDiag d;
   d.steps = nsteps;
   {
@@ -479,9 +520,7 @@
   barrier();
   e0.record(cs);
   if (chained() && nsteps > 1 && multistep_) {
-    launch_riemann_multistep(params_, cfg_.dtype, cfg_.div, shape_, table_.get(), tn,
-                             ms_partials_.get(), nsteps, scale_, result_ptr(0), cs,
-                             close_launch_ ? ms_ticket_.get() : nullptr, false);
+    enqueue_multistep(cs, nsteps, false);
     e1.record(cs);
     if (!close_launch_)
       launch_multistep_close(ms_partials_.get(), shape_.grid, nsteps, scale_, result_ptr(0),
@@ -531,7 +570,7 @@
   return d;
 }
 
-BatchTimeline RiemannPlan::timeline_batch(int nsteps) {
+BatchTimeline RiemannPlan::timeline_batch(int nsteps, const std::string& form) {
   MIINT_CHECK(nsteps >= 1 && nsteps <= cfg_.slots, "timeline_batch: 1 <= steps <= slots");
   MIINT_CHECK(multistep(), "timeline_batch: not a multi-step plan (its batches run chained or "
                            "fused launches: there is no persistent launch to time)");
@@ -539,6 +578,73 @@
   DeviceGuard g(device_);
   TraceRange tr("miint.plan.timeline_batch");
   const DeviceInfo info = device_info(device_);
+  MIINT_CHECK(form == "auto" || form == "static" || form == "queue",
+              "timeline_batch: form must be auto, static or queue (got " + form + ")");
+  MIINT_CHECK(form != "queue" || work_queue_,
+              "timeline_batch: not a queue plan (RiemannConfig::work)");
+  if (form == "queue" || (form == "auto" && work_queue_ && cfg_.work == "queue")) {
+    BatchTimeline t;
+    t.steps = nsteps;
+    t.grid = shape_.grid;
+    t.block = shape_.block;
+    t.work = "queue";
+    t.workgroups = queue_wgs_;
+    MIINT_HIP(hipDeviceGetAttribute(&t.clock_khz, hipDeviceAttributeWallClockRate, device_));
+    MIINT_CHECK(t.clock_khz > 0, "timeline_batch: the device reports no wall clock rate");
+    const size_t wgs = static_cast<size_t>(queue_wgs_);
+    const size_t items = static_cast<size_t>(shape_.grid) * static_cast<size_t>(nsteps);
+    if (qtl_item_stamp_.size() == 0) {
+      const size_t cap = static_cast<size_t>(shape_.grid) * static_cast<size_t>(cfg_.slots);
+      qtl_item_stamp_ = DeviceBuffer<uint64_t>(cap);
+      qtl_item_owner_ = DeviceBuffer<uint32_t>(cap);
+      qtl_wg_stamps_ = DeviceBuffer<uint64_t>(wgs * 2);
+      qtl_shader_ = DeviceBuffer<uint64_t>(wgs * 2);
+      qtl_hw_ = DeviceBuffer<uint32_t>(wgs * 2);
+    }
+    check_allreduce_to_host();
+    hipStream_t cs = compute_.get();
+    sync();
+    barrier();
+    MIINT_HIP(hipMemsetAsync(qtl_item_stamp_.get(), 0, qtl_item_stamp_.bytes(), cs));
+    MIINT_HIP(hipMemsetAsync(qtl_item_owner_.get(), 0xff, qtl_item_owner_.bytes(), cs));
+    MIINT_HIP(hipMemsetAsync(qtl_wg_stamps_.get(), 0, qtl_wg_stamps_.bytes(), cs));
+    MIINT_HIP(hipMemsetAsync(qtl_shader_.get(), 0, qtl_shader_.bytes(), cs));
+    MIINT_HIP(hipMemsetAsync(qtl_hw_.get(), 0xff, qtl_hw_.bytes(), cs));
+    const QueueTimeline q{qtl_item_stamp_.get(), qtl_item_owner_.get(), qtl_wg_stamps_.get(),
+                          qtl_shader_.get(), qtl_hw_.get()};
+    Event a0, a1;
+    a0.record(cs);
+    launch_riemann_queue(params_, cfg_.dtype, cfg_.div, shape_, queue_wgs_, table_.get(),
+                         static_cast<int>(cfg_.table.size()), ms_partials_.get(), nsteps, scale_,
+                         result_ptr(0), cs, queue_.get(), true, &q);
+    a1.record(cs);
+    if (bucketed())
+      enqueue_bucket_reduce(cs, nsteps);
+    else if (!direct_)
+      MIINT_HIP(hipMemcpyAsync(host_.get(), result_.get(), sizeof(double) * nsteps,
+                               hipMemcpyDeviceToHost, cs));
+    t.item_stamp.resize(items);
+    t.item_owner.resize(items);
+    t.wg_stamps.resize(wgs * 2);
+    t.shader_clock.resize(wgs * 2);
+    t.hw.resize(wgs * 2);
+    MIINT_HIP(hipMemcpyAsync(t.item_stamp.data(), qtl_item_stamp_.get(), items * sizeof(uint64_t),
+                             hipMemcpyDeviceToHost, cs));
+    MIINT_HIP(hipMemcpyAsync(t.item_owner.data(), qtl_item_owner_.get(), items * sizeof(uint32_t),
+                             hipMemcpyDeviceToHost, cs));
+    MIINT_HIP(hipMemcpyAsync(t.wg_stamps.data(), qtl_wg_stamps_.get(), qtl_wg_stamps_.bytes(),
+                             hipMemcpyDeviceToHost, cs));
+    MIINT_HIP(hipMemcpyAsync(t.shader_clock.data(), qtl_shader_.get(), qtl_shader_.bytes(),
+                             hipMemcpyDeviceToHost, cs));
+    MIINT_HIP(hipMemcpyAsync(t.hw.data(), qtl_hw_.get(), qtl_hw_.bytes(), hipMemcpyDeviceToHost,
+                             cs));
+    sync();
+    last_mode_ = 1;
+    t.device_us = Event::elapsed_ms(a0, a1) * 1e3;
+    t.values.resize(static_cast<size_t>(nsteps));
+    for (int j = 0; j < nsteps; ++j) t.values[static_cast<size_t>(j)] = host_[j];
+    return t;
+  }
   const int resident =
       riemann_timeline_grid(params_, cfg_.dtype, cfg_.div, shape_.block, info.num_cus);
   MIINT_CHECK(shape_.grid <= resident,
diff --git a/cuda_v_mpi_amd/integrate.py b/cuda_v_mpi_amd/integrate.py
--- a/cuda_v_mpi_amd/integrate.py
+++ b/cuda_v_mpi_amd/integrate.py
@@ -52,7 +52,8 @@
                  chain: bool = True, comm_obj=None, threads: int = 0,
                  slice_of: tuple[int, int] | None = None, step_streams: int = 0,
                  block: int = 256, multistep: bool = True, close: str = "auto",
-                 allreduce_to_host: bool = True, timeout_s: float = 300.0, **spec_kw):
+                 allreduce_to_host: bool = True, timeout_s: float = 300.0,
+                 work: str = "auto", queue_wg_per_cu: int = 0, **spec_kw):
         spec = integrands.get(integrand, **spec_kw) if isinstance(integrand, str) else integrand
         if a is not None or b is not None:
             spec = dataclasses.replace(spec, a=spec.a if a is None else a,
@@ -97,6 +98,10 @@
             cfg.step_streams = step_streams
             cfg.multistep = multistep
             cfg.close = close
+            if work not in ("auto", "static", "queue"):
+                raise ValueError("work must be auto|static|queue")
+            cfg.work = work
+            cfg.queue_wg_per_cu = queue_wg_per_cu
             cfg.allreduce_to_host = allreduce_to_host
             cfg.timeout_s = timeout_s
             if slice_of is not None:
@@ -192,10 +197,10 @@
         if self._plan is not None:
             self._plan.sync()
 
-    def timeline(self, steps: int) -> dict:
+    def timeline(self, steps: int, form: str = "auto") -> dict:
         if self._plan is None:
             raise RuntimeError("timeline needs backend='hip'")
-        t = self._plan.timeline_batch(steps)
+        t = self._plan.timeline_batch(steps, form)
         t["xcc"] = t["hw"][:, 0] & 0xF
         return t
 
```

New measurement: 32280 billion (median of 6 runs). 1.02x the previous value.
